# nzfeng/signed-heat-3d

Measured on AMD Instinct MI355X. Metric: grid-nodes/sec end-to-end SHM (conv+PCG), higher is better.
Workload: dtype f64 (Step 1: f64 / packed-f32 tiers)

## Files before the change

signed-heat-3d_amd/csrc/shm_kernels.hip.h:

```cpp
#pragma once
#include <hip/hip_runtime.h>
#include <stdint.h>

#include <type_traits>

#include "shm_constraints.h"
#include "shm_mc_table.h"

namespace shm {

constexpr int kBlock = 256;
constexpr int kMaxPartials = 8192;

__device__ __forceinline__ double wave_sum(double v) {
#pragma unroll
    for (int off = 32; off > 0; off >>= 1) v += __shfl_down(v, off, kWave);
    return v;
}

__device__ __forceinline__ double block_sum(double v, double* lds ) {
    v = wave_sum(v);
    const int lane = threadIdx.x & 63, w = threadIdx.x >> 6;
    if (lane == 0) lds[w] = v;
    __syncthreads();
// ... 584 lines not shown
        for (int r = 0; r < RY; r++) {
            const int j = j0 + r;
            T left = __shfl_up(cur[r + 1][VEC - 1], 1, kWave), right = __shfl_down(cur[r + 1][0], 1, kWave);
            if (active && j < n) {
                if (threadIdx.x == 0 || lane == 0) left = (i > 0) ? row_ptr(kk, j)[-1] : cur[r + 1][0];
                if (threadIdx.x == blockDim.x - 1 || lane == 63 || i + VEC >= n) right = (i + VEC < n) ? row_ptr(kk, j)[VEC] : cur[r + 1][VEC - 1];
                T out[VEC];
#pragma unroll
                for (int e = 0; e < VEC; e++) {
                    const T c = cur[r + 1][e];
                    const T xm = (e == 0) ? left : cur[r + 1][e - 1];
                    const T xp = (e == VEC - 1) ? right : cur[r + 1][e + 1];
                    const T s = (xp + cur[r + 2][e] + nxt[r][e] + xm + cur[r][e] + prv[r][e]) - (T)6 * c;
                    out[e] = -s * ih2;
                    acc += (double)c * (double)out[e];
                }
                store_vec<T, VEC>(q + (size_t)(kk + 1) * plane + (size_t)j * n + i, out);
            }
        }
        if (active && kk + 1 < kk1) {
#pragma unroll
            for (int r = 0; r < RY; r++)
#pragma unroll
                for (int e = 0; e < VEC; e++) {
                    prv[r][e] = cur[r + 1][e];
                    cur[r + 1][e] = nxt[r][e];
                }
            load_row(kk + 1, j0 - 1, cur[0]);
            load_row(kk + 1, j0 + RY, cur[RY + 1]);
        }
    }
    const int tid = threadIdx.y * blockDim.x + threadIdx.x;
    acc = wave_sum(acc);
    if ((tid & 63) == 0) red[tid >> 6] = acc;
    __syncthreads();
    if (tid == 0) partials[lb] = red[0] + red[1] + red[2] + red[3];
}

template <typename T>
__global__ __launch_bounds__(kBlock) void laplacian_kernel(GridParams G, const T* __restrict__ u, T* __restrict__ out) {
    const int n = G.n;
    const size_t plane = (size_t)n * n;
    const size_t nown = (size_t)G.nzl * plane;
    for (size_t v = (size_t)blockIdx.x * kBlock + threadIdx.x; v < nown; v += (size_t)gridDim.x * kBlock) {
        const int kk = (int)(v / plane);
        const int rem = (int)(v - (size_t)kk * plane);
        const int j = rem / n, i = rem - j * n;
        const int k = G.k0 + kk;
        const size_t c = v + plane;
        const T uc = u[c];
        const T xp = (i < n - 1) ? u[c + 1] : uc, xm = (i > 0) ? u[c - 1] : uc;
        const T yp = (j < n - 1) ? u[c + n] : uc, ym = (j > 0) ? u[c - n] : uc;
        const T zp = (k < n - 1) ? u[c + plane] : uc, zm = (k > 0) ? u[c - plane] : uc;
        out[c] = ((xp + yp + zp + xm + ym + zm) - (T)6 * uc) * (T)G.inv_h2;
    }
}

enum Scalar : int {
    SC_RHO0 = 0,
    SC_RHO_A = 1,
    SC_RHO_B = 2,
    SC_UW = 3,
    SC_SHIFT = 4,
    SC_AREA = 5,
    SC_RR = 6,
    SC_RR0 = 7,
    SC_RZ = 8,
    SC_SUMB = 9,
    SC_AXSUM = 10,
    SC_COUNT = 16
};

static __global__ __launch_bounds__(kBlock) void finalize_sum_kernel(const double* __restrict__ partials, int np, double* __restrict__ dst) {
    __shared__ double red[8];
    double s = 0.;
    for (int a = threadIdx.x; a < np; a += kBlock) s += partials[a];
    s = block_sum(s, red);
    if (threadIdx.x == 0) *dst = s;
}

template <typename T, int VEC>
__global__ __launch_bounds__(kBlock) void update_xr_kernel(size_t nvec , size_t off ,
                                                           const double* __restrict__ sc, int rho_slot, const double* __restrict__ pq,
                                                           T* __restrict__ x, const T* __restrict__ p, T* __restrict__ r,
                                                           const T* __restrict__ q, double* __restrict__ partials) {
    __shared__ double red[8];
    const double rho_cur = sc[rho_slot];
    const double alpha_d = rho_cur == 0. ? 0. : rho_cur / *pq;
    const T alpha = (T)alpha_d;
    double acc = 0.;
    for (size_t v = (size_t)blockIdx.x * kBlock + threadIdx.x; v < nvec; v += (size_t)gridDim.x * kBlock) {
        const size_t c = off + v * VEC;
        T xv[VEC], pv[VEC], rv[VEC], qv[VEC];
        load_vec<T, VEC>(x + c, xv);
        load_vec<T, VEC>(p + c, pv);
        load_vec<T, VEC>(r + c, rv);
        load_vec<T, VEC>(q + c, qv);
#pragma unroll
        for (int e = 0; e < VEC; e++) {
            xv[e] += alpha * pv[e];
            rv[e] += alpha * qv[e];
            acc += (double)rv[e] * (double)rv[e];
        }
        store_vec<T, VEC>(x + c, xv);
        store_vec<T, VEC>(r + c, rv);
    }
    acc = block_sum(acc, red);
    if (threadIdx.x == 0) partials[blockIdx.x] = acc;
}

template <typename T, int VEC>
__global__ __launch_bounds__(kBlock) void norm2_kernel(size_t nvec, size_t off, const T* __restrict__ v_, double* __restrict__ partials) {
    __shared__ double red[8];
    double acc = 0.;
    for (size_t v = (size_t)blockIdx.x * kBlock + threadIdx.x; v < nvec; v += (size_t)gridDim.x * kBlock) {
        T a[VEC];
        load_vec<T, VEC>(v_ + off + v * VEC, a);
#pragma unroll
        for (int e = 0; e < VEC; e++) acc += (double)a[e] * (double)a[e];
    }
    acc = block_sum(acc, red);
    if (threadIdx.x == 0) partials[blockIdx.x] = acc;
}

template <typename T, int VEC>
__global__ __launch_bounds__(kBlock) void update_p_kernel(size_t nvec, size_t off, double* __restrict__ sc, int rho_old_slot, int rho_new_slot,
                                                          const double* __restrict__ red0, int init, int use_uw, const T* __restrict__ z,
                                                          T* __restrict__ p) {
    const double rho_new = *red0 - (use_uw ? sc[SC_UW] : 0.);
    const double rho_old = sc[rho_old_slot];
    const double beta_d = (init || rho_old == 0.) ? 0. : rho_new / rho_old;
    const T beta = (T)beta_d;
    for (size_t v = (size_t)blockIdx.x * kBlock + threadIdx.x; v < nvec; v += (size_t)gridDim.x * kBlock) {
        const size_t c = off + v * VEC;
        T zv[VEC], pv[VEC];
        load_vec<T, VEC>(z + c, zv);
        if (!init) load_vec<T, VEC>(p + c, pv);
#pragma unroll
        for (int e = 0; e < VEC; e++) pv[e] = init ? -zv[e] : (-zv[e] + beta * pv[e]);
        store_vec<T, VEC>(p + c, pv);
    }
    if (blockIdx.x == 0 && threadIdx.x == 0) {
        sc[rho_new_slot] = rho_new;
        if (init) sc[SC_RHO0] = rho_new;
    }
}

template <typename T>
__global__ __launch_bounds__(kBlock) void gather_rows_kernel(int m, const int* __restrict__ row_ptr, const uint32_t* __restrict__ ent_node,
                                                             const double* __restrict__ ent_coef, const T* __restrict__ v,
                                                             const double* __restrict__ partials, int np, double* __restrict__ red) {
    __shared__ double lds[8];
    if (blockIdx.x == 0) {
        double s = 0.;
        for (int a = threadIdx.x; a < np; a += kBlock) s += partials[a];
        s = block_sum(s, lds);
        if (threadIdx.x == 0) red[0] = s;
        return;
    }
    const int gid = (blockIdx.x - 1) * kBlock + threadIdx.x, row = gid >> 3, k = gid & 7;
    double term = 0.;
    if (row < m) {
        const int e = row_ptr[row] + k;
        if (e < row_ptr[row + 1]) term = ent_coef[e] * (double)v[ent_node[e]];
    }
    const int base = (int)(threadIdx.x & 63) & ~7;
    double s = 0.;
#pragma unroll
    for (int a = 0; a < 8; a++) s += __shfl(term, base + a, 64);
    if (row < m && k == 0) red[1 + row] = s;
}

template <typename TM, int U>
__global__ __launch_bounds__(kBlock) void ginv_matvec_kernel(int m, int ld, const TM* __restrict__ Ginv, const double* __restrict__ w,
                                                             double* __restrict__ u) {
    __shared__ double lds[8];
    const int row = blockIdx.x;
    const TM* g = Ginv + (size_t)row * ld;
    auto load4 = [&](int c, TM (&gv)[4]) {
        if (sizeof(TM) == 4) *reinterpret_cast<float4*>(gv) = *reinterpret_cast<const float4*>(g + c);
        else {
            *reinterpret_cast<double2*>(gv) = *reinterpret_cast<const double2*>(g + c);
            *reinterpret_cast<double2*>(gv + 2) = *reinterpret_cast<const double2*>(g + c + 2);
        }
    };
    auto dot4 = [&](int c, const TM (&gv)[4]) {
        double s = (double)gv[0] * w[c];
        if (c + 1 < m) s += (double)gv[1] * w[c + 1];
        if (c + 2 < m) s += (double)gv[2] * w[c + 2];
        if (c + 3 < m) s += (double)gv[3] * w[c + 3];
        return s;
    };
    double s = 0.;
    for (int c0 = 0; c0 < m; c0 += U * kBlock * 4) {
        TM gv[U][4];
#pragma unroll
        for (int a = 0; a < U; a++) {
            const int c = c0 + (threadIdx.x + a * kBlock) * 4;
            if (c < m) load4(c, gv[a]);
        }
#pragma unroll
        for (int a = 0; a < U; a++) {
            const int c = c0 + (threadIdx.x + a * kBlock) * 4;
            if (c < m) s += dot4(c, gv[a]);
        }
    }
    s = block_sum(s, lds);
    if (threadIdx.x == 0) u[row] = s;
}
template <typename TM>
static inline void launch_ginv_matvec(hipStream_t st, int rows, int m, int ld, const TM* G, const double* w, double* u) {
    if (m <= 4 * kBlock * 4) hipLaunchKernelGGL((ginv_matvec_kernel<TM, 4>), dim3(rows), dim3(kBlock), 0, st, m, ld, G, w, u);
    else hipLaunchKernelGGL((ginv_matvec_kernel<TM, 8>), dim3(rows), dim3(kBlock), 0, st, m, ld, G, w, u);
}

template <typename T>
__global__ __launch_bounds__(kBlock) void scatter_nodes_kernel(int nnodes, const uint32_t* __restrict__ node_id, const int* __restrict__ node_ptr,
                                                               const int* __restrict__ ent_row, const double* __restrict__ ent_coef,
                                                               const double* __restrict__ u, const double* __restrict__ w, int m,
                                                               double* __restrict__ sc, int save_rr ,
                                                               T* __restrict__ v, int nred, double* scratch , unsigned* ticket ) {
    __shared__ double lds[8];
    if ((int)blockIdx.x < nred) {
        const int chunk = (m + nred - 1) / nred, a0 = (int)blockIdx.x * chunk, a1 = min(m, a0 + chunk);
        double s = 0.;
        for (int a = a0 + (int)threadIdx.x; a < a1; a += kBlock) s += u[a] * w[a];
        s = block_sum(s, lds);
        __shared__ unsigned last;
        if (threadIdx.x == 0) {
            scratch[blockIdx.x] = s;
            __threadfence();
            last = atomicAdd(ticket, 1u) == (unsigned)nred - 1u;
        }
        __syncthreads();
        if (!last) return;
        if (threadIdx.x == 0) {
            __threadfence();
            double tot = 0.;
            for (int b = 0; b < nred; b++) tot += __builtin_nontemporal_load(scratch + b);
            *ticket = 0u;
            sc[SC_UW] = tot;
            if (save_rr) sc[SC_RR] = w[-1] - tot;
            if (save_rr == 2) sc[SC_RR0] = w[-1] - tot;
        }
        return;
    }
    const int t = ((int)blockIdx.x - nred) * kBlock + threadIdx.x;
    if (t >= nnodes) return;
    double s = 0.;
    for (int e = node_ptr[t]; e < node_ptr[t + 1]; e++) s += ent_coef[e] * u[ent_row[e]];
    v[node_id[t]] = (T)((double)v[node_id[t]] - s);
}

template <typename T>
__global__ __launch_bounds__(kBlock) void shift_partial_kernel(int nitems, const ShiftItem* __restrict__ items, int n, const T* __restrict__ x,
                                                               double* __restrict__ partials) {
    __shared__ double red[8];
    double acc = 0.;
    for (int a = blockIdx.x * kBlock + threadIdx.x; a < nitems; a += gridDim.x * kBlock) {
        const ShiftItem it = items[a];
        const double v00 = -(double)x[it.node], v10 = -(double)x[it.node + 1];
        const double v01 = -(double)x[it.node + n], v11 = -(double)x[it.node + n + 1];
        const double a0 = v00 * (1. - it.tx) + v10 * it.tx;
        const double a1 = v01 * (1. - it.tx) + v11 * it.tx;
        acc += it.weight * (a0 * (1. - it.ty) + a1 * it.ty);
    }
    acc = block_sum(acc, red);
    if (threadIdx.x == 0) partials[blockIdx.x] = acc;
}

template <typename T>
__global__ __launch_bounds__(kBlock) void write_phi_kernel(size_t nown, size_t off, const T* __restrict__ x, const double* __restrict__ red0,
                                                           double area_sum, double* __restrict__ sc, T* __restrict__ phi) {
    const double shift = *red0 / area_sum;
    for (size_t v = (size_t)blockIdx.x * kBlock + threadIdx.x; v < nown; v += (size_t)gridDim.x * kBlock)
        phi[off + v] = (T)(-(double)x[off + v] - shift);
    if (blockIdx.x == 0 && threadIdx.x == 0) sc[SC_SHIFT] = shift;
}

template <typename T>
__device__ __forceinline__ double bfs_step(const T* __restrict__ Y0, const T* __restrict__ Y1, const T* __restrict__ Y2, size_t p, size_t q,
                                           double e0, double e1, double e2) {
    double a0 = (double)Y0[q] + (double)Y0[p], a1 = (double)Y1[q] + (double)Y1[p], a2 = (double)Y2[q] + (double)Y2[p];
    const double nrm = sqrt(a0 * a0 + a1 * a1 + a2 * a2);
    a0 /= nrm; a1 /= nrm; a2 /= nrm;
    return a0 * e0 + a1 * e1 + a2 * e2;
}

template <typename T>
__global__ __launch_bounds__(1024) void bfs_plane0_kernel(int n, double cell, double bx, double by, const T* __restrict__ Y0,
                                                          const T* __restrict__ Y1, const T* __restrict__ Y2, T* __restrict__ x) {
    const size_t off = (size_t)n * n;
    if (threadIdx.x == 0) {
        double phi = 0.;
        x[off] = (T)0;
        for (int i = 1; i < n; i++) {
            const double e0 = (i * cell + bx) - ((i - 1) * cell + bx);
            phi = phi + bfs_step<T>(Y0, Y1, Y2, off + i - 1, off + i, e0, 0., 0.);
            x[off + i] = (T)(-phi);
        }
    }
    __syncthreads();
    for (int i = threadIdx.x; i < n; i += blockDim.x) {
        double phi = -(double)x[off + i];
        for (int j = 1; j < n; j++) {
            const double e1 = (j * cell + by) - ((j - 1) * cell + by);
            phi = phi + bfs_step<T>(Y0, Y1, Y2, off + (size_t)(j - 1) * n + i, off + (size_t)j * n + i, 0., e1, 0.);
            x[off + (size_t)j * n + i] = (T)(-phi);
        }
    }
}

template <typename T>
__global__ __launch_bounds__(kBlock) void bfs_z_kernel(GridParams G, double cell, double bz, const T* __restrict__ Y0, const T* __restrict__ Y1,
                                                       const T* __restrict__ Y2, T* __restrict__ x) {
    const size_t plane = (size_t)G.n * G.n;
    const size_t ij = (size_t)blockIdx.x * kBlock + threadIdx.x;
    if (ij >= plane) return;
    const int kk0 = (G.k0 == 0) ? 1 : 0;
    double phi = -(double)x[(size_t)kk0 * plane + ij];
    for (int kk = kk0; kk < G.nzl; kk++) {
        const int k = G.k0 + kk;
        const double e2 = (k * cell + bz) - ((k - 1) * cell + bz);
        const size_t q = (size_t)(kk + 1) * plane + ij, pidx = q - plane;
        phi = phi + bfs_step<T>(Y0, Y1, Y2, pidx, q, 0., 0., e2);
        x[q] = (T)(-phi);
    }
}

constexpr int kDualBlock = 1024;

__device__ __forceinline__ double block_sum_1024(double v, double* lds ) {
    v = wave_sum(v);
    const int lane = threadIdx.x & 63, w = threadIdx.x >> 6;
    __syncthreads();
    if (lane == 0) lds[w] = v;
    __syncthreads();
    if (threadIdx.x == 0) {
        double s = 0.;
        for (int a = 0; a < kDualBlock / kWave; a++) s += lds[a];
        lds[16] = s;
    }
    __syncthreads();
    return lds[16];
}

template <typename T>
__global__ __launch_bounds__(kBlock) void scatter_rows_to_nodes_kernel(int nnodes, const uint32_t* __restrict__ node_id, const int* __restrict__ node_ptr,
                                                                       const int* __restrict__ ent_row, const double* __restrict__ ent_coef,
                                                                       const double* __restrict__ v, int accumulate, T* __restrict__ w, double scale = 1.0,
                                                                       T* __restrict__ saved = nullptr ) {
    const int t = blockIdx.x * kBlock + threadIdx.x;
    if (t >= nnodes) return;
    double s = 0.;
    for (int e = node_ptr[t]; e < node_ptr[t + 1]; e++) s += ent_coef[e] * v[ent_row[e]];
    const T old = w[node_id[t]];
    if (saved) saved[t] = old;
    w[node_id[t]] = (T)((accumulate ? (double)old : 0.) + scale * s);
}
template <typename T>
__global__ __launch_bounds__(kBlock) void restore_nodes_kernel(int nnodes, const uint32_t* __restrict__ node_id, const T* __restrict__ saved, T* __restrict__ w) {
    const int t = blockIdx.x * kBlock + threadIdx.x;
    if (t < nnodes) w[node_id[t]] = saved[t];
}

static __global__ __launch_bounds__(kBlock) void csr_matvec_kernel(int m, const int* __restrict__ ptr, const int* __restrict__ col, const double* __restrict__ val,
                                                            const double* __restrict__ x, double* __restrict__ y) {
    const int r = blockIdx.x * kBlock + threadIdx.x;
    if (r >= m) return;
    double s = 0.;
    for (int e = ptr[r]; e < ptr[r + 1]; e++) s += val[e] * x[col[e]];
    y[r] = s;
}

template <typename T>
__global__ __launch_bounds__(kBlock) void negate_kernel(size_t count, const T* __restrict__ in, T* __restrict__ out) {
    for (size_t v = (size_t)blockIdx.x * kBlock + threadIdx.x; v < count; v += (size_t)gridDim.x * kBlock) out[v] = -in[v];
}

template <typename T>
__global__ __launch_bounds__(kBlock) void sum_kernel(size_t nown, size_t off, const T* __restrict__ v, double* __restrict__ partials) {
    __shared__ double red[8];
    double acc = 0.;
    for (size_t a = (size_t)blockIdx.x * kBlock + threadIdx.x; a < nown; a += (size_t)gridDim.x * kBlock) acc += (double)v[off + a];
    acc = block_sum(acc, red);
    if (threadIdx.x == 0) partials[blockIdx.x] = acc;
}

static __global__ __launch_bounds__(kDualBlock) void dual_init_mu_kernel(int m, const double* __restrict__ sumb, double* __restrict__ mu, double* __restrict__ sc) {
    const double v = *sumb / (double)m;
    for (int a = threadIdx.x; a < m; a += kDualBlock) mu[a] = v;
    if (threadIdx.x == 0) sc[SC_SUMB] = *sumb;
}

static __global__ __launch_bounds__(kDualBlock) void dual_init_residual_kernel(int m, const double* __restrict__ g, const double* __restrict__ Smu,
                                                                        double* __restrict__ r, double* __restrict__ sc, int set_rr0 = 1) {
    __shared__ double lds[17];
    double s = 0.;
    for (int a = threadIdx.x; a < m; a += kDualBlock) s += g[a] - Smu[a];
    const double mean = block_sum_1024(s, lds) / (double)m;
    double rr = 0.;
    for (int a = threadIdx.x; a < m; a += kDualBlock) {
        const double v = g[a] - Smu[a] - mean;
        r[a] = v;
        rr += v * v;
    }
    rr = block_sum_1024(rr, lds);
    if (threadIdx.x == 0) {
        sc[SC_RR] = rr;
        if (set_rr0) sc[SC_RR0] = rr;
    }
}

static __global__ __launch_bounds__(kDualBlock) void dual_direction_kernel(int m, int init, const double* __restrict__ r, double* __restrict__ z,
                                                                    double* __restrict__ p, double* __restrict__ sc) {
    __shared__ double lds[17];
    double s = 0.;
    for (int a = threadIdx.x; a < m; a += kDualBlock) s += z[a];
    const double mean = block_sum_1024(s, lds) / (double)m;
    double rz = 0.;
    for (int a = threadIdx.x; a < m; a += kDualBlock) {
        const double v = z[a] - mean;
        z[a] = v;
        rz += r[a] * v;
    }
    rz = block_sum_1024(rz, lds);
    const double rz_old = sc[SC_RZ];
    const double beta = (init || rz_old == 0.) ? 0. : rz / rz_old;
    for (int a = threadIdx.x; a < m; a += kDualBlock) p[a] = init ? z[a] : z[a] + beta * p[a];
    __syncthreads();
    if (threadIdx.x == 0) sc[SC_RZ] = rz;
}

static __global__ __launch_bounds__(kDualBlock) void dual_update_kernel(int m, const double* __restrict__ Sp, const double* __restrict__ p, double* __restrict__ mu,
                                                                 double* __restrict__ r, double* __restrict__ sc) {
    __shared__ double lds[17];
    double s = 0.;
    for (int a = threadIdx.x; a < m; a += kDualBlock) s += Sp[a];
    const double mean = block_sum_1024(s, lds) / (double)m;
    double pSp = 0.;
    for (int a = threadIdx.x; a < m; a += kDualBlock) pSp += p[a] * (Sp[a] - mean);
    pSp = block_sum_1024(pSp, lds);
    const double rz_cur = sc[SC_RZ];
    const double alpha = rz_cur == 0. ? 0. : rz_cur / pSp;
    double rr = 0.;
    for (int a = threadIdx.x; a < m; a += kDualBlock) {
        mu[a] += alpha * p[a];
        const double v = r[a] - alpha * (Sp[a] - mean);
        r[a] = v;
        rr += v * v;
    }
    rr = block_sum_1024(rr, lds);
    if (threadIdx.x == 0) sc[SC_RR] = rr;
}

static __global__ __launch_bounds__(kBlock) void sum_slabs_kernel(int nslabs, double* const* __restrict__ bufs, int count) {
    const int a = blockIdx.x * kBlock + threadIdx.x;
    if (a >= count) return;
    double s = 0.;
    for (int t = 0; t < nslabs; t++) s += bufs[t][a];
    for (int t = 0; t < nslabs; t++) bufs[t][a] = s;
}

static __global__ __launch_bounds__(kBlock) void scatter_triplets_kernel(size_t cnt, const uint64_t* __restrict__ idx, const double* __restrict__ val,
                                                                  double* __restrict__ dense) {
    for (size_t a = (size_t)blockIdx.x * kBlock + threadIdx.x; a < cnt; a += (size_t)gridDim.x * kBlock) dense[idx[a]] = val[a];
}

template <typename TS, typename TD>
__global__ __launch_bounds__(kBlock) void convert_kernel(size_t count, const TS* __restrict__ src, TD* __restrict__ dst) {
    for (size_t v = (size_t)blockIdx.x * kBlock + threadIdx.x; v < count; v += (size_t)gridDim.x * kBlock) dst[v] = (TD)src[v];
}


struct GjBatch {
    const int* ptrI;
    const size_t* offD;
    const size_t* offW;
    double* D;
    double* P;
    double* R;
    double* C;
};
__device__ __forceinline__ int gj_batch_ld(const GjBatch& B, int a) { return (B.ptrI[a + 1] - B.ptrI[a] + kGJ - 1) / kGJ * kGJ; }

template <int E, int KR>
__device__ __forceinline__ void gj_scalar_step(double (&r)[E][E], double (*rowk)[kGJ], double (*colk)[kGJ], int kq, int ty, int tx, int* __restrict__ flag) {
    const int k = kq * E + KR;
    constexpr int pb = KR & 1;
    if (kq == ty) {
#pragma unroll
        for (int b = 0; b < E; b++) rowk[pb][tx * E + b] = r[KR][b];
    }
    if (kq == tx) {
#pragma unroll
        for (int a = 0; a < E; a++) colk[pb][ty * E + a] = r[a][KR];
    }
    __syncthreads();
    const double piv = rowk[pb][k];
    if (threadIdx.x == 0 && !(piv > 0.)) *flag = 1;
    double ip = __builtin_amdgcn_rcp(piv);
    ip = fma(fma(-piv, ip, 1.0), ip, ip);
    ip = fma(fma(-piv, ip, 1.0), ip, ip);
    double rv[E], cv[E];
#pragma unroll
    for (int b = 0; b < E; b++) rv[b] = rowk[pb][tx * E + b];
#pragma unroll
    for (int a = 0; a < E; a++) cv[a] = colk[pb][ty * E + a];
    const bool rowsel = ty == kq, colsel = tx == kq;
#pragma unroll
    for (int a = 0; a < E; a++)
#pragma unroll
        for (int b = 0; b < E; b++) {
            const double rowv = rv[b] * ip, colv = -cv[a] * ip;
            const double base = fma(-cv[a], rowv, r[a][b]);
            if (a == KR && b == KR) r[a][b] = rowsel ? (colsel ? ip : rowv) : (colsel ? colv : base);
            else if (a == KR) r[a][b] = rowsel ? rowv : base;
            else if (b == KR) r[a][b] = colsel ? colv : base;
            else r[a][b] = base;
        }
}
template <int E, int KR>
__device__ __forceinline__ void gj_scalar_step2(double (&r)[E][E], double* __restrict__ lds, int kq, int ty, int tx, int* __restrict__ flag) {
    static_assert(KR % 2 == 0 && KR + 1 < E, "a pair of pivots inside one block");
    const int k = kq * E + KR;
    double* buf = lds + ((KR >> 1) & 1) * 4 * kGJ;
    double *rowA = buf, *rowB = buf + kGJ, *colA = buf + 2 * kGJ, *colB = buf + 3 * kGJ;
    if (kq == ty) {
#pragma unroll
        for (int b = 0; b < E; b++) {
            rowA[tx * E + b] = r[KR][b];
            rowB[tx * E + b] = r[KR + 1][b];
        }
    }
    if (kq == tx) {
#pragma unroll
        for (int a = 0; a < E; a++) {
            colA[ty * E + a] = r[a][KR];
            colB[ty * E + a] = r[a][KR + 1];
        }
    }
    __syncthreads();
    const double piv0 = rowA[k], m01 = rowA[k + 1], m10 = colA[k + 1], m11 = rowB[k + 1];
    if (threadIdx.x == 0 && !(piv0 > 0.)) *flag = 1;
    double ip0 = __builtin_amdgcn_rcp(piv0);
    ip0 = fma(fma(-piv0, ip0, 1.0), ip0, ip0);
    ip0 = fma(fma(-piv0, ip0, 1.0), ip0, ip0);
    double rv0[E], cv0[E], rv1[E], cv1[E];
#pragma unroll
    for (int b = 0; b < E; b++) {
        rv0[b] = rowA[tx * E + b];
        rv1[b] = rowB[tx * E + b];
    }
#pragma unroll
    for (int a = 0; a < E; a++) {
        cv0[a] = colA[ty * E + a];
        cv1[a] = colB[ty * E + a];
    }
    const bool rowsel = ty == kq, colsel = tx == kq;
    const double rowv0_k1 = m01 * ip0;
#pragma unroll
    for (int b = 0; b < E; b++) {
        const double base = fma(-m10, rv0[b] * ip0, rv1[b]);
        rv1[b] = (b == KR && colsel) ? -m10 * ip0 : base;
// ... 748 lines not shown
```

signed-heat-3d_amd/csrc/shm_solver.hip.h:

```cpp
#pragma once
#include "shm_host.hip.h"
#include "shm_kernels.hip.h"
#include "shm_conv_tiered.hip.h"
#include "shm_cg_fused.hip.h"
#include "shm_twolevel.hip.h"
#include "shm_schur.hip.h"
#include "shm_dct.hip.h"
#include "shm_dct_gemm.hip.h"
#include "shm_green_fft.hip.h"
#include "shm_sample.hip.h"
#include "shm_audit.hip.h"
#include "shm_iso_indexed.hip.h"
#include "shm_iso_components.hip.h"
#include "shm_raycast.hip.h"
#include "shm_redistance.hip.h"
#include "shm_redistance_exact.hip.h"
#include "shm_plan.h"

namespace shm {

template <typename T> constexpr int vec_width() { return sizeof(T) == 8 ? 2 : 4; }

template <typename T>
struct Slab {
    int k0 = 0, k1 = 0, nzl = 0;
    size_t plane = 0, nown = 0, ntot = 0;
    DevArray<T> Y0, Y1, Y2, r , x, p, q , z ;
    DevArray<double> partials, pq_partials , red , pq , u , sc;
    DevArray<unsigned> proj_ticket;
    DevArray<int> row_ptr, ent_row, node_ptr;
    DevArray<uint32_t> ent_node, node_id;
    DevArray<double> ent_coef, nent_coef;
    DevArray<ShiftItem> shift_items;
    DevArray<double> dv;
    DevArray<int> layer_order;
    DevArray<int> sample_order;
    DevArray<unsigned char> sample_rule;
    DevArray<unsigned long long> sample_ctr;
    long long sample_key = -1;
    int sample_blocks = 0;
    long long layer_order_key = -1;
    DevArray<double> div_partials;
    int div_sum_blocks = 0;
    DevArray<T> touched_save;
    DevArray<T> W1, W2;
    DevArray<T> S1, S2, S4;
    DevArray<int> act_x, act_y;
    DevArray<unsigned> act_z;
    DevArray<int> act_planes;
    int n_act_planes = 0;
    int n_act_x = 0, n_act_y = 0;
    int n_touched = 0, n_shift = 0;
    GridParams gp{};
};

template <typename T>
struct Solver final : SolverBase {
    shm_config cfg;
    hipStream_t stream = nullptr;
    hipStream_t stream2 = nullptr;
    hipStream_t stream3 = nullptr;
    std::unique_ptr<Event> e_sch_in, e_sch_done, e_gs_done;
    hipStream_t stream_h = nullptr;
    int n = 0, alloc_n = -1;
    size_t N = 0;
    double cell = 0., lambda = 0.;
    double bbox_min[3] = {0, 0, 0};
    double conv_ctr[3] = {0, 0, 0};
    double conv_wscale = 1.;
    int64_t S = 0;
    std::vector<double> h_pos, h_wn, h_area;
    double area_sum = 0., conv_far_gap = 0., conv_skip_base = 3.0e38, last_host_setup_ms = 0., last_setup_wall_ms = 0.;
    double conv_tier_log = 0., conv_tier_skip_base = 3.0e38;
    double conv_drop_K = 64., conv_drop_eps64 = 2e-9, conv_drop_eps32 = 6.0e-8;
    double conv_w_span = 0.;
    DevArray<double> d_src_t;
    DevArray<float> d_clusters_t;
    int n_clusters_t = 0;
    bool conv_tiered = false;
    bool conv_tier_exact = false;
    bool conv_tiered32 = false;
    bool conv_reference = false;
    int step1_selected = SHM_STEP1_AUTO;
    int last_step1_arith = SHM_STEP1_AUTO;
    double last_step1_budget = 0.;
    bool fold_pq = false;
    int fold_pq_np = 0;
    double step1_budget = 0.;
    DevArray<unsigned long long> d_pair_counters;
    DevArray<unsigned> d_unit_counters;
    static constexpr int kMaxConvLaunches = 256;
    int conv_launch_index = 0;
    int conv_launches_last = 0;
    int n_clusters = 0;
    int conv_grid_cap = 1 << 30;
    bool o_fast_hint = false;
    int num_cus = 256;
    DevArray<T> d_src;
    DevArray<float> d_src32;
    DevArray<float> d_clusters;
    DevArray<double> d_exptab;
    std::vector<Slab<T>> slabs;
    int total_slabs = 1, first_slab = 0;
    std::vector<int32_t> slab_bounds;
    bool slabs_equal = true;
    void slab_range(int slab, int32_t* k0, int32_t* k1) const {
        *k0 = slab_bounds[(size_t)slab];
        *k1 = slab_bounds[(size_t)slab + 1];
    }
    bool have_problem = false, have_conv = false, have_div = false, have_phi = false, have_constraints = false;
    std::vector<Row> rows;
    std::vector<std::vector<ShiftItem>> shift_host;
    int m = 0, mp = 0;
    DevArray<double> Ginv, gjP, gjR, gjC;
    DevArray<float> Ginv32;
    struct TwoLevel {
        bool on = false;
        int box = 16, P = 0, nI = 0, nS = 0, nSp = 0, ysz = 0;
        DevArray<int> ptrI, ptrS, rowsI, colsS, sepRow, adj_ptr, adj_idx, colour_list, rowBox, chunkBox, chunkCol, tBox, tRow, sBox, sRow;
        DevArray<size_t> offW;
        DevArray<double> gjP, gjR, gjC;
        int nChunks = 0, nTChunks = 0, nbMax = 0;
        int schur_ptr[9] = {0, 0, 0, 0, 0, 0, 0, 0, 0};
        DevArray<size_t> offD, offE;
        DevArray<double> D, E, Tm, tbuf, ybuf, vS, uS;
        DevArray<float> D32, E32, T32;
        int colour_ptr[9] = {0, 0, 0, 0, 0, 0, 0, 0, 0};
        size_t szD = 0, szE = 0;
        TlBoxes view() const { return TlBoxes{ptrI.p, ptrS.p, offD.p, offE.p, rowsI.p, colsS.p}; }
    } tl;
    int ginv_rows = 0, ginv_ld = 0;
    DevArray<int> gjFlag;
    DevArray<double*> d_redptrs;
    DevArray<int> Bptr, Bcol;
    DevArray<double> Bval;
    bool have_B = false;
    using TP = T;
    DevArray<Cplx<TP>> d_tw, d_om;
    DevArray<TP> d_lam;
    DevArray<double> d_lam64;
    DevArray<double> gd_Cm, gd_Ct, gd_W1, gd_W2;
    DevArray<double> gs_lam, gs_ctab, gs_Cm, gs_Ct, gs_W0, gs_W1, gs_T, Sdense, d_rowT;
    DevArray<int> d_rowX;
    std::vector<double> h_gs_lam, h_gs_ctab, h_rowT;
    std::vector<Cplx<double>> h_gs_tw;
    DevArray<Cplx<double>> gs_tw;
    std::vector<int> h_rowX;
    bool have_S = false;
    DevArray<double> Sinv, Sinv_ones ;
    PlanIn plan_in;
    Plan plan;
    double conv_est_total_ms = 1e30;
    int log2n = 0;
    bool precond_ready = false;
    double* h_pinned = nullptr;
    Rccl::comm_t comm = nullptr;
    int vec = 1;
    std::unique_ptr<Solver<T>> full;
    bool solve_only = false;
    bool full_problem_set = false;
    bool pool_held = false;

    explicit Solver(const shm_config& c, bool solve_only_ = false) : cfg(c), solve_only(solve_only_) {
        int ndev = 0;
        hipError_t e = hipGetDeviceCount(&ndev);
        if (e != hipSuccess || ndev <= 0)
            throw Error(SHM_ERR_HIP, fmt("no HIP device available (%s); this library has no CPU fallback",
                                          e == hipSuccess ? "device count 0" : hipGetErrorString(e)));
        if (cfg.device < 0 || cfg.device >= ndev) throw Error(SHM_ERR_INVALID, fmt("device %d out of range [0,%d)", cfg.device, ndev));
        HIPCHK(hipSetDevice(cfg.device));
        HIPCHK(hipStreamCreateWithFlags(&stream, hipStreamNonBlocking));
        {
            hipDeviceProp_t prop;
            HIPCHK(hipGetDeviceProperties(&prop, cfg.device));
            conv_grid_cap = std::max(1, prop.multiProcessorCount * 4);
            num_cus = prop.multiProcessorCount;
        }
        {
            int least = 0, greatest = 0;
            HIPCHK(hipDeviceGetStreamPriorityRange(&least, &greatest));
            HIPCHK(hipStreamCreateWithPriority(&stream2, hipStreamNonBlocking, greatest));
        }
        HIPCHK(hipHostMalloc((void**)&h_pinned, 64 * sizeof(double)));
        if (cfg.world > 1 && !cfg.rccl_unique_id) throw Error(SHM_ERR_INVALID, "world>1 needs rccl_unique_id");
        if (cfg.rccl_unique_id) {
            Rccl& R = Rccl::get();
            Rccl::unique_id id;
            memcpy(&id, cfg.rccl_unique_id, sizeof id);
            R.chk(R.CommInitRank(&comm, cfg.world, id, cfg.rank), "ncclCommInitRank");
        }
        PinnedPool::get().acquire(cfg.device);
        pool_held = true;
    }
    ~Solver() override {
        (void)hipSetDevice(cfg.device);
        if (comm) (void)Rccl::get().CommDestroy(comm);
        if (h_pinned) (void)hipHostFree(h_pinned);
        for (void* b : smp_pinned)
            if (b) (void)hipHostFree(b);
        for (void* b : ray_pinned)
            if (b) (void)hipHostFree(b);
        slabs.clear();
        if (stream) (void)hipStreamDestroy(stream);
        if (stream2) (void)hipStreamDestroy(stream2);
        if (stream3) (void)hipStreamDestroy(stream3);
        if (stream_h) (void)hipStreamDestroy(stream_h);
        if (pool_held) PinnedPool::get().release(cfg.device);
    }

    void log(const char* f, ...) {
        if (!cfg.verbose) return;
        va_list ap;
        va_start(ap, f);
        vfprintf(stderr, f, ap);
        va_end(ap);
        fputc('\n', stderr);
    }

    static int grid_for(size_t work_items, int cap = 2048) {
        size_t b = (work_items + kBlock - 1) / kBlock;
        if (b < 1) b = 1;
        if (b > (size_t)cap) b = cap;
        return (int)b;
    }

    void set_problem(const shm_sources& src, const shm_grid& g) override {
        HIPCHK(hipSetDevice(cfg.device));
        if (g.n < 2) throw Error(SHM_ERR_INVALID, "grid.n must be >= 2");
        if (!(g.cell > 0.) || !std::isfinite(g.cell)) throw Error(SHM_ERR_INVALID, "grid.cell must be positive and finite");
        if (src.S <= 0 || !src.pos || !src.wnormal || !src.area) throw Error(SHM_ERR_INVALID, "sources: S>0 and non-null arrays required");
        if (!(src.lambda > 0.) || !std::isfinite(src.lambda)) throw Error(SHM_ERR_INVALID, "sources.lambda must be positive and finite");
        if (src.S > (int64_t)1 << 28) throw Error(SHM_ERR_INVALID, "too many sources");
        total_slabs = cfg.world * cfg.local_slabs;
        first_slab = cfg.rank * cfg.local_slabs;
        if (g.n < total_slabs) throw Error(SHM_ERR_INVALID, fmt("grid.n=%d smaller than the number of z-slabs %d", g.n, total_slabs));
        n = g.n;
        N = (size_t)n * n * n;
        cell = g.cell;
        lambda = src.lambda;
        for (int a = 0; a < 3; a++) bbox_min[a] = g.bbox_min[a];
        S = src.S;
        h_pos.assign(src.pos, src.pos + 3 * S);
        h_wn.assign(src.wnormal, src.wnormal + 3 * S);
        h_area.assign(src.area, src.area + S);
        for (int64_t s = 0; s < S; s++)
            for (int a = 0; a < 3; a++) {
                const double d = (h_pos[3 * s + a] - bbox_min[a]) / cell;
                if (!(d >= 0.) || !(std::floor(d) + 1. <= (double)(n - 1)))
                    throw Error(SHM_ERR_INVALID, fmt("source %lld lies outside the grid cells", (long long)s));
            }
        area_sum = 0.;
        for (int64_t s = 0; s < S; s++) area_sum += h_area[s];
        {
            double lo[3] = {1e300, 1e300, 1e300}, hi[3] = {-1e300, -1e300, -1e300};
            for (int64_t s = 0; s < S; s++)
                for (int a = 0; a < 3; a++) {
                    lo[a] = std::min(lo[a], h_pos[3 * s + a]);
                    hi[a] = std::max(hi[a], h_pos[3 * s + a]);
                }
            const double ext = std::max({hi[0] - lo[0], hi[1] - lo[1], hi[2] - lo[2], 1e-300});
            auto spread = [](uint64_t v) {
                v &= 0x1fffff;
                v = (v | v << 32) & 0x1f00000000ffffULL;
                v = (v | v << 16) & 0x1f0000ff0000ffULL;
                v = (v | v << 8) & 0x100f00f00f00f00fULL;
                v = (v | v << 4) & 0x10c30c30c30c30c3ULL;
                v = (v | v << 2) & 0x1249249249249249ULL;
                return v;
            };
            std::vector<std::pair<uint64_t, int64_t>> order((size_t)S);
            for (int64_t s = 0; s < S; s++) {
                uint64_t code = 0;
                for (int a = 0; a < 3; a++) {
                    const uint64_t q = (uint64_t)std::min(1048575.0, std::max(0.0, (h_pos[3 * s + a] - lo[a]) / ext * 1048575.0));
                    code |= spread(q) << a;
                }
                order[(size_t)s] = {code, s};
            }
            std::sort(order.begin(), order.end());
            for (int a = 0; a < 3; a++) conv_ctr[a] = bbox_min[a] + 0.5 * (double)(n - 1) * cell;
            constexpr int kConvCluster = conv_cluster<T>();
            n_clusters = (int)((S + kConvCluster - 1) / kConvCluster);
            const int64_t Spad = (int64_t)n_clusters * kConvCluster;
            std::vector<T> packed((size_t)Spad * 6, (T)0);
            std::vector<float> packed32((size_t)Spad * 6, 0.f), cl((size_t)n_clusters * kConvClusterRec, 0.f);
            double amin = 1e300, amax = 0.;
            for (int64_t s = 0; s < S; s++) {
                const double w = std::sqrt(h_wn[3 * s] * h_wn[3 * s] + h_wn[3 * s + 1] * h_wn[3 * s + 1] + h_wn[3 * s + 2] * h_wn[3 * s + 2]);
                if (w > 0.) amin = std::min(amin, w);
                amax = std::max(amax, w);
            }
            conv_wscale = amax > 0. && std::isfinite(amax) ? std::ldexp(1.0, -std::ilogb(amax) - 1) : 1.0;
            conv_w_span = amax > 0. && amin < 1e300 ? std::log(amax / amin) : 0.;
            const double wscale = sizeof(T) == 4 ? conv_wscale : 1.0;
            for (int64_t t = 0; t < Spad; t++) {
                const int64_t s = order[(size_t)std::min<int64_t>(t, S - 1)].second;
                for (int a = 0; a < 3; a++) {
                    packed[6 * t + a] = (T)(h_pos[3 * s + a] - conv_ctr[a]);
                    packed32[6 * t + a] = (float)(h_pos[3 * s + a] - conv_ctr[a]);
                    if (t < S) {
                        packed[6 * t + 3 + a] = (T)(h_wn[3 * s + a] * wscale);
                        packed32[6 * t + 3 + a] = (float)(h_wn[3 * s + a] * wscale);
                    }
                }
            }
            for (int c = 0; c < n_clusters; c++) {
                double cc[3] = {0, 0, 0};
                for (int e = 0; e < kConvCluster; e++)
                    for (int a = 0; a < 3; a++) cc[a] += (double)packed[6 * ((size_t)c * kConvCluster + e) + a];
                for (int a = 0; a < 3; a++) cc[a] /= kConvCluster;
                double rad = 0.;
                for (int e = 0; e < kConvCluster; e++) {
                    double d2 = 0.;
                    for (int a = 0; a < 3; a++) {
                        const double d = (double)packed[6 * ((size_t)c * kConvCluster + e) + a] - cc[a];
                        d2 += d * d;
                    }
                    rad = std::max(rad, std::sqrt(d2));
                }
                for (int a = 0; a < 3; a++) cl[kConvClusterRec * (size_t)c + a] = (float)cc[a];
                cl[kConvClusterRec * (size_t)c + 3] = (float)(rad * 1.00001 + 1e-30);
                double wmax2 = 0., wsum = 0.;
                for (int e = 0; e < kConvCluster; e++) {
                    double w2 = 0.;
                    for (int a = 0; a < 3; a++) {
                        const double w = (double)packed[6 * ((size_t)c * kConvCluster + e) + 3 + a];
                        w2 += w * w;
                    }
                    wmax2 = std::max(wmax2, w2);
                    wsum += std::sqrt(w2);
                }
                cl[kConvClusterRec * (size_t)c + 4] = wmax2 > 0. ? (float)(0.5 * std::log(wmax2) + 1e-5) : -1.0e30f;
                cl[kConvClusterRec * (size_t)c + 5] = wsum > 0. ? (float)(std::log(wsum) + 1e-5) : -1.0e30f;
            }
            {
                const double far_log = 25.0;
                conv_far_gap = (far_log + std::log(std::max(1.0, amax / std::max(amin, 1e-300)))) / lambda;
                const double eps = sizeof(T) == 8 ? 1.1e-16 : 6.0e-8;
                const char* sk = knob("SHM_CONV_NO_SKIP");
                conv_skip_base = sk ? 3.0e38 : std::log((double)S / eps);
                const char* tl = knob("SHM_CONV_TIER_LOG");
                conv_tier_log = tl ? atof(tl) : 8.0;
                conv_tier_skip_base = sk ? 3.0e38 : std::log((double)S / 2e-9);
                conv_drop_eps64 = sk ? 0. : 2e-9;
                conv_drop_eps32 = sk ? 0. : 6.0e-8;
                conv_drop_K = drop_rule_K(S, h_wn.data(), lambda);
                select_step1_arith(SHM_STEP1_AUTO);
            }
            d_src.upload(packed, stream);
            d_src32.upload(packed32, stream);
            {
                const int per = conv_chunk<T>();
                const int nchunks = (n_clusters + per - 1) / per;
                for (int g = 0; g < nchunks; g++) {
                    const int a = g * per, b = std::min(n_clusters, a + per);
                    double cc[3] = {0, 0, 0};
                    for (int c = a; c < b; c++)
                        for (int t = 0; t < 3; t++) cc[t] += cl[kConvClusterRec * (size_t)c + t];
                    for (int t = 0; t < 3; t++) cc[t] /= (b - a);
                    double rad = 0., lnw = -1.0e30;
                    for (int c = a; c < b; c++) {
                        double d2 = 0.;
                        for (int t = 0; t < 3; t++) {
                            const double d = (double)cl[kConvClusterRec * (size_t)c + t] - cc[t];
                            d2 += d * d;
                        }
                        rad = std::max(rad, std::sqrt(d2) + (double)cl[kConvClusterRec * (size_t)c + 3]);
                        lnw = std::max(lnw, (double)cl[kConvClusterRec * (size_t)c + 4]);
                    }
                    for (int t = 0; t < 3; t++) cl.push_back((float)cc[t]);
                    cl.push_back((float)(rad * 1.00001 + 1e-30));
                    cl.push_back((float)lnw);
                    cl.push_back(0.f);
                }
            }
            d_clusters.upload(cl, stream);
            if constexpr (sizeof(T) == 8) {
                if (!solve_only)
                    conv_drop_K = choose_drop_K(reinterpret_cast<const double*>(packed.data()), n_clusters, cl.data(), kConvClusterRec, lambda, n, cell, conv_drop_eps64, S, conv_drop_K);
            }
            if constexpr (sizeof(T) == 4) {
                n_clusters_t = (int)((S + kTierCluster - 1) / kTierCluster);
                const int64_t Sp = (int64_t)n_clusters_t * kTierCluster;
                std::vector<double> pk((size_t)Sp * 6, 0.);
                for (int64_t t = 0; t < Sp; t++) {
                    const int64_t sidx = order[(size_t)std::min<int64_t>(t, S - 1)].second;
                    for (int a = 0; a < 3; a++) {
                        pk[6 * t + a] = h_pos[3 * sidx + a] - conv_ctr[a];
                        if (t < S) pk[6 * t + 3 + a] = h_wn[3 * sidx + a];
                    }
                }
                std::vector<float> clt((size_t)n_clusters_t * kConvClusterRec, 0.f);
                for (int c = 0; c < n_clusters_t; c++) {
                    const double* q = pk.data() + 6 * (size_t)c * kTierCluster;
                    double cc[3] = {0, 0, 0}, rad = 0., wmax2 = 0., wsum = 0.;
                    for (int e = 0; e < kTierCluster; e++)
                        for (int a = 0; a < 3; a++) cc[a] += q[6 * e + a] / kTierCluster;
                    for (int e = 0; e < kTierCluster; e++) {
                        double d2 = 0., w2 = 0.;
                        for (int a = 0; a < 3; a++) {
                            d2 += (q[6 * e + a] - cc[a]) * (q[6 * e + a] - cc[a]);
                            w2 += q[6 * e + 3 + a] * q[6 * e + 3 + a];
                        }
                        rad = std::max(rad, std::sqrt(d2));
                        wmax2 = std::max(wmax2, w2);
                        wsum += std::sqrt(w2);
                    }
                    for (int a = 0; a < 3; a++) clt[kConvClusterRec * (size_t)c + a] = (float)cc[a];
                    clt[kConvClusterRec * (size_t)c + 3] = (float)(rad * 1.00001 + 1e-30);
                    clt[kConvClusterRec * (size_t)c + 4] = wmax2 > 0. ? (float)(0.5 * std::log(wmax2) + 1e-5) : -1.0e30f;
                    clt[kConvClusterRec * (size_t)c + 5] = wsum > 0. ? (float)(std::log(wsum) + 1e-5) : -1.0e30f;
                }
                if (!solve_only)
                    conv_drop_K = choose_drop_K(pk.data(), n_clusters_t, clt.data(), kConvClusterRec, lambda, n, cell, conv_drop_eps32, S, conv_drop_K);
                d_src_t.upload(pk, stream);
                d_clusters_t.upload(clt, stream);
            }
            if (!d_exptab.p) {
                std::vector<double> tab(2048);
                for (int j = 0; j < 2048; j++) tab[(size_t)j] = std::exp2((double)j / 2048.0);
                d_exptab.upload(tab, stream);
            }
            HIPCHK(hipStreamSynchronize(stream));
        }

        {
            const bool weighted = cfg.slab_plan == SHM_SLAB_PLAN_STEP1 && total_slabs > 1 && !solve_only;
            slab_bounds.assign((size_t)total_slabs + 1, 0);
            if (weighted) {
                std::vector<double> w((size_t)n);
                step1_plane_weights_host(S, h_pos.data(), h_wn.data(), lambda, n, bbox_min, cell, sizeof(T) == 8 ? SHM_F64 : SHM_F32, conv_tier_log, w.data(),
                                         sizeof(T) == 4 && knob("SHM_CONV32_CLASSIC") == nullptr);
                plan_slabs_weighted(n, total_slabs, w.data(), sizeof(T) == 8 ? 4 : 8, slab_bounds);
            } else {
                for (int sidx = 0; sidx < total_slabs; sidx++) {
                    int32_t k0, k1;
                    shm_plan_slab(n, total_slabs, sidx, &k0, &k1);
                    slab_bounds[(size_t)sidx] = k0;
                    slab_bounds[(size_t)sidx + 1] = k1;
                }
            }
            slabs_equal = true;
            for (int sidx = 0; sidx < total_slabs; sidx++) {
                int32_t k0, k1;
                shm_plan_slab(n, total_slabs, sidx, &k0, &k1);
                slabs_equal = slabs_equal && slab_bounds[(size_t)sidx] == k0 && slab_bounds[(size_t)sidx + 1] == k1;
            }
        }
        vec = (n % vec_width<T>() == 0) ? vec_width<T>() : 1;
        if (!(have_problem && n == alloc_n && (int)slabs.size() == cfg.local_slabs)) {
            slabs.clear();
            slabs.resize(cfg.local_slabs);
        }
        alloc_n = n;
        for (int ls = 0; ls < cfg.local_slabs; ls++) {
            Slab<T>& sl = slabs[ls];
            int32_t k0, k1;
            slab_range(first_slab + ls, &k0, &k1);
            sl.k0 = k0;
            sl.k1 = k1;
            sl.nzl = k1 - k0;
            sl.plane = (size_t)n * n;
            sl.nown = sl.plane * sl.nzl;
            sl.ntot = sl.plane * (sl.nzl + 2);
            if (sl.ntot >= ((size_t)1 << 32)) throw Error(SHM_ERR_INVALID, "slab too large for 32-bit local node indices; use more slabs");
            if (!solve_only)
                for (DevArray<T>* a : {&sl.Y0, &sl.Y1, &sl.Y2}) a->alloc(sl.ntot);
            for (DevArray<T>* a : {&sl.r, &sl.x, &sl.p, &sl.q}) a->alloc(sl.ntot);
            HIPCHK(hipMemsetAsync(sl.p.p, 0, sl.ntot * sizeof(T), stream));
            if (!solve_only) HIPCHK(hipMemsetAsync(sl.Y2.p, 0, sl.ntot * sizeof(T), stream));
            sl.partials.alloc(std::max<size_t>(kMaxPartials, (size_t)n * n / 8 + 8));
            sl.pq.alloc(1);
            sl.sc.alloc(SC_COUNT);
            HIPCHK(hipMemsetAsync(sl.sc.p, 0, SC_COUNT * sizeof(double), stream));
            sl.gp.n = n;
            sl.gp.nzl = sl.nzl;
            sl.gp.k0 = sl.k0;
            sl.gp.inv_h = 1. / cell;
            sl.gp.inv_h2 = 1. / (cell * cell);
        }
        HIPCHK(hipStreamSynchronize(stream));
        precond_ready = false;
        have_problem = true;
        have_conv = have_div = have_phi = have_constraints = false;
        iso_idx_valid = false;
        ray_bricks_valid = false;
        redist_valid = false;
        audit_src_ready = false;
        full_problem_set = false;
        if (!(cfg.world > 1 && !solve_only && n >= 4 && n <= 1024)) full.reset();
        log("[shm] problem set: n=%d N=%zu S=%lld slabs=%d(local %d) vec=%d", n, N, (long long)S, total_slabs, cfg.local_slabs, vec);
    }

    bool full_wanted() const { return cfg.world > 1 && !solve_only && n >= 4 && n <= 1024; }
    void ensure_full() {
        if (!full_wanted()) return;
        if (!full) {
            shm_config c = cfg;
            c.world = 1;
            c.rank = 0;
            c.local_slabs = 1;
            c.rccl_unique_id = nullptr;
            full.reset(new Solver<T>(c, true));
        }
        if (!full_problem_set) {
            shm_sources src{};
            src.S = S;
            src.pos = h_pos.data();
            src.wnormal = h_wn.data();
            src.area = h_area.data();
            src.lambda = lambda;
            shm_grid g{};
            g.n = n;
            for (int a = 0; a < 3; a++) g.bbox_min[a] = bbox_min[a];
            g.cell = cell;
            full->set_problem(src, g);
            full_problem_set = true;
        }
    }
    Step1Kernel step1_kernel() const { return conv_tiered ? kStep1TieredF64 : conv_tiered32 ? kStep1TieredF32 : kStep1Untiered; }
    PlanIn plan_inputs(const shm_opts* o) const {
        PlanIn in;
        in.f64 = sizeof(T) == 8; in.n = n; in.S = S; in.total_slabs = total_slabs;
        in.full_wanted = full_wanted(); in.fft_available = fft_available(); in.gemm_dct = gemm_dct(); in.fused_available = fused_available();
        in.step1 = step1_kernel(); in.conv_est_total_ms = conv_est_total_ms;
        if (o) {
            in.solver = o->solver; in.preconditioner = o->preconditioner; in.dual_form = o->dual_form;
            in.step1_budget = o->step1_budget; in.fast = o->fast_integration != 0;
        }
        in.knobs = plan_knobs(knob);
        return in;
    }
    void select_step1_arith(int arith) {
        if (arith != SHM_STEP1_AUTO && arith != SHM_STEP1_EXACT_F64 && arith != SHM_STEP1_REFERENCE_F64) throw Error(SHM_ERR_INVALID, "unknown step1_arith");
        conv_reference = sizeof(T) == 8 && arith == SHM_STEP1_REFERENCE_F64;
        conv_tiered = sizeof(T) == 8 && arith == SHM_STEP1_AUTO && knob("SHM_CONV_EXACT") == nullptr && tier_exponent_span_ok();
        conv_tier_exact = sizeof(T) == 8 && arith == SHM_STEP1_EXACT_F64 && knob("SHM_CONV_EXACT_CLASSIC") == nullptr && tier_exponent_span_ok(true);
        conv_tiered = conv_tiered || conv_tier_exact;
        conv_tiered32 = sizeof(T) == 4 && knob("SHM_CONV32_CLASSIC") == nullptr && tier_exponent_span_ok();
        step1_selected = sizeof(T) == 4 || (conv_tiered && !conv_tier_exact) ? SHM_STEP1_AUTO : conv_reference ? SHM_STEP1_REFERENCE_F64 : SHM_STEP1_EXACT_F64;
    }
    bool tier_exponent_span_ok(bool every_pair = false) const {
        const double rt = std::sqrt(2 * 3.5 * 3.5 + 1.5 * 1.5) * cell;
        const double reach = every_pair ? lambda * std::sqrt(3.0) * (double)(n - 1) * cell : std::min((sizeof(T) == 8 ? conv_tier_skip_base : conv_skip_base) + 2.0794415416798357, 1.0e6);
        const double bits = (4.0 * rt * lambda + reach + std::max(conv_w_span, 43.0)) * 1.4426950408889634 + 16.0;
        return bits < 990.0;
    }
    void need_problem() const {
        if (!have_problem) throw Error(SHM_ERR_STATE, "shm_grid_set_problem has not been called");
    }

    const int* layer_order_for(Slab<T>& sl, int kk_begin, int layers, int npt) {
        const bool off = knob("SHM_TIER_LAYER_ORDER") != nullptr && atoi(knob("SHM_TIER_LAYER_ORDER")) == 0;
        if (off || layers < 16) return nullptr;
        const long long key = ((long long)kk_begin << 40) ^ ((long long)layers << 20) ^ ((long long)npt << 8) ^ (long long)sl.k0 * 0x9E3779B1LL;
        if (sl.layer_order.p && sl.layer_order_key == key) return sl.layer_order.p;
        std::vector<std::pair<double, int>> byc((size_t)layers);
        for (int l = 0; l < layers; l++) byc[(size_t)l] = {std::fabs((double)(sl.k0 + kk_begin - 1 + l * npt) + 0.5 * (npt - 1) - 0.5 * (n - 1)), l};
        std::stable_sort(byc.begin(), byc.end());
        std::vector<int> order;
        order.reserve((size_t)layers);
        for (int q = 0; q < 8; q++)
            for (int r = q; r < layers; r += 8) order.push_back(byc[(size_t)r].second);
        sl.layer_order.upload(order, stream);
        sl.layer_order_key = key;
        return sl.layer_order.p;
    }
    int far_rule_now() const {
        const char* e = knob("SHM_TIER_FAR_RULE");
        if (e) return atoi(e) != 0;
        return 0;
    }
    bool far_rule_plan(Slab<T>& sl, int planes, int npt) {
        if (sizeof(T) != 8 || !conv_tiered || conv_tier_exact || slabs.size() != 1 || total_slabs != 1 || knob("SHM_TIER_FAR_RULE") != nullptr) return false;
        if (step1_budget > 0. && step1_budget != kTierBudget) return false;
        const int layers = (planes + npt - 1) / npt;
        if (layers < 64 || layers % 8 != 0 || planes % npt != 0) return false;
        const long long key = ((long long)layers << 32) ^ ((long long)npt << 16);
        if (sl.sample_key != key) {
            std::vector<char> role((size_t)layers, 2);
            std::vector<int> A, B1;
            const int nA = 8;
            for (int a = 0; a < nA; a++) {
                const int l = (int)(((long long)(2 * a + 1) * layers) / (2 * nA));
                A.push_back(l);
                role[(size_t)l] = 1;
            }
            std::vector<std::pair<double, int>> byc;
            for (int l = 0; l < layers; l++)
                if (role[(size_t)l] != 1) byc.push_back({std::fabs((double)(sl.k0 + l * npt) + 0.5 * (npt - 1) - 0.5 * (n - 1)), l});
            std::stable_sort(byc.begin(), byc.end());
            for (int a = 0; a < 8; a++) B1.push_back(byc[(size_t)a].second);
            std::vector<int> order;
            std::vector<unsigned char> rule;
            size_t next_rest = 8;
            std::vector<std::vector<int>> rest(8);
            {
                std::vector<int> want(8);
                for (int q = 0; q < 8; q++) want[(size_t)q] = layers / 8 - 1 - ((nA == 8 || q % 2 == 0) ? 1 : 0);
                bool any = true;
                while (any && next_rest < byc.size()) {
                    any = false;
                    for (int q = 0; q < 8 && next_rest < byc.size(); q++)
                        if ((int)rest[(size_t)q].size() < want[(size_t)q]) {
                            rest[(size_t)q].push_back(byc[next_rest++].second);
                            any = true;
                        }
                }
            }
            for (int q = 0, a = 0; q < 8; q++) {
                if (nA == 8 || q % 2 == 0) {
                    order.push_back(A[(size_t)a++]);
                    rule.push_back(1);
                }
                order.push_back(B1[(size_t)q]);
                rule.push_back(0);
                for (int l : rest[(size_t)q]) {
                    order.push_back(l);
                    rule.push_back(2);
                }
            }
            if ((int)order.size() != layers) throw Error(SHM_ERR_INVALID, "far_rule_plan: internal count mismatch");
            sl.sample_blocks = nA * ((n + kTierTX - 1) / kTierTX) * ((n + kTierTY - 1) / kTierTY);
            sl.sample_order.upload(order, stream);
            sl.sample_rule.upload(rule, stream);
            sl.sample_ctr.alloc(4);
            sl.sample_key = key;
        }
        return true;
    }
    void launch_conv() {
        const bool slab_log = knob("SHM_CONV_SLAB_LOG") != nullptr;
        Event slab_ev[2];
        unsigned long long slab_pairs_seen[2] = {0, 0};
        for (Slab<T>& sl : slabs) {
            if (slab_log) {
                HIPCHK(hipStreamSynchronize(stream));
                slab_ev[0].record(stream);
            }
            ConvParams P;
            P.layer_order = nullptr;
            P.unit_rule = nullptr;
            P.sample_ctr = nullptr;
            P.sample_blocks = 0;
            P.far_rule = conv_tiered && !conv_tier_exact && sizeof(T) == 8 ? far_rule_now() : 0;
            P.n = n;
            P.kk_begin = 1;
            P.kk_end = sl.nzl + 1;
            P.k0 = sl.k0;
            for (int a = 0; a < 3; a++) P.bbox_min[a] = bbox_min[a] - conv_ctr[a];
            P.cell = cell;
            P.lambda = lambda;
            P.cexp = -lambda * 2954.639443740597;
            P.cexp_inv = 1.0 / std::fabs(P.cexp);
            P.S = n_clusters * conv_cluster<T>();
            P.n_clusters = n_clusters;
            P.far_gap = conv_reference ? 3.0e38f : (float)conv_far_gap;
            const double budget = step1_budget > 0. ? step1_budget : kTierBudget;
            const double g_shift = std::log(budget / kTierBudget);
            P.tier_log = conv_tier_exact ? 3.0e38f : conv_tiered32 ? -1.0e30f : (float)std::max(2.0, conv_tier_log - g_shift);
            P.wscale = conv_wscale;
            {
                const double ratio = budget / kTierEpsFar;
                P.far_redo_ratio = ratio > 0. ? (float)ratio : 3.0e38f;
            }
            P.skip_base = conv_tier_exact || conv_reference ? 3.0e38f : (float)std::min(conv_tiered ? conv_tier_skip_base - g_shift : conv_skip_base, 3.0e38);
            {
                const double eps = conv_tier_exact ? 0. : sizeof(T) == 8 ? conv_drop_eps64 * (budget / kTierBudget) : conv_drop_eps32;
                const double eps_soft = 0.875 * eps, tau = eps_soft / conv_drop_K, tau_hard = 0.125 * eps / (double)std::max<int64_t>(1, S);
                P.drop_eps_soft = (float)eps_soft;
                P.drop_ltau = eps > 0. ? (float)std::log2(tau) : -3.0e38f;
                P.drop_ltau_hard = eps > 0. ? (float)std::log2(tau_hard) : -3.0e38f;
                P.drop_tau_hard = (float)(tau_hard * 1.0001);
                P.drop_check = P.far_redo_ratio < 1.0e30f ? (float)((double)P.far_redo_ratio / budget) : (float)(1.0 / kTierEpsFar);
                P.tier_u0 = (float)kTierU0;
                P.tier_flush = kTierFlush;
            }
            P.inv_lambda = (float)(1.0 / lambda);
            P.tiles_x = (n + kConvTile - 1) / kConvTile;
            P.tiles_y = P.tiles_x;
            const int planes = P.kk_end - P.kk_begin;
            const bool npt4 = (long long)P.tiles_x * P.tiles_y * ((planes + 15) / 16) >= conv_grid_cap;
            const bool npt4_env = knob("SHM_CONV_NPT4") != nullptr;
            const bool npt8 = sizeof(T) == 4 && !npt4_env && npt4 && (long long)P.tiles_x * P.tiles_y * ((planes + 31) / 32) >= conv_grid_cap;
            const int tile_z = npt8 ? 32 : npt4 ? 16 : 8;
            const double half_z = 0.5 * ((npt8 ? 16 : tile_z) - 1);
            const double tile_diam = 2.0 * std::sqrt(2 * 3.5 * 3.5 + half_z * half_z) * cell;
            P.exact_offset = (lambda * tile_diam > 30.0) ? 1 : 0;
            const int tiles_z = (planes + tile_z - 1) / tile_z;
            P.n_tiles = P.tiles_x * P.tiles_y * tiles_z;
            unsigned grid = (unsigned)std::min(P.n_tiles, conv_grid_cap);
            {
                int occ = 0;
                const void* kfn = npt4 ? reinterpret_cast<const void*>(conv_normalize_kernel<T, 4>) : reinterpret_cast<const void*>(conv_normalize_kernel<T, 2>);
                if constexpr (sizeof(T) == 4)
                    if (npt8) kfn = reinterpret_cast<const void*>(conv_normalize_kernel<float, 8>);
                if (conv_tiered) kfn = npt4 ? reinterpret_cast<const void*>(conv_tiered_kernel<4, double, true>) : reinterpret_cast<const void*>(conv_tiered_kernel<2, double, true>);
                if (conv_tiered32) kfn = npt4 ? reinterpret_cast<const void*>(conv_tiered_kernel<4, float, false>) : reinterpret_cast<const void*>(conv_tiered_kernel<2, float, false>);
                if (hipOccupancyMaxActiveBlocksPerMultiprocessor(&occ, kfn, kBlock, 0) != hipSuccess || occ < 1) occ = 2;
                const unsigned resident = (unsigned)(occ * num_cus);
                const double pairs = (double)sl.nown * (double)S;
                const double conv_est_ms = pairs / (sizeof(T) == 8 ? 1.2e9 : 3.5e9);
                conv_est_total_ms = (&sl == &slabs[0] ? 0. : conv_est_total_ms) + conv_est_ms;
                const double setup_est_ms = 2.2e-3 * (double)std::min<int64_t>(S, (int64_t)8 * n * n);
                if (conv_tiered || conv_tiered32) grid = std::min(grid, resident);
                if (!o_fast_hint && conv_est_ms < 4.0 * setup_est_ms && grid > resident - resident / 8) grid = resident - resident / 8;
            }
            const bool uniform_tiles = lambda * cell * n < 100.;
            const int want_chunks = (conv_tiered || conv_tiered32) ? 1 : (uniform_tiles && conv_est_total_ms >= 10. ? std::min(16, (int)std::lround(conv_est_total_ms / 2.5)) : 1);
            const int nchunks = std::max(1, std::min(tiles_z, want_chunks));
            const int chunk_planes = ((tiles_z + nchunks - 1) / nchunks) * tile_z;
            if (!d_pair_counters.p) d_pair_counters.alloc(3);
            if (!d_unit_counters.p) d_unit_counters.alloc(8 * kMaxConvLaunches);
            if (&sl == &slabs[0]) {
                HIPCHK(hipMemsetAsync(d_pair_counters.p, 0, 3 * sizeof(unsigned long long), stream));
                HIPCHK(hipMemsetAsync(d_unit_counters.p, 0, 8 * kMaxConvLaunches * sizeof(unsigned), stream));
                conv_launch_index = 0;
                conv_launches_last = 0;
            }
            unsigned long long* const cnt = d_pair_counters.p;
            auto launch_range = [&](int b0, int b1, int sel, int rule = -1, const int* order = nullptr, int order_layers = 0) {
                if (b1 <= b0) return;
                conv_launches_last++;
                const int tz_sel = 4 * sel;
                ConvParams Pc = P;
                Pc.kk_begin = 1 + b0;
                Pc.kk_end = std::min(sl.nzl + 1, 1 + b1);
                Pc.n_tiles = P.tiles_x * P.tiles_y * ((Pc.kk_end - Pc.kk_begin + tz_sel - 1) / tz_sel);
                const dim3 g((unsigned)std::min<long long>(Pc.n_tiles, grid));
                if (conv_tiered || conv_tiered32) {
                    if (conv_launch_index >= kMaxConvLaunches) throw Error(SHM_ERR_INVALID, "too many Step-1 launches");
                    unsigned* const head = d_unit_counters.p + 8 * conv_launch_index++;
                    const int npt = npt4 ? 4 : 2;
                    Pc.tiles_x = (n + kTierTX - 1) / kTierTX;
                    Pc.tiles_y = (n + kTierTY - 1) / kTierTY;
                    const int layers = order ? order_layers : (Pc.kk_end - Pc.kk_begin + npt - 1) / npt;
                    Pc.n_tiles = Pc.tiles_x * Pc.tiles_y * layers;
                    Pc.layer_order = order ? order : layer_order_for(sl, Pc.kk_begin, layers, npt);
                    if (rule >= 0) Pc.far_rule = rule;
                    const dim3 gt((unsigned)std::min<long long>((Pc.n_tiles + 3) / 4, grid));
                    if constexpr (sizeof(T) == 8) {
                        if (npt4)
                            hipLaunchKernelGGL((conv_tiered_kernel<4, double, true>), gt, dim3(kBlock), 0, stream, Pc, d_src.p, d_clusters.p, d_exptab.p, sl.Y0.p, sl.Y1.p, sl.Y2.p, cnt, head);
                        else
                            hipLaunchKernelGGL((conv_tiered_kernel<2, double, true>), gt, dim3(kBlock), 0, stream, Pc, d_src.p, d_clusters.p, d_exptab.p, sl.Y0.p, sl.Y1.p, sl.Y2.p, cnt, head);
                    } else {
                        Pc.S = n_clusters_t * kTierCluster;
                        Pc.n_clusters = n_clusters_t;
                        if (npt4)
                            hipLaunchKernelGGL((conv_tiered_kernel<4, float, false>), gt, dim3(kBlock), 0, stream, Pc, d_src_t.p, d_clusters_t.p, d_exptab.p, sl.Y0.p, sl.Y1.p, sl.Y2.p, cnt, head);
                        else
                            hipLaunchKernelGGL((conv_tiered_kernel<2, float, false>), gt, dim3(kBlock), 0, stream, Pc, d_src_t.p, d_clusters_t.p, d_exptab.p, sl.Y0.p, sl.Y1.p, sl.Y2.p, cnt, head);
                    }
                    return;
                }
                unsigned* head = nullptr;
                if (conv_launch_index < kMaxConvLaunches) head = d_unit_counters.p + 8 * conv_launch_index++;
                if constexpr (sizeof(T) == 4) {
                    if (sel == 8) {
                        hipLaunchKernelGGL((conv_normalize_kernel<float, 8>), g, dim3(kBlock), 0, stream, Pc, d_src.p, d_src32.p, d_clusters.p, d_exptab.p, sl.Y0.p, sl.Y1.p,
                                           sl.Y2.p, cnt, head);
                        return;
                    }
                }
                if (sel >= 4)
                    hipLaunchKernelGGL((conv_normalize_kernel<T, 4>), g, dim3(kBlock), 0, stream, Pc, d_src.p, d_src32.p, d_clusters.p, d_exptab.p, sl.Y0.p, sl.Y1.p, sl.Y2.p, cnt, head);
                else
                    hipLaunchKernelGGL((conv_normalize_kernel<T, 2>), g, dim3(kBlock), 0, stream, Pc, d_src.p, d_src32.p, d_clusters.p, d_exptab.p, sl.Y0.p, sl.Y1.p, sl.Y2.p, cnt, head);
            };
            const int sel0 = npt8 ? 8 : npt4 ? 4 : 2;
            if (sizeof(T) == 4 && !conv_tiered32 && nchunks == 1 && sel0 > 2 && planes % tile_z != 0) {
                int b = (planes / tile_z) * tile_z;
                launch_range(0, b, sel0);
                for (int sel = sel0 / 2; sel >= 2; sel /= 2) {
                    const int tz_sel = 4 * sel, take = sel > 2 ? ((planes - b) / tz_sel) * tz_sel : planes - b;
                    launch_range(b, b + take, sel);
                    b += take;
                }
            } else if (far_rule_plan(sl, planes, npt4 ? 4 : 2)) {
                const int npt = npt4 ? 4 : 2, layers = planes / npt;
                HIPCHK(hipMemsetAsync(sl.sample_ctr.p, 0, 4 * sizeof(unsigned long long), stream));
                P.unit_rule = sl.sample_rule.p;
                P.sample_ctr = sl.sample_ctr.p;
                P.sample_blocks = sl.sample_blocks;
                launch_range(0, planes, sel0, 0, sl.sample_order.p, layers);
                P.unit_rule = nullptr;
            } else {
                for (int b0 = 0; b0 < planes; b0 += chunk_planes) launch_range(b0, std::min(planes, b0 + chunk_planes), sel0);
            }
            if (slab_log) {
                slab_ev[1].record(stream);
                HIPCHK(hipStreamSynchronize(stream));
                unsigned long long h[2] = {0, 0};
                HIPCHK(hipMemcpy(h, d_pair_counters.p, sizeof h, hipMemcpyDeviceToHost));
                fprintf(stderr, "[shm] step1 slab planes [%d,%d) ms %.3f pairs_fp64 %.6e pairs_fp32 %.6e\n", sl.k0, sl.k1, elapsed(slab_ev[0], slab_ev[1]),
                        (double)(h[0] - slab_pairs_seen[0]), (double)(h[1] - slab_pairs_seen[1]));
                slab_pairs_seen[0] = h[0];
                slab_pairs_seen[1] = h[1];
            }
        }
        HIPCHK(hipGetLastError());
        exchange_Y_halos();
        have_conv = true;
        last_step1_arith = step1_selected;
        last_step1_budget = sizeof(T) == 8 && conv_tiered && !conv_tier_exact ? (step1_budget > 0. ? step1_budget : kTierBudget) : 0.;
    }
    void exchange_Y_halos() {
        if (total_slabs <= 1) return;
        for (int sel : {ARR_Y0, ARR_Y1, ARR_Y2}) halo_exchange(sel);
    }

    void launch_div(int scrub) {
        for (Slab<T>& sl : slabs) {
            if (vec == 1) {
                hipLaunchKernelGGL((divergence_kernel<T>), dim3((unsigned)((n + kBlock - 1) / kBlock), (unsigned)n, (unsigned)sl.nzl), dim3(kBlock), 0, stream, sl.gp,
                                   sl.Y0.p, sl.Y1.p, sl.Y2.p, sl.r.p, scrub);
                sl.div_sum_blocks = 0;
                continue;
            }
            constexpr int V = vec_width<T>();
            const DivGeometry g = div_geometry(sl);
            sl.div_partials.alloc(g.nblk);
            sl.div_sum_blocks = (int)g.nblk;
            hipLaunchKernelGGL((divergence_march_kernel<T, V>), dim3(g.nblk), dim3(kBlock), 0, stream, sl.gp, g.LX, g.xchunks, g.rowgroups, g.ZC, sl.Y0.p, sl.Y1.p, sl.Y2.p,
                               sl.r.p, scrub, sl.div_partials.p);
        }
        HIPCHK(hipGetLastError());
        have_div = true;
    }
    struct DivGeometry {
        int LX, xchunks, rowgroups, ZC;
        unsigned nblk;
    };
    DivGeometry div_geometry(const Slab<T>& sl) const {
        constexpr int V = vec_width<T>();
        const int lanes = (n + V - 1) / V;
        int LX = 1;
        while (LX < lanes && LX < kBlock) LX *= 2;
        const int xchunks = (lanes + LX - 1) / LX, RB = kBlock / LX, rowgroups = (n + RB - 1) / RB;
        const int ZC = 4;
        return {LX, xchunks, rowgroups, ZC, (unsigned)((long long)xchunks * rowgroups * ((sl.nzl + ZC - 1) / ZC))};
    }
    void sum_b_in_div_order(Slab<T>& sl, hipStream_t on) {
        if (vec == 1) {
            sl.div_sum_blocks = 0;
            return;
        }
        constexpr int V = vec_width<T>();
        const DivGeometry g = div_geometry(sl);
        sl.div_partials.alloc(g.nblk);
        sl.div_sum_blocks = (int)g.nblk;
        hipLaunchKernelGGL((sum_march_kernel<T, V>), dim3(g.nblk), dim3(kBlock), 0, on, sl.gp, g.LX, g.xchunks, g.rowgroups, g.ZC, sl.r.p, sl.div_partials.p);
        HIPCHK(hipGetLastError());
    }

    void run_conv(int step1_arith) override {
        need_problem();
        HIPCHK(hipSetDevice(cfg.device));
        step1_budget = 0.;
        select_step1_arith(step1_arith);
        launch_conv();
        HIPCHK(hipStreamSynchronize(stream));
    }
    void run_divergence(int scrub) override {
        need_problem();
        if (!have_conv) throw Error(SHM_ERR_STATE, "run_conv must precede run_divergence");
        HIPCHK(hipSetDevice(cfg.device));
        launch_div(scrub);
        HIPCHK(hipStreamSynchronize(stream));
    }

    void build_rows() {
        shm::build_rows(S, h_pos.data(), bbox_min, cell, n, rows);
        m = (int)rows.size();
        mp = ((m + kGJ - 1) / kGJ) * kGJ;
    }

    void build_shift_items(hipStream_t stream) {
        shift_host.resize(slabs.size());
        for (size_t si = 0; si < slabs.size(); si++) {
            Slab<T>& sl = slabs[si];
            shift_items_for_slab(S, h_pos.data(), h_area.data(), bbox_min, cell, n, sl.k0, sl.k1, shift_host[si]);
            sl.n_shift = (int)shift_host[si].size();
            sl.shift_items.upload(shift_host[si], stream);
        }
    }
    void upload_red_tables(hipStream_t stream) {
        std::vector<double*> ptrs;
        for (Slab<T>& sl : slabs) ptrs.push_back(sl.red.p);
        for (Slab<T>& sl : slabs) ptrs.push_back(sl.pq.p);
        d_redptrs.upload(ptrs, stream);
        HIPCHK(hipStreamSynchronize(stream));
    }
    void build_shift_items_only() {
        build_shift_items(stream);
        upload_red_tables(stream);
    }

    double estimate_step1_ms_tiered() const {
        if (S <= 0) return 0.;
        if (conv_tier_exact) {
            double nodes = 0.;
            for (const Slab<T>& sl : slabs) nodes += (double)sl.nown;
            return nodes * (double)S * 1.229e-9;
        }
        const int K = (int)std::max<int64_t>(32, std::min<int64_t>(128, 2000000 / S));
        const int64_t stride = std::max<int64_t>(1, (S * K + 1999999) / 2000000);
        uint64_t st = 0x9E3779B97F4A7C15ULL;
        auto rnd = [&]() {
            st = st * 6364136223846793005ULL + 1442695040888963407ULL;
            return (double)(st >> 11) * (1.0 / 9007199254740992.0);
        };
        const double ext = (double)(n - 1) * cell, rt2 = 2.0 * 5.17 * cell;
        const double r_near_gap = rt2 + conv_tier_log / lambda, r_keep_gap = rt2 + std::log(std::min((double)S, conv_drop_K) / (0.875 * 2e-9)) / lambda;
        std::vector<float> d2((size_t)S);
        size_t c_near = 0, c_keep = 0;
        for (int k = 0; k < K; k++) {
            const float x = (float)(bbox_min[0] + rnd() * ext), y = (float)(bbox_min[1] + rnd() * ext), z = (float)(bbox_min[2] + rnd() * ext);
            float dmin = 3.0e38f;
            for (int64_t s = 0; s < S; s += stride) {
                const float dx = x - (float)h_pos[3 * s], dy = y - (float)h_pos[3 * s + 1], dz = z - (float)h_pos[3 * s + 2];
                const float v = dx * dx + dy * dy + dz * dz;
                d2[(size_t)s] = v;
                dmin = std::min(dmin, v);
            }
            const double rn = std::sqrt((double)dmin);
            const float tn = (float)((rn + r_near_gap) * (rn + r_near_gap)), tk = (float)((rn + r_keep_gap) * (rn + r_keep_gap));
            for (int64_t s = 0; s < S; s += stride) {
                c_near += d2[(size_t)s] < tn;
                c_keep += d2[(size_t)s] < tk;
            }
        }
        const double sampled = (double)K * (double)((S + stride - 1) / stride);
        const double f_keep = (double)c_keep / sampled;
        const double f_near = conv_tiered32 ? 0. : (double)c_near / sampled;
        double nodes = 0.;
        for (const Slab<T>& sl : slabs) nodes += (double)sl.nown;
        return nodes * (double)S * (1.229e-9 * f_near + 1.84e-10 * (f_keep - f_near) + 3.3e-12);
    }
    double step1_hidden_ms(double conv_est_ms) const {
        double nodes_here = 0.;
        for (const Slab<T>& sl : slabs) nodes_here += (double)sl.nown;
        const double share = std::min(1.0, conv_est_ms / std::max(1e-30, nodes_here * (double)S / 1.2e9));
        return estimate_step1_ms_tiered() * share;
    }

    void build_constraints(const PlanIn& in, const Plan& p) {
        hipStream_t stream = stream2;
// ... 223 lines not shown
                const double* Rp = gjR.p + (size_t)((k + 1) & 1) * kGJ * mp;
                const double* Cp = gjC.p + (size_t)((k + 1) & 1) * mp * kGJ;
                hipLaunchKernelGGL(gj_step_kernel, dim3(grid), dim3(kBlock), 0, stream, M, mp, nb, k, Rp, Cp, Rn, Cn, gjFlag.p, plan.setup_prio);
            }
        } else if (outer == 1) {
            for (int kb = 0; kb < nb; kb++) {
                launch_pivot(kb);
                hipLaunchKernelGGL(gj_panels_kernel, dim3(nb), dim3(kBlock), 0, stream, M, mp, kb, gjP.p, gjR.p, 0, gjC.p, c_ld, 0, plan.setup_prio);
                hipLaunchKernelGGL((gj_update_kernel<GJ_ALL>), dim3((unsigned)((size_t)nb * (nb + 1) / 2)), dim3(kBlock), 0, stream, M, mp, nb, kb, 0, 1,
                                   gjR.p, 0, gjC.p, c_ld, 0, kGJ, plan.setup_prio);
            }
        } else {
            for (int k0 = 0; k0 < nb; k0 += outer) {
                const int nO = std::min(outer, nb - k0);
                for (int t = 0; t < nO; t++) {
                    const int kb = k0 + t;
                    launch_pivot(kb);
                    hipLaunchKernelGGL(gj_panels_kernel, dim3(nb), dim3(kBlock), 0, stream, M, mp, kb, gjP.p, gjR.p, t * kGJ, gjC.p, c_ld, t * kGJ, plan.setup_prio);
                    hipLaunchKernelGGL((gj_update_kernel<GJ_CROSS>), dim3((unsigned)(nO * nb + nO * k0)), dim3(kBlock), 0, stream, M, mp, nb, kb, k0, nO,
                                       gjR.p, t * kGJ, gjC.p, c_ld, t * kGJ, kGJ, plan.setup_prio);
                }
                const size_t nr = (size_t)(nb - nO);
                if (nr > 0)
                    hipLaunchKernelGGL((gj_update_kernel<GJ_REST>), dim3((unsigned)(nr * (nr + 1) / 2)), dim3(kBlock), 0, stream, M, mp, nb, -1, k0, nO,
                                       gjR.p, 0, gjC.p, c_ld, 0, nO * kGJ, plan.setup_prio);
            }
        }
        if (nb > 1) hipLaunchKernelGGL(gj_mirror_kernel, dim3((unsigned)((size_t)nb * (nb - 1) / 2)), dim3(kBlock), 0, stream, M, mp);
        HIPCHK(hipGetLastError());
    }
    void enqueue_invert_G() {
        const int mp = ginv_ld;
        enqueue_gj_invert(Ginv.p, mp);
        Ginv32.alloc((size_t)mp * mp);
        hipLaunchKernelGGL((convert_kernel<double, float>), dim3(grid_for((size_t)mp * mp, 4096)), dim3(kBlock), 0, stream2, (size_t)mp * mp, Ginv.p, Ginv32.p);
        HIPCHK(hipGetLastError());
    }
    void enqueue_green_table(hipStream_t st) {
        const int P = n + 8;
        const size_t n1 = (size_t)n + 1;
        {
            const double pi = 3.14159265358979323846;
            h_gs_lam.resize(n);
            h_gs_ctab.resize(2 * (size_t)n);
            for (int k = 0; k < n; k++) h_gs_lam[k] = (2. - 2. * std::cos(pi * k / n)) / (cell * cell);
            for (int r = 0; r < 2 * n; r++) h_gs_ctab[r] = std::cos(pi * r / n);
            gs_lam.upload(h_gs_lam, st);
            gs_ctab.upload(h_gs_ctab, st);
            gs_T.alloc(n1 * n1 * P);
        }
        {
            DevArray<double>&W0 = gs_W0, &W1 = gs_W1, &W2 = gs_W0;
            gs_Cm.alloc(n1 * n);
            gs_Ct.alloc((size_t)n * P);
            W0.alloc(std::max((size_t)n * n * n, (size_t)n * n1 * P));
            W1.alloc((size_t)n * n * P);
            const bool by_fft = (n & (n - 1)) == 0 && n >= 16 && n <= 512;
            if (by_fft) {
                const double pi = 3.14159265358979323846;
                h_gs_tw.resize(2 * (size_t)n);
                for (int t = 0; t < n; t++) {
                    h_gs_tw[(size_t)t] = {std::cos(2. * pi * t / n), -std::sin(2. * pi * t / n)};
                    h_gs_tw[(size_t)n + t] = {std::cos(pi * t / n), -std::sin(pi * t / n)};
                }
                gs_tw.upload(h_gs_tw, st);
                HIPCHK(hipMemsetAsync(W1.p, 0, (size_t)n * n * P * sizeof(double), st));
                hipLaunchKernelGGL(green_symbol_kernel, dim3((unsigned)std::min(n * n, 8 * num_cus)), dim3(kBlock), 0, st, n, gs_lam.p, W0.p);
                const long long Pl = P, n1l = (long long)n1;
                auto pass = [&](bool xpass, int ntiles, int tiles_a, DctAddr in, DctAddr out, const double* src, double* dst) {
                    CosiParams C;
                    C.ntiles = ntiles;
                    C.tiles_a = tiles_a;
                    C.in = in;
                    C.out = out;
                    const dim3 g((unsigned)std::min(ntiles, 16 * num_cus));
                    const Cplx<double>*tw = gs_tw.p, *om = gs_tw.p + n;
                    int l2 = 0;
                    while ((1 << l2) < n) l2++;
#define SHM_COSI_CASE(L)                                                                                                                              \
    case L:                                                                                                                                            \
        if (xpass) hipLaunchKernelGGL((cosi_lines_kernel<L, true>), g, dim3(kBlock), 0, st, C, src, dst, tw, om, plan.setup_prio);                         \
        else hipLaunchKernelGGL((cosi_lines_kernel<L, false>), g, dim3(kBlock), 0, st, C, src, dst, tw, om, plan.setup_prio);                              \
        break;
                    switch (l2) {
                        SHM_COSI_CASE(4) SHM_COSI_CASE(5) SHM_COSI_CASE(6) SHM_COSI_CASE(7) SHM_COSI_CASE(8) SHM_COSI_CASE(9)
                        default: throw Error(SHM_ERR_INVALID, "Green's table by FFT: n out of range");
                    }
#undef SHM_COSI_CASE
                };
                auto addr = [](long long a_stride, long long b_stride, long long line_stride, long long elem_stride) {
                    DctAddr A;
                    A.off = 0; A.a_stride = a_stride; A.b_stride = b_stride; A.line_stride = line_stride; A.elem_stride = elem_stride;
                    A.seg_stride = 0; A.seg_shift = 30; A.seg_mask = 0x3fffffff;
                    return A;
                };
                const int L = kCosiL;
                pass(true, n * n / L, n * n / L, addr((long long)L * n, 0, n, 1), addr((long long)L * Pl, 0, Pl, 1), W0.p, W1.p);
                pass(false, n * (P / L), P / L, addr(L, (long long)n * Pl, 1, Pl), addr(L, n1l * Pl, 1, Pl), W1.p, W2.p);
                pass(false, (int)(n1l * Pl / L), (int)(n1l * Pl / L), addr(L, 0, 1, n1l * Pl), addr(L, 0, 1, n1l * Pl), W2.p, gs_T.p);
                HIPCHK(hipGetLastError());
                return;
            }
            HIPCHK(hipMemsetAsync(gs_Ct.p, 0, (size_t)n * P * sizeof(double), st));
            hipLaunchKernelGGL(cosine_tables_kernel, dim3(grid_for(n1 * n, 1024)), dim3(kBlock), 0, st, n, P, gs_ctab.p, gs_Cm.p, gs_Ct.p);
            hipLaunchKernelGGL(green_symbol_kernel, dim3((unsigned)std::min(n * n, 8 * num_cus)), dim3(kBlock), 0, st, n, gs_lam.p, W0.p);
            const bool narrow = plan_in.tiered();
            auto tiles = [](size_t v) { return (unsigned)((v + kGemmT - 1) / kGemmT); };
            auto gemm = [&](unsigned batches, int M, int N, int K, const double* A, int lda, long long sA, const double* B, int ldb, long long sB, double* C, int ldc, long long sC) {
                if (narrow)
                    hipLaunchKernelGGL(dgemm_rm_kernel<1>, dim3((unsigned)((N + 31) / 32), tiles((size_t)M), batches), dim3(kBlock), 0, st, M, N, K, A, lda, sA, B, ldb, sB, C, ldc, sC, plan.setup_prio);
                else
                    hipLaunchKernelGGL(dgemm_rm_kernel<4>, dim3(tiles((size_t)N), tiles((size_t)M), batches), dim3(kBlock), 0, st, M, N, K, A, lda, sA, B, ldb, sB, C, ldc, sC, plan.setup_prio);
            };
            gemm(1, n * n, P, n, W0.p, n, 0LL, gs_Ct.p, P, 0LL, W1.p, P, 0LL);
            gemm((unsigned)n, (int)n1, P, n, gs_Cm.p, n, 0LL, W1.p, P, (long long)n * P, W2.p, P, (long long)(n1 * P));
            gemm(1, (int)n1, (int)(n1 * P), n, gs_Cm.p, n, 0LL, W2.p, (int)(n1 * P), 0LL, gs_T.p, (int)(n1 * P), 0LL);
            HIPCHK(hipGetLastError());
        }
    }
    void prepare_schur() {
        hipStream_t st = stream2;
        have_S = false;
        if (!plan.explicit_S) return;
        if (!plan.green_early) enqueue_green_table(st);
        schur_row_order(rows, h_rowX, h_rowT);
        d_rowX.upload(h_rowX, st);
        d_rowT.upload(h_rowT, st);
        Sdense.alloc((size_t)mp * mp);
        if (!stream3) {
            int least = 0, greatest = 0;
            HIPCHK(hipDeviceGetStreamPriorityRange(&least, &greatest));
            HIPCHK(hipStreamCreateWithPriority(&stream3, hipStreamNonBlocking, greatest));
            e_sch_in.reset(new Event());
            e_sch_done.reset(new Event());
        }
        e_sch_in->record(st);
    }
    void enqueue_schur() {
        if (!plan.explicit_S) return;
        const bool dual_direct = plan.dual_form == SHM_DUAL_DIRECT;
        hipStream_t st = dual_direct ? stream2 : stream3;
        HIPCHK(hipStreamWaitEvent(st, e_sch_in->e, 0));
        const int P = n + 8;
        if (plan.green_early) HIPCHK(hipStreamWaitEvent(st, e_gs_done->e, 0));
        HIPCHK(hipMemsetAsync(Sdense.p, 0, (size_t)mp * mp * sizeof(double), st));
        const unsigned mt = (unsigned)((m + 15) / 16);
        hipLaunchKernelGGL(schur_assemble_kernel, dim3(mt, mt), dim3(kBlock), 0, st, m, mp, n, P, d_rowX.p, d_rowT.p, gs_T.p, Sdense.p, plan.setup_prio);
        HIPCHK(hipGetLastError());
        if (dual_direct) {
            Sinv.alloc((size_t)mp * mp);
            HIPCHK(hipMemcpyAsync(Sinv.p, Sdense.p, (size_t)mp * mp * sizeof(double), hipMemcpyDeviceToDevice, st));
            if (mp > m) hipLaunchKernelGGL(set_diagonal_kernel, dim3((unsigned)((mp - m + kBlock - 1) / kBlock)), dim3(kBlock), 0, st, Sinv.p, mp, m, mp, 1.0);
            enqueue_gj_invert(Sinv.p, mp, true);
            Sinv_ones.alloc((size_t)2 * mp);
            hipLaunchKernelGGL(fill_kernel, dim3((unsigned)((m + kBlock - 1) / kBlock)), dim3(kBlock), 0, st, Sinv_ones.p + mp, m, 1.0);
            launch_ginv_matvec<double>(st, m, m, mp, Sinv.p, Sinv_ones.p + mp, Sinv_ones.p);
        } else {
            e_sch_done->record(st);
            HIPCHK(hipStreamWaitEvent(stream2, e_sch_done->e, 0));
        }
        have_S = true;
    }
    void finish_invert_G() {
        hipStream_t stream = stream2;
        int flag[2] = {0, 0};
        if (!tl.on) HIPCHK(hipMemsetAsync(gjFlag.p + 1, 0, sizeof(int), stream));
        HIPCHK(hipMemcpyAsync(flag, gjFlag.p, 2 * sizeof(int), hipMemcpyDeviceToHost, stream));
        HIPCHK(hipStreamSynchronize(stream));
        if (flag[0] || flag[1]) throw Error(SHM_ERR_SINGULAR, "A A^T is not positive definite (duplicate or degenerate constraint rows)");
    }

    void allreduce(int which , int count) {
        auto buf = [&](Slab<T>& sl) { return which == 0 ? sl.red.p : sl.pq.p; };
        if (slabs.size() > 1) {
            double** slot = d_redptrs.p + (which ? slabs.size() : 0);
            hipLaunchKernelGGL(sum_slabs_kernel, dim3((count + kBlock - 1) / kBlock), dim3(kBlock), 0, stream, (int)slabs.size(), slot, count);
        }
        if (comm) {
            Rccl& R = Rccl::get();
            R.chk(R.AllReduce(buf(slabs[0]), buf(slabs[0]), (size_t)count, Rccl::kFloat64, Rccl::kSum, comm, stream), "ncclAllReduce");
            for (size_t s = 1; s < slabs.size(); s++)
                HIPCHK(hipMemcpyAsync(buf(slabs[s]), buf(slabs[0]), (size_t)count * sizeof(double), hipMemcpyDeviceToDevice, stream));
        }
    }

    void halo_exchange_p() { halo_exchange(ARR_P); }
    void halo_exchange(int sel) { halo_exchange(sel, stream); }
    void halo_exchange(int sel, hipStream_t stream) {
        const size_t pb = slabs[0].plane * sizeof(T);
        for (size_t s = 0; s + 1 < slabs.size(); s++) {
            Slab<T>&a = slabs[s], &b = slabs[s + 1];
            HIPCHK(hipMemcpyAsync(arr(b, sel), arr(a, sel) + (size_t)a.nzl * a.plane, pb, hipMemcpyDeviceToDevice, stream));
            HIPCHK(hipMemcpyAsync(arr(a, sel) + (size_t)(a.nzl + 1) * a.plane, arr(b, sel) + b.plane, pb, hipMemcpyDeviceToDevice, stream));
        }
        if (comm) {
            Rccl& R = Rccl::get();
            const int dt = sizeof(T) == 8 ? Rccl::kFloat64 : Rccl::kFloat32;
            Slab<T>&lo = slabs.front(), &hi = slabs.back();
            const size_t cnt = lo.plane;
            R.chk(R.GroupStart(), "ncclGroupStart");
            if (cfg.rank > 0) {
                R.chk(R.Send(arr(lo, sel) + lo.plane, cnt, dt, cfg.rank - 1, comm, stream), "ncclSend(lo)");
                R.chk(R.Recv(arr(lo, sel), cnt, dt, cfg.rank - 1, comm, stream), "ncclRecv(lo)");
            }
            if (cfg.rank < cfg.world - 1) {
                R.chk(R.Send(arr(hi, sel) + (size_t)hi.nzl * hi.plane, cnt, dt, cfg.rank + 1, comm, stream), "ncclSend(hi)");
                R.chk(R.Recv(arr(hi, sel) + (size_t)(hi.nzl + 1) * hi.plane, cnt, dt, cfg.rank + 1, comm, stream), "ncclRecv(hi)");
            }
            R.chk(R.GroupEnd(), "ncclGroupEnd");
        }
    }

    struct StencilLaunch {
        dim3 grid, block;
        int xchunks, yblocks, zc;
    };
    StencilLaunch stencil_dims(const Slab<T>& sl) const {
        const int per_row = (n + vec - 1) / vec;
        int tx = 1;
        while (tx < per_row && tx < kBlock) tx <<= 1;
        const int tyb = kBlock / tx;
        const int xchunks = (per_row + tx - 1) / tx;
        const int yblocks = (n + tyb * kStRY - 1) / (tyb * kStRY);
        int zc = 16;
        while (zc > 4 && (long long)xchunks * yblocks * ((sl.nzl + zc - 1) / zc) < 1024) zc >>= 1;
        const int zchunks = (sl.nzl + zc - 1) / zc;
        return {dim3((unsigned)(xchunks * yblocks * zchunks)), dim3((unsigned)tx, (unsigned)tyb), xchunks, yblocks, zc};
    }

    void launch_stencil(Slab<T>& sl) {
        const StencilLaunch L = stencil_dims(sl);
        if (vec == 1)
            hipLaunchKernelGGL((stencil_dot_kernel<T, 1>), L.grid, L.block, 0, stream, sl.gp, L.xchunks, L.yblocks, L.zc, sl.p.p, sl.q.p, sl.partials.p);
        else
            hipLaunchKernelGGL((stencil_dot_kernel<T, vec_width<T>()>), L.grid, L.block, 0, stream, sl.gp, L.xchunks, L.yblocks, L.zc, sl.p.p, sl.q.p, sl.partials.p);
    }

    template <int VEC> void launch_update_xr(Slab<T>& sl, int rho_slot, int grid) {
        hipLaunchKernelGGL((update_xr_kernel<T, VEC>), dim3(grid), dim3(kBlock), 0, stream, sl.nown / VEC, sl.plane, sl.sc.p, rho_slot, sl.pq.p,
                           sl.x.p, sl.p.p, sl.r.p, sl.q.p, sl.partials.p);
    }
    template <int VEC> void launch_update_p(Slab<T>& sl, int rho_old, int rho_new, int init, int use_uw, const T* zsrc, int grid) {
        hipLaunchKernelGGL((update_p_kernel<T, VEC>), dim3(grid), dim3(kBlock), 0, stream, sl.nown / VEC, sl.plane, sl.sc.p, rho_old, rho_new,
                           sl.red.p, init, use_uw, zsrc, sl.p.p);
    }
    void update_p_all(int rho_old, int rho_new, int init, bool pre, const std::vector<int>& nparts) {
        for (size_t s = 0; s < slabs.size(); s++) {
            const T* zsrc = pre ? slabs[s].z.p : slabs[s].r.p;
            if (vec == 1) launch_update_p<1>(slabs[s], rho_old, rho_new, init, pre ? 0 : 1, zsrc, nparts[s]);
            else launch_update_p<vec_width<T>()>(slabs[s], rho_old, rho_new, init, pre ? 0 : 1, zsrc, nparts[s]);
        }
    }
    template <int VEC> void launch_norm2(Slab<T>& sl, const T* v, int grid) {
        hipLaunchKernelGGL((norm2_kernel<T, VEC>), dim3(grid), dim3(kBlock), 0, stream, sl.nown / VEC, sl.plane, v, sl.partials.p);
    }

    struct FusedCfg {
        int wx = 0, ry = 8, zc = 16, yblocks = 0, zchunks = 0, nw = 8, part = 0;
    };
    bool fused_available() const {
        static const bool off = knob("SHM_CG_CLASSIC") != nullptr;
        return !off && (n + vec - 1) / vec <= 8 * 64;
    }
    FusedCfg fused_cfg(const Slab<T>& sl) const {
        FusedCfg c;
        const int lanes = (n + vec - 1) / vec;
        c.wx = 1;
        while (c.wx * 64 < lanes) c.wx <<= 1;
        static const int nw_env = knob("SHM_FUSED_WAVES") ? atoi(knob("SHM_FUSED_WAVES")) : 0;
        c.ry = (vec == 1) ? 4 : 2;
        c.nw = (c.ry <= 2 && (nw_env == 16 || (nw_env == 0 && c.wx >= 4))) ? 16 : 8;
        const int wy = c.nw / c.wx;
        static const int zc_env = knob("SHM_FUSED_ZC") ? atoi(knob("SHM_FUSED_ZC")) : 0;
        c.yblocks = (n + wy * c.ry - 1) / (wy * c.ry);
        const int want = std::max(1, (2 * num_cus + c.yblocks - 1) / c.yblocks);
        c.zc = std::min(64, std::max(8, sl.nzl / want));
        if (zc_env > 0) c.zc = zc_env;
        c.zc = std::max(1, std::min(c.zc, sl.nzl));
        c.zchunks = (sl.nzl + c.zc - 1) / c.zc;
        while ((size_t)c.yblocks * c.zchunks > sl.partials.count && c.zc < sl.nzl) {
            c.zc = std::min(sl.nzl, 2 * c.zc);
            c.zchunks = (sl.nzl + c.zc - 1) / c.zc;
        }
        return c;
    }
    enum FusedPart { FUSED_ALL = 0, FUSED_INTERIOR = 1, FUSED_BOUNDARY = 2 };
    template <int MODE, int VEC, int RY, int WX>
    void launch_fused_k(Slab<T>& sl, const FusedCfg& cc, int slot_old, int slot_new, int init, int use_uw, int alpha_slot, const T* zsrc, const T* pin, T* pout) {
        FusedCfg c = cc;
        FusedParams F;
        F.n = n; F.nzl = sl.nzl; F.k0 = sl.k0; F.zc = c.zc; F.yblocks = c.yblocks; F.inv_h2 = sl.gp.inv_h2;
        F.zc_first = 0; F.zc_stride = 1;
        const bool dir_to_own = fold_pq && MODE == CGF_DIR;
        const int pq_np = (fold_pq && MODE == CGF_RES) ? fold_pq_np : 0;
        if (fold_pq && !sl.pq_partials.p) sl.pq_partials.alloc(sl.partials.count);
        if (c.part == FUSED_INTERIOR) { F.zc_first = 1; c.zchunks -= 2; }
        else if (c.part == FUSED_BOUNDARY) { F.zc_stride = c.zchunks - 1; c.zchunks = 2; }
        if constexpr (RY <= 2) {
            if (c.nw == 16) {
                hipLaunchKernelGGL((cg_fused_kernel<T, VEC, RY, WX, 16 / WX, MODE>), dim3((unsigned)(c.yblocks * c.zchunks)), dim3(1024), 0, stream, F, sl.sc.p, slot_old,
                                   slot_new, sl.red.p, sl.pq.p, init, use_uw, alpha_slot, zsrc, pin, pout, sl.r.p, dir_to_own ? sl.pq_partials.p : sl.partials.p, sl.pq_partials.p, pq_np);
                return;
            }
        }
        hipLaunchKernelGGL((cg_fused_kernel<T, VEC, RY, WX, 8 / WX, MODE>), dim3((unsigned)(c.yblocks * c.zchunks)), dim3(512), 0, stream, F, sl.sc.p, slot_old,
                           slot_new, sl.red.p, sl.pq.p, init, use_uw, alpha_slot, zsrc, pin, pout, sl.r.p, dir_to_own ? sl.pq_partials.p : sl.partials.p, sl.pq_partials.p, pq_np);
    }
    template <int MODE, int VEC, int RY>
    void launch_fused_w(Slab<T>& sl, const FusedCfg& c, int slot_old, int slot_new, int init, int use_uw, int alpha_slot, const T* zsrc, const T* pin, T* pout) {
        switch (c.wx) {
            case 1: launch_fused_k<MODE, VEC, RY, 1>(sl, c, slot_old, slot_new, init, use_uw, alpha_slot, zsrc, pin, pout); break;
            case 2: launch_fused_k<MODE, VEC, RY, 2>(sl, c, slot_old, slot_new, init, use_uw, alpha_slot, zsrc, pin, pout); break;
            case 4: launch_fused_k<MODE, VEC, RY, 4>(sl, c, slot_old, slot_new, init, use_uw, alpha_slot, zsrc, pin, pout); break;
            default: launch_fused_k<MODE, VEC, RY, 8>(sl, c, slot_old, slot_new, init, use_uw, alpha_slot, zsrc, pin, pout); break;
        }
    }
    template <int MODE>
    int launch_fused(Slab<T>& sl, int slot_old, int slot_new, int init, int use_uw, int alpha_slot, const T* zsrc, const T* pin, T* pout, int part = FUSED_ALL) {
        FusedCfg c = fused_cfg(sl);
        c.part = part;
        if (vec == 1) launch_fused_w<MODE, 1, 4>(sl, c, slot_old, slot_new, init, use_uw, alpha_slot, zsrc, pin, pout);
        else launch_fused_w<MODE, vec_width<T>(), 2>(sl, c, slot_old, slot_new, init, use_uw, alpha_slot, zsrc, pin, pout);
        return c.yblocks * c.zchunks;
    }
    void launch_x_update2(Slab<T>& sl, int use_a, int use_b, hipStream_t st = nullptr, int half = -1) {
        if (!st) st = stream;
        const size_t nall = sl.nown / vec, nlow = nall / 2;
        const size_t v0 = half == 1 ? nlow : 0, nvec = half < 0 ? nall : (half == 0 ? nlow : nall - nlow);
        if (nvec == 0) return;
        const size_t off = sl.plane + v0 * (size_t)vec;
        const unsigned g = (unsigned)((nvec + (size_t)kXuTiles * kBlock - 1) / ((size_t)kXuTiles * kBlock));
        if (vec == 1)
            hipLaunchKernelGGL((cg_x_update2_kernel<T, 1>), dim3(g), dim3(kBlock), 0, st, nvec, off, sl.sc.p, use_a, use_b, sl.p.p, sl.q.p, sl.x.p);
        else
            hipLaunchKernelGGL((cg_x_update2_kernel<T, vec_width<T>()>), dim3(g), dim3(kBlock), 0, st, nvec, off, sl.sc.p, use_a, use_b, sl.p.p, sl.q.p,
                               sl.x.p);
    }

    int stream_grid(const Slab<T>& sl) const { return grid_for(sl.nown / vec, 2048); }

    void launch_projection(const std::vector<int>& nparts, bool on_z = false, int save_rr = 0, hipStream_t st = nullptr) {
        hipStream_t stream = st ? st : this->stream;
        for (size_t s = 0; s < slabs.size(); s++) {
            Slab<T>& sl = slabs[s];
            hipLaunchKernelGGL((gather_rows_kernel<T>), dim3(1 + (8 * m + kBlock - 1) / kBlock), dim3(kBlock), 0, stream, m, sl.row_ptr.p, sl.ent_node.p,
                               sl.ent_coef.p, on_z ? sl.z.p : sl.r.p, sl.partials.p, nparts[s], sl.red.p);
        }
        if (!st) allreduce(0, 1 + m);
        for (Slab<T>& sl : slabs) {
            apply_Ginv(sl.red.p + 1, sl.u.p, false, stream);
            const int nred = std::max(1, std::min(16, m / 1024));
            if (!sl.proj_ticket.p) {
                sl.proj_ticket.alloc(1);
                HIPCHK(hipMemsetAsync(sl.proj_ticket.p, 0, sizeof(unsigned), stream));
            }
            hipLaunchKernelGGL((scatter_nodes_kernel<T>), dim3(nred + (sl.n_touched + kBlock - 1) / kBlock), dim3(kBlock), 0, stream, sl.n_touched,
                               sl.node_id.p, sl.node_ptr.p, sl.ent_row.p, sl.nent_coef.p, sl.u.p, sl.red.p + 1, m, sl.sc.p, save_rr,
                               on_z ? sl.z.p : sl.r.p, nred, sl.partials.p, sl.proj_ticket.p);
        }
    }

    bool fft_available() const {
        if (n < 16 || n > 1024 || (n & (n - 1)) != 0) return false;
        if (total_slabs == 1) return true;
        return slabs_equal && (total_slabs & (total_slabs - 1)) == 0 && n % total_slabs == 0;
    }
    bool gemm_dct() const { return !fft_available() && total_slabs == 1 && n >= 4 && n <= 1024; }
    bool precond_available() const { return fft_available() || gemm_dct(); }
    void setup_precond() {
        if (precond_ready) return;
        log2n = 0;
        while ((1 << log2n) < n) log2n++;
        std::vector<Cplx<TP>> tw(n), om(n);
        std::vector<TP> lam(n);
        const double pi = 3.14159265358979323846;
        for (int k = 0; k < n; k++) {
            tw[k] = {(TP)std::cos(-2. * pi * k / n), (TP)std::sin(-2. * pi * k / n)};
            om[k] = {(TP)std::cos(-pi * k / (2. * n)), (TP)std::sin(-pi * k / (2. * n))};
            lam[k] = (TP)((2. - 2. * std::cos(pi * k / n)) / (cell * cell));
        }
        d_tw.upload(tw, stream);
        d_om.upload(om, stream);
        d_lam.upload(lam, stream);
        std::vector<double> lam64(n);
        for (int k = 0; k < n; k++) lam64[k] = (2. - 2. * std::cos(pi * k / n)) / (cell * cell);
        d_lam64.upload(lam64, stream);
        for (Slab<T>& sl : slabs) {
            if (!gemm_dct()) sl.W1.alloc(sl.nown);
            if (total_slabs > 1) sl.W2.alloc(sl.nown);
            sl.z.alloc(sl.ntot);
            HIPCHK(hipMemsetAsync(sl.z.p, 0, sl.ntot * sizeof(T), stream));
        }
        if (gemm_dct()) {
            std::vector<double> ctab(4 * (size_t)n);
            for (int r = 0; r < 4 * n; r++) ctab[(size_t)r] = std::cos(pi * r / (2. * n));
            DevArray<double> d_ctab;
            d_ctab.upload(ctab, stream);
            gd_Cm.alloc((size_t)n * n);
            gd_Ct.alloc((size_t)n * n);
            gd_W1.alloc((size_t)n * n * n);
            gd_W2.alloc((size_t)n * n * n);
            hipLaunchKernelGGL(dct_matrix_kernel, dim3(grid_for((size_t)n * n, 1024)), dim3(kBlock), 0, stream, n, d_ctab.p, gd_Cm.p, gd_Ct.p);
            HIPCHK(hipGetLastError());
            HIPCHK(hipStreamSynchronize(stream));
        }
        HIPCHK(hipStreamSynchronize(stream));
        precond_ready = true;
    }

    void launch_dgemm(hipStream_t st, bool narrow, int prio, unsigned batches, int M, int N, int K, const double* A, int lda, long long sA, const double* B, int ldb,
                      long long sB, double* C, int ldc, long long sC) {
        auto tiles = [](size_t v) { return (unsigned)((v + kGemmT - 1) / kGemmT); };
        if (narrow)
            hipLaunchKernelGGL(dgemm_rm_kernel<1>, dim3((unsigned)((N + 31) / 32), tiles((size_t)M), batches), dim3(kBlock), 0, st, M, N, K, A, lda, sA, B, ldb, sB, C, ldc, sC, prio);
        else
            hipLaunchKernelGGL(dgemm_rm_kernel<4>, dim3(tiles((size_t)N), tiles((size_t)M), batches), dim3(kBlock), 0, st, M, N, K, A, lda, sA, B, ldb, sB, C, ldc, sC, prio);
    }

    int launch_precond_gemm(bool dot, int in_sel, int out_sel) {
        Slab<T>& sl = slabs[0];
        const size_t N3 = (size_t)n * n * n;
        const int nn = n, n2 = n * n;
        double *W1 = gd_W1.p, *W2 = gd_W2.p;
        const double* X;
        double* Z;
        if constexpr (sizeof(T) == 8) {
            X = reinterpret_cast<const double*>(arr(sl, in_sel)) + sl.plane;
            Z = reinterpret_cast<double*>(arr(sl, out_sel)) + sl.plane;
        } else {
            hipLaunchKernelGGL((convert_kernel<T, double>), dim3(grid_for(N3, 4096)), dim3(kBlock), 0, stream, N3, arr(sl, in_sel) + sl.plane, W2);
            X = W2;
            Z = W2;
        }
        auto gemm = [&](unsigned batches, int M, int Nc, int K, const double* A, int lda, long long sA, const double* B, int ldb, long long sB, double* C, int ldc, long long sC) {
            launch_dgemm(stream, false, 0, batches, M, Nc, K, A, lda, sA, B, ldb, sB, C, ldc, sC);
        };
        gemm(1, n2, nn, nn, X, nn, 0LL, gd_Ct.p, nn, 0LL, W1, nn, 0LL);
        gemm((unsigned)n, nn, nn, nn, gd_Cm.p, nn, 0LL, W1, nn, (long long)n2, W2, nn, (long long)n2);
        gemm(1, nn, n2, nn, gd_Cm.p, nn, 0LL, W2, n2, 0LL, W1, n2, 0LL);
        hipLaunchKernelGGL(spectral_scale_kernel, dim3(grid_for(N3, 4096)), dim3(kBlock), 0, stream, n, d_lam64.p, W1);
        gemm(1, nn, n2, nn, gd_Ct.p, nn, 0LL, W1, n2, 0LL, W2, n2, 0LL);
        gemm((unsigned)n, nn, nn, nn, gd_Ct.p, nn, 0LL, W2, nn, (long long)n2, W1, nn, (long long)n2);
        gemm(1, n2, nn, nn, W1, nn, 0LL, gd_Cm.p, nn, 0LL, Z, nn, 0LL);
        if constexpr (sizeof(T) != 8) hipLaunchKernelGGL((convert_kernel<double, T>), dim3(grid_for(N3, 4096)), dim3(kBlock), 0, stream, N3, W2, arr(sl, out_sel) + sl.plane);
        int np = 0;
        if (dot) {
            np = grid_for(N3, 2048);
            hipLaunchKernelGGL((dot_partial_kernel<T>), dim3(np), dim3(kBlock), 0, stream, N3, arr(sl, in_sel) + sl.plane, arr(sl, out_sel) + sl.plane, sl.partials.p);
        }
        return np;
    }

    template <int MODE, typename TIn, typename TOut, bool DOT, int LOG2N, bool XPASS>
    void launch_dct_n(const DctParams& P, int ntiles, const TIn* in, TOut* out, const TOut* dotw, double* partials, const int* tile_list, const unsigned* elem_mask) {
        constexpr bool kCanSeg = !XPASS && MODE != DCT_FUSED && !DOT;
        const bool seg = P.in.seg_shift < 30 || P.out.seg_shift < 30;
        if (seg && !kCanSeg) throw Error(SHM_ERR_INVALID, "DCT: segmented layout in a sweep that does not support it");
        if constexpr (kCanSeg) {
            if (seg) {
                launch_dct_pf<MODE, TIn, TOut, DOT, LOG2N, XPASS, true, false>(P, ntiles, in, out, dotw, partials, tile_list, elem_mask);
                return;
            }
        }
        launch_dct_pf<MODE, TIn, TOut, DOT, LOG2N, XPASS, false, false>(P, ntiles, in, out, dotw, partials, tile_list, elem_mask);
    }
    template <int MODE, typename TIn, typename TOut, bool DOT, int LOG2N, bool XPASS, bool SEG, bool PF>
    void launch_dct_pf(const DctParams& P, int ntiles, const TIn* in, TOut* out, const TOut* dotw, double* partials, const int* tile_list, const unsigned* elem_mask) {
        static uint64_t configured = 0;
        constexpr size_t lds = dct_lds_bytes<LOG2N, (int)sizeof(TP)>() + (PF ? dct_stage_bytes<LOG2N, (int)sizeof(TP)>() : 0);
        const uint64_t dev_bit = 1ull << (cfg.device & 63);
        if (!(configured & dev_bit) || cfg.device >= 64) {
            HIPCHK(hipFuncSetAttribute(reinterpret_cast<const void*>(&dct_lines_kernel<TP, TIn, TOut, MODE, DOT, LOG2N, XPASS, SEG, PF>), hipFuncAttributeMaxDynamicSharedMemorySize, (int)lds));
            configured |= dev_bit;
        }
        DctParams Q = P;
        Q.ntiles = ntiles;
        Q.debug_skip = 0;
        hipLaunchKernelGGL((dct_lines_kernel<TP, TIn, TOut, MODE, DOT, LOG2N, XPASS, SEG, PF>), dim3((unsigned)ntiles), dim3(kBlock), lds, stream, Q, in, out, d_tw.p, d_om.p, d_lam.p, dotw,
                           partials, tile_list, elem_mask);
    }
    template <int MODE, typename TIn, typename TOut, bool DOT, bool XPASS>
    void launch_dct(const DctParams& P, int ntiles, const TIn* in, TOut* out, const TOut* dotw, double* partials, const int* tile_list = nullptr,
                    const unsigned* elem_mask = nullptr) {
        switch (log2n) {
            case 4: launch_dct_n<MODE, TIn, TOut, DOT, 4, XPASS>(P, ntiles, in, out, dotw, partials, tile_list, elem_mask); break;
            case 5: launch_dct_n<MODE, TIn, TOut, DOT, 5, XPASS>(P, ntiles, in, out, dotw, partials, tile_list, elem_mask); break;
            case 6: launch_dct_n<MODE, TIn, TOut, DOT, 6, XPASS>(P, ntiles, in, out, dotw, partials, tile_list, elem_mask); break;
            case 7: launch_dct_n<MODE, TIn, TOut, DOT, 7, XPASS>(P, ntiles, in, out, dotw, partials, tile_list, elem_mask); break;
            case 8: launch_dct_n<MODE, TIn, TOut, DOT, 8, XPASS>(P, ntiles, in, out, dotw, partials, tile_list, elem_mask); break;
            case 9: launch_dct_n<MODE, TIn, TOut, DOT, 9, XPASS>(P, ntiles, in, out, dotw, partials, tile_list, elem_mask); break;
            case 10: launch_dct_n<MODE, TIn, TOut, DOT, 10, XPASS>(P, ntiles, in, out, dotw, partials, tile_list, elem_mask); break;
            default: throw Error(SHM_ERR_INVALID, "DCT preconditioner: unsupported grid size");
        }
    }

    static DctAddr plain_addr(long long off, long long a_stride, long long b_stride, long long line_stride, long long elem_stride) {
        DctAddr A{};
        A.off = off; A.a_stride = a_stride; A.b_stride = b_stride; A.line_stride = line_stride; A.elem_stride = elem_stride;
        A.seg_stride = 0; A.seg_shift = 30; A.seg_mask = (1 << 30) - 1;
        return A;
    }

    void alltoall_blocks(bool w1_to_w2, size_t blk) {
        auto srcp = [&](Slab<T>& sl) { return w1_to_w2 ? sl.W1.p : sl.W2.p; };
        auto dstp = [&](Slab<T>& sl) { return w1_to_w2 ? sl.W2.p : sl.W1.p; };
        const int ls = cfg.local_slabs;
        for (int a = 0; a < ls; a++)
            for (int b = 0; b < ls; b++)
                HIPCHK(hipMemcpyAsync(dstp(slabs[b]) + (size_t)(first_slab + a) * blk, srcp(slabs[a]) + (size_t)(first_slab + b) * blk, blk * sizeof(T),
                                      hipMemcpyDeviceToDevice, stream));
        if (comm) {
            Rccl& R = Rccl::get();
            const int dt = sizeof(T) == 8 ? Rccl::kFloat64 : Rccl::kFloat32;
            R.chk(R.GroupStart(), "ncclGroupStart");
            for (int peer = 0; peer < cfg.world; peer++) {
                if (peer == cfg.rank) continue;
                for (int a = 0; a < ls; a++)
                    for (int b = 0; b < ls; b++)
                        R.chk(R.Send(srcp(slabs[a]) + (size_t)(peer * ls + b) * blk, blk, dt, peer, comm, stream), "ncclSend(a2a)");
                for (int b = 0; b < ls; b++)
                    for (int a = 0; a < ls; a++)
                        R.chk(R.Recv(dstp(slabs[a]) + (size_t)(peer * ls + b) * blk, blk, dt, peer, comm, stream), "ncclRecv(a2a)");
            }
            R.chk(R.GroupEnd(), "ncclGroupEnd");
        }
    }

    enum ArrSel { ARR_R = 0, ARR_Z = 1, ARR_P = 2, ARR_X = 3, ARR_Q = 4, ARR_Y0 = 5, ARR_Y1 = 6, ARR_Y2 = 7 };
    static T* arr(Slab<T>& sl, int sel) {
        switch (sel) {
            case ARR_R: return sl.r.p;
            case ARR_Z: return sl.z.p;
            case ARR_P: return sl.p.p;
            case ARR_X: return sl.x.p;
            case ARR_Y0: return sl.Y0.p;
            case ARR_Y1: return sl.Y1.p;
            case ARR_Y2: return sl.Y2.p;
            default: return sl.q.p;
        }
    }
    int launch_precond(bool dot, int in_sel = ARR_R, int out_sel = ARR_Z, double scale = 1.0 ) {
        if (gemm_dct()) {
            if (scale != 1.0) throw Error(SHM_ERR_INVALID, "launch_precond: no scale on the dense-product transforms");
            return launch_precond_gemm(dot, in_sel, out_sel);
        }
        const long long nn = n, plane = (long long)n * n;
        const int P = total_slabs;
        const int nzl = n / P, nyl = n / P;
        const double inv8 = scale * 8.0 / ((double)n * n * n);
        const int kDctLines = dct_lines_for(log2n, (int)sizeof(TP));
        const int tiles_slab = (int)((long long)nzl * nn / kDctLines);
        int log2nyl = 0;
        while ((1 << log2nyl) < nyl) log2nyl++;
        const long long blk = (long long)nzl * nyl * nn;
        for (int pass = 0; pass < 7; pass++) {
            if (P == 1 && (pass == 2 || pass == 4)) continue;
            if (pass == 2) { alltoall_blocks(false, (size_t)blk); continue; }
            if (pass == 4) { alltoall_blocks(true, (size_t)blk); continue; }
            for (size_t si = 0; si < slabs.size(); si++) {
                Slab<T>& sl = slabs[si];
                const int g = first_slab + (int)si;
                DctParams Q{};
                Q.inv_n3_8 = inv8;
                Q.ky0 = 0;
                switch (pass) {
                    case 0:
                        Q.tiles_a = tiles_slab;
                        Q.in = plain_addr((long long)sl.plane, (long long)kDctLines * nn, 0, nn, 1);
                        Q.out = plain_addr(0, (long long)kDctLines * nn, 0, nn, 1);
                        launch_dct<DCT_FWD, T, TP, false, true>(Q, tiles_slab, arr(sl, in_sel), sl.W1.p, (const TP*)nullptr, nullptr);
                        break;
                    case 1:
                        Q.tiles_a = n / kDctLines;
                        Q.in = plain_addr(0, kDctLines, plane, 1, nn);
                        if (P == 1) {
                            Q.out = Q.in;
                            launch_dct<DCT_FWD, TP, TP, false, false>(Q, tiles_slab, sl.W1.p, sl.W1.p, (const TP*)nullptr, nullptr);
                        } else {
                            Q.out = plain_addr(0, kDctLines, (long long)nyl * nn, 1, nn);
                            Q.out.seg_shift = log2nyl; Q.out.seg_mask = nyl - 1; Q.out.seg_stride = blk;
                            launch_dct<DCT_FWD, TP, TP, false, false>(Q, tiles_slab, sl.W1.p, sl.W2.p, (const TP*)nullptr, nullptr);
                        }
                        break;
                    case 3: {
                        Q.tiles_a = n / kDctLines;
                        Q.in = plain_addr(0, kDctLines, nn, 1, (long long)nyl * nn);
                        Q.out = Q.in;
                        Q.ky0 = g * nyl;
                        const int tiles_z = (n / kDctLines) * nyl;
                        launch_dct<DCT_FUSED, TP, TP, false, false>(Q, tiles_z, sl.W1.p, sl.W1.p, (const TP*)nullptr, nullptr);
                        break;
                    }
                    case 5:
                        Q.tiles_a = n / kDctLines;
                        Q.out = plain_addr(0, kDctLines, plane, 1, nn);
                        if (P == 1) {
                            Q.in = Q.out;
                            launch_dct<DCT_INV, TP, TP, false, false>(Q, tiles_slab, sl.W1.p, sl.W1.p, (const TP*)nullptr, nullptr);
                        } else {
                            Q.in = plain_addr(0, kDctLines, (long long)nyl * nn, 1, nn);
                            Q.in.seg_shift = log2nyl; Q.in.seg_mask = nyl - 1; Q.in.seg_stride = blk;
                            launch_dct<DCT_INV, TP, TP, false, false>(Q, tiles_slab, sl.W2.p, sl.W1.p, (const TP*)nullptr, nullptr);
                        }
                        break;
                    case 6:
                        Q.tiles_a = tiles_slab;
                        Q.in = plain_addr(0, (long long)kDctLines * nn, 0, nn, 1);
                        Q.out = plain_addr((long long)sl.plane, (long long)kDctLines * nn, 0, nn, 1);
                        if (dot) launch_dct<DCT_INV, TP, T, true, true>(Q, tiles_slab, sl.W1.p, arr(sl, out_sel), arr(sl, in_sel), sl.partials.p);
                        else launch_dct<DCT_INV, TP, T, false, true>(Q, tiles_slab, sl.W1.p, arr(sl, out_sel), (const T*)nullptr, nullptr);
                        break;
                    default: break;
                }
            }
        }
        return dot ? tiles_slab : 0;
    }

    struct SolveClock {
        Event e_start, e_conv, e_div;
        Event e_s2a, e_s2b;
        Event e_setup;
        std::chrono::steady_clock::time_point wall0 = std::chrono::steady_clock::now();
        bool has_step1 = true;
        bool has_setup = true;
    };
    void fill_phase_stats(shm_stats* st, SolveClock& c, Event& e_pcg, Event& e_end, int iters, double rel_residual) {
        const auto wall1 = std::chrono::steady_clock::now();
        memset(st, 0, sizeof *st);
        st->n = n;
        st->S = S;
        st->iters = iters;
        st->rel_residual = rel_residual;
        st->shift = h_pinned[SC_SHIFT];
        if (c.has_step1) {
            st->ms_conv = elapsed(c.e_start, c.e_conv);
            st->ms_div = elapsed(c.e_conv, c.e_div);
        }
        if (c.has_setup) {
            st->m = m;
            HIPCHK(hipEventSynchronize(c.e_s2b.e));
            st->ms_setup = last_setup_wall_ms;
            if (c.has_step1) st->ms_wait_setup = elapsed(c.e_div, c.e_setup);
        }
        st->ms_pcg = elapsed(c.has_setup ? c.e_setup : c.e_div, e_pcg);
        st->ms_shift = elapsed(e_pcg, e_end);
        st->ms_total = std::chrono::duration<double, std::milli>(wall1 - c.wall0).count();
    }
    struct Residual {
        double rr0 = 0., rr = 0.;
        bool finite = true;
        double rel() const { return rr0 > 0. ? std::sqrt(std::fabs(rr / rr0)) : 0.; }
        bool below(double tol) const { return rr <= tol * tol * rr0; }
    };
    Residual fetch_residual(int extra_slot = -1 ) {
        HIPCHK(hipMemcpyAsync(h_pinned, slabs[0].sc.p, SC_COUNT * sizeof(double), hipMemcpyDeviceToHost, stream));
        HIPCHK(hipStreamSynchronize(stream));
        Residual r;
        r.rr0 = h_pinned[SC_RR0];
        r.rr = h_pinned[SC_RR];
        r.finite = std::isfinite(r.rr) && std::isfinite(r.rr0) && (extra_slot < 0 || std::isfinite(h_pinned[extra_slot]));
        return r;
    }
    void throw_loop_end(const char* name, bool breakdown, bool converged, int it, const Residual& r, const shm_opts& o) {
        if (breakdown) throw Error(SHM_ERR_BREAKDOWN, fmt("%s broke down at iteration %d (rr=%g, rr0=%g)", name, it, r.rr, r.rr0));
        if (!converged) throw Error(SHM_ERR_NOCONV, fmt("%s: max_iters=%d reached, rel. residual %.3e > tol %.1e", name, o.max_iters, r.rel(), o.tol));
    }
    struct SampleTimer {
        std::vector<std::unique_ptr<Event>> ev;
        const int max_samples, per;
        int n = 0;
        bool on = false;
        SampleTimer(bool enabled, int max_samples_, int events_per_sample) : max_samples(max_samples_), per(events_per_sample) {
            if (enabled) for (int a = 0; a < per * max_samples; a++) ev.emplace_back(new Event());
        }
        bool begin(bool wanted = true) { return on = !ev.empty() && n < max_samples && wanted; }
        void mark(int k, hipStream_t st) { if (on) ev[(size_t)(per * n + k)]->record(st); }
        void end() { if (on) n++; on = false; }
        double avg(int i, int j) const {
            double a = 0.;
            for (int q = 0; q < n; q++) a += elapsed(*ev[(size_t)(per * q + i)], *ev[(size_t)(per * q + j)]);
            return n ? a / n : 0.;
        }
    };
    void primal_prologue(bool pre, std::vector<int>& nparts, std::vector<int>& zparts) {
        for (size_t s = 0; s < slabs.size(); s++) {
            Slab<T>& sl = slabs[s];
            HIPCHK(hipMemsetAsync(sl.x.p, 0, sl.ntot * sizeof(T), stream));
            nparts[s] = stream_grid(sl);
            if (vec == 1) launch_norm2<1>(sl, sl.r.p, nparts[s]);
            else launch_norm2<vec_width<T>()>(sl, sl.r.p, nparts[s]);
        }
        launch_projection(nparts, false, 2);
        if (pre) {
            const int np = launch_precond(true);
            for (auto& v : zparts) v = np;
            launch_projection(zparts, true, 0);
        }
    }

    void launch_shift_and_phi() {
        for (Slab<T>& sl : slabs) {
            const int g = std::max(1, std::min(256, (sl.n_shift + kBlock - 1) / kBlock));
            hipLaunchKernelGGL((shift_partial_kernel<T>), dim3(g), dim3(kBlock), 0, stream, sl.n_shift, sl.shift_items.p, n, sl.x.p, sl.partials.p);
            hipLaunchKernelGGL(finalize_sum_kernel, dim3(1), dim3(kBlock), 0, stream, sl.partials.p, g, sl.pq.p);
        }
        allreduce(1, 1);
        for (Slab<T>& sl : slabs)
            hipLaunchKernelGGL((write_phi_kernel<T>), dim3(grid_for(sl.nown, 4096)), dim3(kBlock), 0, stream, sl.nown, sl.plane, sl.x.p, sl.pq.p, area_sum,
                               sl.sc.p, sl.q.p);
        HIPCHK(hipGetLastError());
    }

    void solve_fast(const shm_opts& o, shm_stats* st, SolveClock& clk) {
        (void)o;
        Event e_int, e_end;
        build_shift_items_only();
        Rccl* R = comm ? &Rccl::get() : nullptr;
        const int dt = sizeof(T) == 8 ? Rccl::kFloat64 : Rccl::kFloat32;
        for (size_t si = 0; si < slabs.size(); si++) {
            Slab<T>& sl = slabs[si];
            if (sl.k0 == 0) {
                hipLaunchKernelGGL((bfs_plane0_kernel<T>), dim3(1), dim3(std::min(1024, ((n + 63) / 64) * 64)), 0, stream, n, cell, bbox_min[0], bbox_min[1],
                                   sl.Y0.p, sl.Y1.p, sl.Y2.p, sl.x.p);
            } else if (si == 0) {
                R->chk(R->Recv(sl.x.p, sl.plane, dt, cfg.rank - 1, comm, stream), "ncclRecv(bfs)");
            }
            hipLaunchKernelGGL((bfs_z_kernel<T>), dim3((unsigned)((sl.plane + kBlock - 1) / kBlock)), dim3(kBlock), 0, stream, sl.gp, cell, bbox_min[2], sl.Y0.p,
                               sl.Y1.p, sl.Y2.p, sl.x.p);
            const T* top = sl.x.p + (size_t)sl.nzl * sl.plane;
            if (si + 1 < slabs.size()) HIPCHK(hipMemcpyAsync(slabs[si + 1].x.p, top, sl.plane * sizeof(T), hipMemcpyDeviceToDevice, stream));
            else if (comm && cfg.rank < cfg.world - 1) R->chk(R->Send(top, sl.plane, dt, cfg.rank + 1, comm, stream), "ncclSend(bfs)");
        }
        HIPCHK(hipGetLastError());
        e_int.record(stream);
        launch_shift_and_phi();
        e_end.record(stream);
        fetch_residual();
        have_phi = true;
        if (st) {
            fill_phase_stats(st, clk, e_int, e_end, 0, 0.);
            st->preconditioner = SHM_PRECOND_NONE;
        }
    }

    void build_active_tiles(const std::vector<int64_t>& touched_nodes) {
        Slab<T>& sl = slabs[0];
        const int L = dct_lines_for(log2n_of(n), (int)sizeof(TP));
        const ActiveTiles at = active_tiles(touched_nodes, n, L);
        sl.act_z.upload(at.zmask, stream2);
        sl.n_act_planes = (int)at.planes.size();
        sl.act_planes.upload(at.planes, stream2);
        sl.n_act_x = (int)at.ax.size();
        sl.n_act_y = (int)at.ay.size();
        sl.act_x.upload(at.ax, stream2);
        sl.act_y.upload(at.ay, stream2);
        sl.S1.alloc(sl.nown);
        sl.S2.alloc(sl.nown);
        sl.S4.alloc(sl.nown);
        sl.W1.alloc(sl.nown);
        HIPCHK(hipMemsetAsync(sl.S1.p, 0, sl.nown * sizeof(T), stream2));
        HIPCHK(hipStreamSynchronize(stream2));
    }
    static int log2n_of(int v) {
        int l = 0;
        while ((1 << l) < v) l++;
        return l;
    }
    void launch_precond_sparse(int in_sel, int out_sel) {
        Slab<T>& sl = slabs[0];
        const long long nn = n, plane = (long long)n * n;
        const int L = dct_lines_for(log2n, (int)sizeof(TP));
        const int tiles_all = (int)(plane * nn / L / nn);
        DctParams Q{};
        Q.inv_n3_8 = 8.0 / ((double)n * n * n);
        Q.ky0 = 0;
        Q.tiles_a = tiles_all;
        Q.in = plain_addr((long long)sl.plane, (long long)L * nn, 0, nn, 1);
        Q.out = plain_addr(0, (long long)L * nn, 0, nn, 1);
        launch_dct<DCT_FWD, T, TP, false, true>(Q, sl.n_act_x, arr(sl, in_sel), sl.S1.p, (const TP*)nullptr, nullptr, sl.act_x.p);
        Q.tiles_a = n / L;
        Q.in = plain_addr(0, L, plane, 1, nn);
        Q.out = Q.in;
        launch_dct<DCT_FWD, TP, TP, false, false>(Q, sl.n_act_y, sl.S1.p, sl.S2.p, (const TP*)nullptr, nullptr, sl.act_y.p);
        Q.in = plain_addr(0, L, nn, 1, plane);
        Q.out = Q.in;
        if (n < 256) launch_dct<DCT_FUSED, TP, TP, false, false>(Q, tiles_all, sl.S2.p, sl.W1.p, (const TP*)nullptr, nullptr, nullptr, sl.act_z.p);
        else {
            hipLaunchKernelGGL((zsolve_sparse_kernel<TP>), dim3((unsigned)((plane + kBlock - 1) / kBlock) + 1), dim3(kBlock), 0, stream, n, sl.n_act_planes,
                               sl.act_planes.p, d_lam64.p, sl.gp.inv_h2, sl.S2.p, sl.W1.p);
        }
        Q.in = plain_addr(0, L, plane, 1, nn);
        Q.out = Q.in;
        launch_dct<DCT_INV, TP, TP, false, false>(Q, sl.n_act_y, sl.W1.p, sl.S4.p, (const TP*)nullptr, nullptr, sl.act_y.p);
        Q.tiles_a = tiles_all;
        Q.in = plain_addr(0, (long long)L * nn, 0, nn, 1);
        Q.out = plain_addr((long long)sl.plane, (long long)L * nn, 0, nn, 1);
        launch_dct<DCT_INV, TP, T, false, true>(Q, sl.n_act_x, sl.S4.p, arr(sl, out_sel), (const T*)nullptr, nullptr, sl.act_x.p);
    }

    void solve_dual(const shm_opts& o, shm_stats* st, SolveClock& clk) {
        Event e_pcg, e_end;
        const int check_every = o.check_every > 0 ? std::min(o.check_every, 4) : 2;
        auto mv = [&](Slab<T>& sl, int k) { return sl.dv.p + (size_t)k * mp; };
        enum { V_MU = 0, V_R = 1, V_P = 2, V_Z = 3, V_T1 = 4, V_T2 = 5, V_G = 6 };
        const std::vector<int> nopart(slabs.size(), 0);
        auto gather = [&](int sel) {
            for (Slab<T>& sl : slabs)
                hipLaunchKernelGGL((gather_rows_kernel<T>), dim3(1 + (8 * m + kBlock - 1) / kBlock), dim3(kBlock), 0, stream, m, sl.row_ptr.p, sl.ent_node.p,
                                   sl.ent_coef.p, arr(sl, sel), sl.partials.p, 0, sl.red.p);
            allreduce(0, 1 + m);
        };
        auto scatter = [&](int vec, int sel, int accumulate, double scale = 1.0, bool save = false) {
            for (Slab<T>& sl : slabs)
                hipLaunchKernelGGL((scatter_rows_to_nodes_kernel<T>), dim3((sl.n_touched + kBlock - 1) / kBlock + 1), dim3(kBlock), 0, stream, sl.n_touched,
                                   sl.node_id.p, sl.node_ptr.p, sl.ent_row.p, sl.nent_coef.p, mv(sl, vec), accumulate, arr(sl, sel), scale, save ? sl.touched_save.p : (T*)nullptr);
        };
        auto precondition = [&](int init) {
            for (Slab<T>& sl : slabs) {
                apply_Ginv(mv(sl, V_R), mv(sl, V_T1), true, stream);
                hipLaunchKernelGGL(csr_matvec_kernel, dim3((m + kBlock - 1) / kBlock), dim3(kBlock), 0, stream, m, Bptr.p, Bcol.p, Bval.p, mv(sl, V_T1), mv(sl, V_T2));
                apply_Ginv(mv(sl, V_T2), mv(sl, V_Z), true, stream);
                hipLaunchKernelGGL(dual_direction_kernel, dim3(1), dim3(kDualBlock), 0, stream, m, init, mv(sl, V_R), mv(sl, V_Z), mv(sl, V_P), sl.sc.p);
            }
        };
        launch_precond(false, ARR_R, ARR_Z);
        gather(ARR_Z);
        for (Slab<T>& sl : slabs) {
            HIPCHK(hipMemcpyAsync(mv(sl, V_G), sl.red.p + 1, (size_t)m * sizeof(double), hipMemcpyDeviceToDevice, stream));
            if (sl.div_sum_blocks > 0) {
                hipLaunchKernelGGL(finalize_sum_kernel, dim3(1), dim3(kBlock), 0, stream, sl.div_partials.p, sl.div_sum_blocks, sl.pq.p);
                continue;
            }
            const int g = grid_for(sl.nown, 1024);
            hipLaunchKernelGGL((sum_kernel<T>), dim3(g), dim3(kBlock), 0, stream, sl.nown, sl.plane, sl.r.p, sl.partials.p);
            hipLaunchKernelGGL(finalize_sum_kernel, dim3(1), dim3(kBlock), 0, stream, sl.partials.p, g, sl.pq.p);
        }
        allreduce(1, 1);
        for (Slab<T>& sl : slabs) {
            hipLaunchKernelGGL(dual_init_mu_kernel, dim3(1), dim3(kDualBlock), 0, stream, m, sl.pq.p, mv(sl, V_MU), sl.sc.p);
        }
        const bool sparse_ok = total_slabs == 1 && slabs[0].n_act_x > 0;
        const bool dense_S = have_S;
        if (!dense_S)
            for (Slab<T>& sl : slabs) HIPCHK(hipMemsetAsync(sl.p.p, 0, sl.ntot * sizeof(T), stream));
        auto apply_S = [&](int vec) {
            for (Slab<T>& sl : slabs) launch_ginv_matvec<double>(stream, m, m, mp, Sdense.p, mv(sl, vec), sl.red.p + 1);
        };
        if (dense_S) apply_S(V_MU);
        else {
            scatter(V_MU, ARR_P, 0);
            if (sparse_ok) launch_precond_sparse(ARR_P, ARR_Z);
            else launch_precond(false, ARR_P, ARR_Z);
            gather(ARR_Z);
        }
        for (Slab<T>& sl : slabs)
            hipLaunchKernelGGL(dual_init_residual_kernel, dim3(1), dim3(kDualBlock), 0, stream, m, mv(sl, V_G), sl.red.p + 1, mv(sl, V_R), sl.sc.p, 1);
        const bool direct = plan.dual_form == SHM_DUAL_DIRECT && dense_S;
        if (!direct) precondition(1);
        HIPCHK(hipGetLastError());

        SampleTimer tm(st != nullptr, 32, 3);
        int it = 0;
        Residual res;
        bool converged = false, breakdown = false;
        auto finish = [&]() {
            if (gemm_dct()) {
                for (Slab<T>& sl : slabs)
                    hipLaunchKernelGGL((negate_kernel<T>), dim3(grid_for(sl.ntot, 4096)), dim3(kBlock), 0, stream, sl.ntot, sl.r.p, sl.q.p);
                scatter(V_MU, ARR_Q, 1);
                launch_precond(false, ARR_Q, ARR_X);
            } else {
                scatter(V_MU, ARR_R, 1, -1.0, true);
                launch_precond(false, ARR_R, ARR_X, -1.0);
                for (Slab<T>& sl : slabs)
                    hipLaunchKernelGGL((restore_nodes_kernel<T>), dim3((sl.n_touched + kBlock - 1) / kBlock + 1), dim3(kBlock), 0, stream, sl.n_touched, sl.node_id.p,
                                       sl.touched_save.p, sl.r.p);
            }
            gather(ARR_X);
            for (Slab<T>& sl : slabs) hipLaunchKernelGGL(finalize_sum_kernel, dim3(1), dim3(kBlock), 0, stream, sl.red.p + 1, m, sl.sc.p + SC_AXSUM);
            e_pcg.record(stream);
            launch_shift_and_phi();
            e_end.record(stream);
            return fetch_residual();
        };
        bool finished = false;
        if (direct) {
            auto apply_Sinv = [&](const double* w, double* u) { launch_ginv_matvec<double>(stream, m, m, mp, Sinv.p, w, u); };
            const int max_passes = std::min(o.max_iters, 6);
            double rr_prev = -1.;
            while (it < max_passes && !converged && !breakdown) {
                tm.begin();
                tm.mark(0, stream);
                for (Slab<T>& sl : slabs) {
                    apply_Sinv(mv(sl, V_R), mv(sl, V_T1));
                    hipLaunchKernelGGL(dual_bordered_kernel, dim3(1), dim3(kDualBlock), 0, stream, m, mv(sl, V_T1), Sinv_ones.p, (const double*)nullptr, 1, mv(sl, V_MU));
                }
                tm.mark(1, stream);
                apply_S(V_MU);
                for (Slab<T>& sl : slabs)
                    hipLaunchKernelGGL(dual_init_residual_kernel, dim3(1), dim3(kDualBlock), 0, stream, m, mv(sl, V_G), sl.red.p + 1, mv(sl, V_R), sl.sc.p, 0);
                tm.mark(2, stream);
                tm.end();
                it++;
                HIPCHK(hipGetLastError());
                res = finish();
                finished = true;
                if (!res.finite) breakdown = true;
                else if (res.below(o.tol)) converged = true;
                else if (rr_prev >= 0. && res.rr > 0.0625 * rr_prev && res.rr <= 1e-18 * res.rr0) converged = true;
                rr_prev = res.rr;
                log("[shm] dual (direct) pass=%d rel_res=%.3e", it, res.rel());
            }
        }
        while (!direct && it < o.max_iters && !converged && !breakdown) {
            const int batch_end = std::min(o.max_iters, it + check_every);
            for (; it < batch_end; it++) {
                tm.begin();
                if (!dense_S) scatter(V_P, ARR_P, 0);
                tm.mark(0, stream);
                if (dense_S) apply_S(V_P);
                else if (sparse_ok) launch_precond_sparse(ARR_P, ARR_Z);
                else launch_precond(false, ARR_P, ARR_Z);
                tm.mark(1, stream);
                if (!dense_S) gather(ARR_Z);
                for (Slab<T>& sl : slabs)
                    hipLaunchKernelGGL(dual_update_kernel, dim3(1), dim3(kDualBlock), 0, stream, m, sl.red.p + 1, mv(sl, V_P), mv(sl, V_MU), mv(sl, V_R), sl.sc.p);
                precondition(0);
                tm.mark(2, stream);
                tm.end();
            }
            HIPCHK(hipGetLastError());
            res = fetch_residual(SC_RZ);
            if (!res.finite) breakdown = true;
            else if (res.below(o.tol)) converged = true;
            log("[shm] dual it=%d rel_res=%.3e", it, res.rel());
        }
        if (!finished) finish();
        have_phi = true;
        have_div = false;
        if (st) {
            fill_phase_stats(st, clk, e_pcg, e_end, it, res.rel());
            st->shift += h_pinned[SC_AXSUM] / (double)m;
            st->ms_precond_avg = tm.avg(0, 1);
            st->ms_project_avg = tm.avg(1, 2);
            st->kernel_samples = tm.n;
            st->preconditioner = SHM_PRECOND_DCT;
            st->solver = total_slabs > 1 ? SHM_SOLVER_DUAL_SLABS : SHM_SOLVER_DUAL;
            if (direct) {
                st->bytes_per_iter = 2.0 * (double)m * m * sizeof(double);
                st->cg_form = 2;
            } else if (dense_S) {
                st->bytes_per_iter = (double)m * m * (sizeof(double) + 2.0 * sizeof(float));
                st->cg_form = 3;
            } else if (sparse_ok) {
                const double L = dct_lines_for(log2n, (int)sizeof(TP)), tile_bytes = L * n * sizeof(TP);
                const double planes_active = (double)slabs[0].n_act_y / (n / L);
                st->bytes_per_iter = 4.0 * slabs[0].n_act_x * tile_bytes + 4.0 * slabs[0].n_act_y * tile_bytes + 2.0 * planes_active * n * n * sizeof(TP);
            } else {
                st->bytes_per_iter = (double)N * (3.0 * sizeof(T) + 8.0 * sizeof(TP)) - (double)N * sizeof(T);
            }
        }
        throw_loop_end("dual CG", breakdown, converged, it, res, o);
    }

    void solve_gathered(const shm_opts& o, const PlanIn& in, shm_stats* st, SolveClock& clk) {
        Solver<T>& F = *full;
        Slab<T>& fs = F.slabs[0];
        Event e_gather;
        SolveClock fclk;
        fclk.wall0 = clk.wall0;
        fclk.has_step1 = false;
        fclk.e_s2a.record(F.stream2);
        PlanIn fin = in;
        fin.total_slabs = 1; fin.fft_available = F.fft_available(); fin.gemm_dct = F.gemm_dct();
        fin.step1 = in.tiered() ? kStep1TieredF64 : kStep1Untiered;
        Plan fplan;
        fplan.path = kPathGathered; fplan.dual_requested = true;
        F.build_constraints(fin, fplan);
        fclk.e_s2b.record(F.stream2);
        F.setup_precond();
        const size_t plane = (size_t)n * n;
        for (Slab<T>& sl : slabs)
            HIPCHK(hipMemcpyAsync(fs.r.p + (size_t)(sl.k0 + 1) * plane, sl.r.p + plane, sl.nown * sizeof(T), hipMemcpyDeviceToDevice, stream));
        if (comm) {
            Rccl& R = Rccl::get();
            const int dt = sizeof(T) == 8 ? Rccl::kFloat64 : Rccl::kFloat32;
            R.chk(R.GroupStart(), "ncclGroupStart");
            for (int peer = 0; peer < cfg.world; peer++) {
                if (peer == cfg.rank) continue;
                for (Slab<T>& sl : slabs) R.chk(R.Send(sl.r.p + plane, sl.nown, dt, peer, comm, stream), "ncclSend(gather b)");
                for (int b = 0; b < cfg.local_slabs; b++) {
                    int32_t k0, k1;
                    slab_range(peer * cfg.local_slabs + b, &k0, &k1);
                    R.chk(R.Recv(fs.r.p + (size_t)(k0 + 1) * plane, (size_t)(k1 - k0) * plane, dt, peer, comm, stream), "ncclRecv(gather b)");
                }
            }
            R.chk(R.GroupEnd(), "ncclGroupEnd");
        }
        e_gather.record(stream);
        HIPCHK(hipStreamWaitEvent(F.stream, e_gather.e, 0));
        fclk.e_start.record(F.stream);
        fclk.e_setup.record(F.stream);
        F.have_div = true;
        F.sum_b_in_div_order(fs, F.stream);
        shm_stats cst;
        memset(&cst, 0, sizeof cst);
        bool noconv = false;
        std::string noconv_msg;
        try {
            F.solve_dual(o, &cst, fclk);
        } catch (const Error& e) {
            if (e.code != SHM_ERR_NOCONV) throw;
            noconv = true;
            noconv_msg = e.what();
        }
        for (Slab<T>& sl : slabs)
            HIPCHK(hipMemcpyAsync(sl.q.p + plane, fs.q.p + (size_t)(sl.k0 + 1) * plane, sl.nown * sizeof(T), hipMemcpyDeviceToDevice, stream));
        HIPCHK(hipStreamSynchronize(stream));
        have_phi = true;
        if (st) {
            *st = cst;
            st->ms_conv = elapsed(clk.e_start, clk.e_conv);
            st->ms_div = elapsed(clk.e_conv, clk.e_div);
            st->ms_wait_setup = elapsed(clk.e_div, e_gather);
            st->ms_total = std::chrono::duration<double, std::milli>(std::chrono::steady_clock::now() - clk.wall0).count();
        }
        if (noconv) throw Error(SHM_ERR_NOCONV, noconv_msg);
    }

    void solve_primal_fused(const shm_opts& o, shm_stats* st, bool pre, SolveClock& clk) {
        std::vector<int> nparts(slabs.size()), zparts(slabs.size(), 0), kparts(slabs.size(), 0);
        fold_pq = total_slabs == 1 && !comm;
        fold_pq_np = 0;
        auto dirbuf = [&](Slab<T>& sl, int k) { return (k & 1) ? sl.q.p : sl.p.p; };
        const int zsel = pre ? ARR_Z : ARR_R;
        primal_prologue(pre, nparts, zparts);
        const bool halo_serial = comm != nullptr && knob("SHM_HALO_OVERLAP") == nullptr;
        bool overlap = total_slabs > 1 && !halo_serial;
        for (Slab<T>& sl : slabs) overlap = overlap && fused_cfg(sl).zchunks >= 3;
        if (overlap && !stream_h) HIPCHK(hipStreamCreateWithFlags(&stream_h, hipStreamNonBlocking));
        Event e_ready, e_halo;
        auto run_dir = [&](int k, int slot_old, int slot_new, int init) {
            auto sweep = [&](int part) {
                for (size_t s = 0; s < slabs.size(); s++) {
                    Slab<T>& sl = slabs[s];
                    const int out = init ? 0 : k + 1;
                    kparts[s] = launch_fused<CGF_DIR>(sl, slot_old, slot_new, init, pre ? 0 : 1, 0, arr(sl, zsel), dirbuf(sl, k), dirbuf(sl, out), part);
                }
            };
            if (!overlap) {
                if (total_slabs > 1) halo_exchange(zsel);
                sweep(FUSED_ALL);
                return;
            }
            e_ready.record(stream);
            HIPCHK(hipStreamWaitEvent(stream_h, e_ready.e, 0));
            sweep(FUSED_INTERIOR);
            halo_exchange(zsel, stream_h);
            e_halo.record(stream_h);
            HIPCHK(hipStreamWaitEvent(stream, e_halo.e, 0));
            sweep(FUSED_BOUNDARY);
        };
        auto finalize_pq = [&]() {
            if (fold_pq) {
                fold_pq_np = kparts[0];
                return;
            }
            for (size_t s = 0; s < slabs.size(); s++)
                hipLaunchKernelGGL(finalize_sum_kernel, dim3(1), dim3(kBlock), 0, stream, slabs[s].partials.p, kparts[s], slabs[s].pq.p);
            allreduce(1, 1);
        };
        run_dir(0, SC_RHO_A, SC_RHO_A, 1);
        finalize_pq();
        HIPCHK(hipGetLastError());

        SampleTimer tm(st != nullptr, 12, 8);
        const int sample_stride = pre ? 2 : 8;
        const bool xoverlap = total_slabs == 1 && !comm;
        const bool xsplit = xoverlap && !pre;
        Event e_xfork, e_xjoin;
        hipStream_t const stream_x = stream2;
        int it = 0;
        Residual res;
        bool converged = false, breakdown = false;
        while (it < o.max_iters && !converged && !breakdown) {
            const int batch_end = std::min(o.max_iters, it + o.check_every);
            for (; it < batch_end; it++) {
                const int slot_old = (it & 1) ? SC_RHO_B : SC_RHO_A, slot_new = (it & 1) ? SC_RHO_A : SC_RHO_B;
                const bool sample = tm.begin(it % sample_stride == 1);
                auto mark = [&](int k) { tm.mark(k, stream); };
                mark(0);
                for (size_t s = 0; s < slabs.size(); s++)
                    nparts[s] = launch_fused<CGF_RES>(slabs[s], slot_old, slot_new, 0, 0, (it & 1) ? SC_ALPHA_B : SC_ALPHA_A, (const T*)nullptr,
                                                      dirbuf(slabs[s], it), (T*)nullptr);
                mark(1);
                const bool fork_x = xoverlap && ((it & 1) || xsplit) && !sample && !pre;
                if (fork_x) {
                    e_xfork.record(stream);
                    HIPCHK(hipStreamWaitEvent(stream_x, e_xfork.e, 0));
                    launch_projection(nparts, false, 1, stream_x);
                    e_xjoin.record(stream_x);
                    if (xsplit) launch_x_update2(slabs[0], 1, it > 0, nullptr, it & 1);
                    else launch_x_update2(slabs[0], 1, 1);
                    HIPCHK(hipStreamWaitEvent(stream, e_xjoin.e, 0));
                } else {
                    launch_projection(nparts, false, 1);
                }
                mark(2);
                if (pre) launch_precond(true);
                mark(3);
                if (pre) launch_projection(zparts, true, 0);
                mark(4);
                if (!fork_x && xsplit) launch_x_update2(slabs[0], 1, it > 0, nullptr, it & 1);
                else if (!fork_x && (it & 1))
                    for (Slab<T>& sl : slabs) launch_x_update2(sl, 1, 1);
                mark(5);
                run_dir(it, slot_old, slot_new, 0);
                mark(6);
                finalize_pq();
                mark(7);
                tm.end();
            }
            HIPCHK(hipGetLastError());
            res = fetch_residual((it & 1) ? SC_RHO_B : SC_RHO_A);
            if (!res.finite) breakdown = true;
            else if (res.below(o.tol)) converged = true;
            log("[shm] it=%d rel_res=%.3e", it, res.rel());
        }
        if (xsplit) {
            if (it & 1) launch_x_update2(slabs[0], 1, 0, nullptr, 1);
            else if (it > 0) launch_x_update2(slabs[0], 0, 1, nullptr, 0);
        } else if (it & 1)
            for (Slab<T>& sl : slabs) launch_x_update2(sl, 1, 0);
        const PrimalLoop loop = {xsplit ? 4 : 1, 8.0, {5, 6}, {0, 1}, {{1, 2}, {3, 4}}, {4, 5}, {2, 3}};
        finish_primal(o, st, pre, clk, tm, it, res, converged, breakdown, loop);
    }
    struct PrimalLoop {
        int cg_form;
        double sweep_nt;
        int stencil[2], update_xr[2], project[2][2], update_p[2], precond[2];
    };
    void finish_primal(const shm_opts& o, shm_stats* st, bool pre, SolveClock& clk, SampleTimer& tm, int it, const Residual& res, bool converged, bool breakdown,
                       const PrimalLoop& loop) {
        Event e_pcg, e_end;
        e_pcg.record(stream);
        launch_shift_and_phi();
        e_end.record(stream);
        fetch_residual();
        have_phi = true;
        have_div = false;
        if (st) {
            fill_phase_stats(st, clk, e_pcg, e_end, it, res.rel());
            auto avg = [&](const int (&ij)[2]) { return tm.avg(ij[0], ij[1]); };
            st->ms_stencil_avg = avg(loop.stencil);
            st->ms_update_xr_avg = avg(loop.update_xr);
            st->ms_project_avg = avg(loop.project[0]) + avg(loop.project[1]);
            st->ms_update_p_avg = avg(loop.update_p);
            st->ms_precond_avg = pre ? avg(loop.precond) : 0.;
            st->kernel_samples = tm.n;
            st->preconditioner = pre ? SHM_PRECOND_DCT : SHM_PRECOND_NONE;
            st->solver = SHM_SOLVER_PRIMAL;
            st->cg_form = loop.cg_form;
            st->bytes_per_iter = loop.sweep_nt * (double)N * sizeof(T) + (pre ? (double)N * (3.0 * sizeof(T) + 8.0 * sizeof(TP)) : 0.);
        }
        throw_loop_end("projected CG", breakdown, converged, it, res, o);
    }

    void solve_primal_classic(const shm_opts& o, shm_stats* st, bool pre, SolveClock& clk) {
        std::vector<int> nparts(slabs.size()), zparts(slabs.size(), 0);
        primal_prologue(pre, nparts, zparts);
        update_p_all(SC_RHO_A, SC_RHO_A, 1, pre, nparts);
        HIPCHK(hipGetLastError());

        SampleTimer tm(st != nullptr, 32, 8);
        const int sample_stride = pre ? 2 : 8;
        int it = 0;
        Residual res;
        bool converged = false, breakdown = false;
        while (it < o.max_iters && !converged && !breakdown) {
            const int batch_end = std::min(o.max_iters, it + o.check_every);
            for (; it < batch_end; it++) {
                const int slot_old = (it & 1) ? SC_RHO_B : SC_RHO_A, slot_new = (it & 1) ? SC_RHO_A : SC_RHO_B;
                halo_exchange_p();
                tm.begin(it % sample_stride == 1);
                auto mark = [&](int k) { tm.mark(k, stream); };
                mark(0);
                for (Slab<T>& sl : slabs) launch_stencil(sl);
                mark(1);
                for (Slab<T>& sl : slabs) {
                    const StencilLaunch L = stencil_dims(sl);
                    hipLaunchKernelGGL(finalize_sum_kernel, dim3(1), dim3(kBlock), 0, stream, sl.partials.p, (int)L.grid.x, sl.pq.p);
                }
                allreduce(1, 1);
                mark(2);
                for (size_t s = 0; s < slabs.size(); s++) {
                    if (vec == 1) launch_update_xr<1>(slabs[s], slot_old, nparts[s]);
                    else launch_update_xr<vec_width<T>()>(slabs[s], slot_old, nparts[s]);
                }
                mark(3);
                launch_projection(nparts, false, 1);
                mark(4);
                if (pre) launch_precond(true);
                mark(5);
                if (pre) launch_projection(zparts, true, 0);
                mark(6);
                update_p_all(slot_old, slot_new, 0, pre, nparts);
                mark(7);
                tm.end();
            }
            HIPCHK(hipGetLastError());
            res = fetch_residual((it & 1) ? SC_RHO_B : SC_RHO_A);
            if (!res.finite) breakdown = true;
            else if (res.below(o.tol)) converged = true;
            log("[shm] it=%d rel_res=%.3e", it, res.rel());
        }
        const PrimalLoop loop = {0, 11.0, {0, 1}, {2, 3}, {{3, 4}, {5, 6}}, {6, 7}, {4, 5}};
        finish_primal(o, st, pre, clk, tm, it, res, converged, breakdown, loop);
    }

    void report_pairs(shm_stats* st) noexcept {
        if (!st || !d_pair_counters.p) return;
        unsigned long long h[3] = {0, 0, 0};
        if (hipMemcpy(h, d_pair_counters.p, sizeof h, hipMemcpyDeviceToHost) != hipSuccess) return;
        st->pairs_fp64 = (double)h[0];
        st->pairs_fp32 = (double)h[1];
        st->pairs_redone = (double)h[2];
        st->conv_launches = conv_launches_last;
    }
    void solve(const shm_opts& o_in, shm_stats* st) override {
        struct Fin {
            Solver* s;
            shm_stats* st;
            ~Fin() { s->report_pairs(st); }
        } fin{this, st};
        solve_impl(o_in, st);
    }
    void solve_impl(const shm_opts& o_in, shm_stats* st) {
        need_problem();
        HIPCHK(hipSetDevice(cfg.device));
        shm_opts o = o_in;
        PlanIn in = plan_inputs(&o);
        const Plan p = plan_solve(in);
        if (p.status != SHM_OK) throw Error(p.status, p.error);
        iso_idx_valid = false;
        ray_bricks_valid = false;
        redist_valid = false;
        const bool pre = p.precond;
        if (!(o.tol > 0.)) o.tol = sizeof(T) == 8 ? 1e-8 : 1e-5;
        if (o.max_iters <= 0) o.max_iters = 20 * n;
        if (o.check_every <= 0) o.check_every = pre ? 4 : 32;

        SolveClock clk;
        step1_budget = o.step1_budget;
        select_step1_arith(o.step1_arith);
        clk.e_start.record(stream);
        for (Slab<T>& sl : slabs)
            if (sl.proj_ticket.p) HIPCHK(hipMemsetAsync(sl.proj_ticket.p, 0, sizeof(unsigned), stream));
        o_fast_hint = o.fast_integration != 0;
        launch_conv();
        clk.e_conv.record(stream);
        launch_div(o.scrub_nonfinite);
        clk.e_div.record(stream);
        if (p.path == kPathFast) {
            log("[shm] plan: fast");
            clk.has_setup = false;
            solve_fast(o, st, clk);
            return;
        }
        in.step1 = step1_kernel();
        in.conv_est_total_ms = conv_est_total_ms;
        if (p.path == kPathGathered) {
            ensure_full();
            solve_gathered(o, in, st, clk);
            return;
        }
        static const bool setup_alone = knob("SHM_SETUP_ALONE") != nullptr;
        if (setup_alone) HIPCHK(hipStreamSynchronize(stream));
        clk.e_s2a.record(stream2);
        build_constraints(in, p);
        clk.e_s2b.record(stream2);
        const bool dual = p.path == kPathDualSlabs || p.path == kPathDualLocal;
        if (pre || dual) setup_precond();
        clk.e_setup.record(stream);
        if (dual) solve_dual(o, st, clk);
        else if (p.path == kPathPrimalFused) solve_primal_fused(o, st, pre, clk);
        else solve_primal_classic(o, st, pre, clk);
    }
    void copy_planes_to_host(int which, int ka, int kb, double* out) {
        size_t off = 0;
        for (Slab<T>& sl : slabs) {
            const int a = std::max(ka, sl.k0), b = std::min(kb, sl.k1);
            if (b <= a) continue;
            const T* srcp = nullptr;
            switch (which) {
                case SHM_FIELD_Y0: srcp = sl.Y0.p; break;
                case SHM_FIELD_Y1: srcp = sl.Y1.p; break;
                case SHM_FIELD_Y2: srcp = sl.Y2.p; break;
                case SHM_FIELD_DIV: srcp = sl.r.p; break;
                default: srcp = sl.q.p; break;
            }
            srcp += sl.plane * (size_t)(a - sl.k0 + 1);
            const size_t cnt = sl.plane * (size_t)(b - a);
            if (sizeof(T) == 8) {
                HIPCHK(hipMemcpyAsync(out + off, srcp, cnt * sizeof(double), hipMemcpyDeviceToHost, stream));
            } else {
                DevArray<double> tmp;
                tmp.alloc(cnt);
                hipLaunchKernelGGL((convert_kernel<T, double>), dim3(grid_for(cnt, 4096)), dim3(kBlock), 0, stream, cnt, srcp, tmp.p);
                HIPCHK(hipMemcpyAsync(out + off, tmp.p, cnt * sizeof(double), hipMemcpyDeviceToHost, stream));
                HIPCHK(hipStreamSynchronize(stream));
            }
            off += cnt;
        }
        HIPCHK(hipStreamSynchronize(stream));
    }
    void copy_owned_to_host(int which, double* out) {
        size_t off = 0;
        for (Slab<T>& sl : slabs) {
            const T* srcp = nullptr;
            switch (which) {
                case SHM_FIELD_Y0: srcp = sl.Y0.p; break;
                case SHM_FIELD_Y1: srcp = sl.Y1.p; break;
                case SHM_FIELD_Y2: srcp = sl.Y2.p; break;
                case SHM_FIELD_DIV: srcp = sl.r.p; break;
                default: srcp = sl.q.p; break;
            }
            srcp += sl.plane;
            if (sizeof(T) == 8) {
                HIPCHK(hipMemcpyAsync(out + off, srcp, sl.nown * sizeof(double), hipMemcpyDeviceToHost, stream));
            } else {
                DevArray<double> tmp;
                tmp.alloc(sl.nown);
                hipLaunchKernelGGL((convert_kernel<T, double>), dim3(grid_for(sl.nown, 4096)), dim3(kBlock), 0, stream, sl.nown, srcp, tmp.p);
                HIPCHK(hipMemcpyAsync(out + off, tmp.p, sl.nown * sizeof(double), hipMemcpyDeviceToHost, stream));
                HIPCHK(hipStreamSynchronize(stream));
            }
            off += sl.nown;
        }
        HIPCHK(hipStreamSynchronize(stream));
    }

    void owned_planes(int32_t* kb, int32_t* ke) override {
        need_problem();
        if (kb) *kb = slabs.front().k0;
        if (ke) *ke = slabs.back().k1;
    }
    void get_phi(double* out, int32_t* kb, int32_t* ke) override {
        need_problem();
        if (!have_phi) throw Error(SHM_ERR_STATE, "no phi: shm_grid_solve has not completed");
        HIPCHK(hipSetDevice(cfg.device));
        copy_owned_to_host(SHM_FIELD_PHI, out);
        if (kb) *kb = slabs.front().k0;
        if (ke) *ke = slabs.back().k1;
    }

    void get_field(shm_field f, double* out) override {
        need_problem();
        HIPCHK(hipSetDevice(cfg.device));
        if ((f == SHM_FIELD_Y0 || f == SHM_FIELD_Y1 || f == SHM_FIELD_Y2) && !have_conv) throw Error(SHM_ERR_STATE, "Y not computed");
        if (f == SHM_FIELD_DIV && !have_div) throw Error(SHM_ERR_STATE, "divergence not computed");
        if (f == SHM_FIELD_PHI && !have_phi) throw Error(SHM_ERR_STATE, "phi not computed");
        copy_owned_to_host((int)f, out);
    }

    void get_field_planes(shm_field f, int ka, int kb, double* out) override {
        need_problem();
        HIPCHK(hipSetDevice(cfg.device));
        if ((f == SHM_FIELD_Y0 || f == SHM_FIELD_Y1 || f == SHM_FIELD_Y2) && !have_conv) throw Error(SHM_ERR_STATE, "Y not computed");
        if (f == SHM_FIELD_DIV && !have_div) throw Error(SHM_ERR_STATE, "divergence not computed");
        if (f == SHM_FIELD_PHI && !have_phi) throw Error(SHM_ERR_STATE, "phi not computed");
        if (ka < slabs.front().k0 || kb > slabs.back().k1 || kb < ka) throw Error(SHM_ERR_INVALID, "plane range outside the planes this process owns");
        copy_planes_to_host((int)f, ka, kb, out);
    }

    void upload_owned(const double* in, int which) {
        std::vector<T> tmp;
        for (Slab<T>& sl : slabs) {
            tmp.assign(sl.ntot, (T)0);
            const int klo = std::max(0, sl.k0 - 1), khi = std::min(n, sl.k1 + 1);
            for (int k = klo; k < khi; k++)
                for (size_t a = 0; a < sl.plane; a++) tmp[(size_t)(k - sl.k0 + 1) * sl.plane + a] = (T)in[(size_t)k * sl.plane + a];
            T* dst = which == 0 ? sl.p.p : sl.r.p;
            HIPCHK(hipMemcpyAsync(dst, tmp.data(), sl.ntot * sizeof(T), hipMemcpyHostToDevice, stream));
            HIPCHK(hipStreamSynchronize(stream));
        }
    }

    void apply_laplacian(const double* u, double* out) override {
        need_problem();
        if (cfg.world != 1) throw Error(SHM_ERR_INVALID, "apply_laplacian is a single-process test entry point");
        HIPCHK(hipSetDevice(cfg.device));
        upload_owned(u, 0);
        for (Slab<T>& sl : slabs)
            hipLaunchKernelGGL((laplacian_kernel<T>), dim3(grid_for(sl.nown, 4096)), dim3(kBlock), 0, stream, sl.gp, sl.p.p, sl.q.p);
        HIPCHK(hipGetLastError());
        copy_owned_to_host(SHM_FIELD_PHI, out);
        have_phi = false;
        iso_idx_valid = false;
        ray_bricks_valid = false;
        redist_valid = false;
    }

    void get_constraints(int64_t* nodes, double* coeffs, int32_t* m_out) override {
        need_problem();
        build_rows();
        for (int r = 0; r < m; r++)
            for (int e = 0; e < 8; e++) {
                nodes[8 * (size_t)r + e] = rows[r].nodes[e];
                coeffs[8 * (size_t)r + e] = rows[r].coeffs[e];
            }
// ... 933 lines not shown
```

Before: 692.4 million.

## Pool events, consolidate control counters, and overlap dual solve tail on side stream

Replaces per-solve event creation with a persistent event pool, and merges the scattered small device counters (pair counters, unit counters, sample counters, projection tickets) into one control buffer that a single memset clears. The dual solve tail gets a fused start kernel and a two-block finalize kernel, runs the S·mu residual check on a second stream joined by an event, and queues the pair-counter copy asynchronously with the final residual fetch instead of a blocking memcpy afterward. The aim is to cut host-side launch, allocation and synchronisation overhead in the end-to-end solve. It adds stream fork/join complexity and host timing instrumentation.

```diff
diff --git a/signed-heat-3d_amd/csrc/shm_kernels.hip.h b/signed-heat-3d_amd/csrc/shm_kernels.hip.h
--- a/signed-heat-3d_amd/csrc/shm_kernels.hip.h
+++ b/signed-heat-3d_amd/csrc/shm_kernels.hip.h
@@ -760,6 +760,7 @@
                                                              const double* __restrict__ partials, int np, double* __restrict__ red) {
     __shared__ double lds[8];
     if (blockIdx.x == 0) {
+        if (np < 0) return;
         double s = 0.;
         for (int a = threadIdx.x; a < np; a += kBlock) s += partials[a];
         s = block_sum(s, lds);
@@ -1018,6 +1019,57 @@
         sc[SC_RR] = rr;
         if (set_rr0) sc[SC_RR0] = rr;
     }
+}
+
+static __global__ __launch_bounds__(kDualBlock) void dual_start_kernel(int m, const double* __restrict__ b_partials, int np, const double* __restrict__ g,
+                                                                const double* __restrict__ S_ones, double* __restrict__ mu, double* __restrict__ r,
+                                                                double* __restrict__ sc) {
+    __shared__ double lds[17];
+    __shared__ double sumb_s;
+    {
+        double s = 0.;
+        if (threadIdx.x < kBlock)
+            for (int a = threadIdx.x; a < np; a += kBlock) s += b_partials[a];
+        s = wave_sum(s);
+        if (threadIdx.x < kBlock && (threadIdx.x & 63) == 0) lds[threadIdx.x >> 6] = s;
+        __syncthreads();
+        if (threadIdx.x == 0) {
+            double t = 0.;
+            for (int a = 0; a < kBlock / kWave; a++) t += lds[a];
+            sumb_s = t;
+            sc[SC_SUMB] = t;
+        }
+        __syncthreads();
+    }
+    const double v = sumb_s / (double)m;
+    double s = 0.;
+    for (int a = threadIdx.x; a < m; a += kDualBlock) {
+        mu[a] = v;
+        s += g[a] - __dmul_rn(v, S_ones[a]);
+    }
+    const double mean = block_sum_1024(s, lds) / (double)m;
+    double rr = 0.;
+    for (int a = threadIdx.x; a < m; a += kDualBlock) {
+        const double w = g[a] - __dmul_rn(v, S_ones[a]) - mean;
+        r[a] = w;
+        rr += w * w;
+    }
+    rr = block_sum_1024(rr, lds);
+    if (threadIdx.x == 0) {
+        sc[SC_RR] = rr;
+        sc[SC_RR0] = rr;
+    }
+}
+
+static __global__ __launch_bounds__(kBlock) void finalize_sum2_kernel(const double* __restrict__ partials0, int np0, double* __restrict__ dst0,
+                                                               const double* __restrict__ partials1, int np1, double* __restrict__ dst1) {
+    __shared__ double red[8];
+    const double* __restrict__ partials = blockIdx.x ? partials1 : partials0;
+    const int np = blockIdx.x ? np1 : np0;
+    double s = 0.;
+    for (int a = threadIdx.x; a < np; a += kBlock) s += partials[a];
+    s = block_sum(s, red);
+    if (threadIdx.x == 0) *(blockIdx.x ? dst1 : dst0) = s;
 }
 
 static __global__ __launch_bounds__(kDualBlock) void dual_direction_kernel(int m, int init, const double* __restrict__ r, double* __restrict__ z,
diff --git a/signed-heat-3d_amd/csrc/shm_solver.hip.h b/signed-heat-3d_amd/csrc/shm_solver.hip.h
--- a/signed-heat-3d_amd/csrc/shm_solver.hip.h
+++ b/signed-heat-3d_amd/csrc/shm_solver.hip.h
@@ -21,13 +21,17 @@
 
 template <typename T> constexpr int vec_width() { return sizeof(T) == 8 ? 2 : 4; }
 
+template <typename U> struct CtrlView {
+    U* p = nullptr;
+};
+
 template <typename T>
 struct Slab {
     int k0 = 0, k1 = 0, nzl = 0;
     size_t plane = 0, nown = 0, ntot = 0;
     DevArray<T> Y0, Y1, Y2, r , x, p, q , z ;
     DevArray<double> partials, pq_partials , red , pq , u , sc;
-    DevArray<unsigned> proj_ticket;
+    CtrlView<unsigned> proj_ticket;
     DevArray<int> row_ptr, ent_row, node_ptr;
     DevArray<uint32_t> ent_node, node_id;
     DevArray<double> ent_coef, nent_coef;
@@ -36,7 +40,7 @@
     DevArray<int> layer_order;
     DevArray<int> sample_order;
     DevArray<unsigned char> sample_rule;
-    DevArray<unsigned long long> sample_ctr;
+    CtrlView<unsigned long long> sample_ctr;
     long long sample_key = -1;
     int sample_blocks = 0;
     long long layer_order_key = -1;
@@ -61,6 +65,13 @@
     hipStream_t stream2 = nullptr;
     hipStream_t stream3 = nullptr;
     std::unique_ptr<Event> e_sch_in, e_sch_done, e_gs_done;
+    enum { EV_START, EV_CONV, EV_DIV, EV_S2A, EV_S2B, EV_SETUP, EV_PCG, EV_END, EV_FORK, EV_JOIN, EV_AUX0, EV_AUX1, EV_AUX2, EV_AUX3, EV_SLAB0, EV_SLAB1, EV_TIMER0 };
+    std::vector<std::unique_ptr<Event>> ev_pool;
+    Event& ev(int slot) {
+        if ((size_t)slot >= ev_pool.size()) ev_pool.resize((size_t)slot + 1);
+        if (!ev_pool[(size_t)slot]) ev_pool[(size_t)slot].reset(new Event());
+        return *ev_pool[(size_t)slot];
+    }
     hipStream_t stream_h = nullptr;
     int n = 0, alloc_n = -1;
     size_t N = 0;
@@ -87,8 +98,15 @@
     bool fold_pq = false;
     int fold_pq_np = 0;
     double step1_budget = 0.;
-    DevArray<unsigned long long> d_pair_counters;
-    DevArray<unsigned> d_unit_counters;
+    DevArray<unsigned long long> ctrl;
+    unsigned long long* h_pairs = nullptr;
+    double host_us[4] = {0., 0., 0., 0.};
+    using HostClock = std::chrono::steady_clock;
+    static double us_since(HostClock::time_point t0) { return std::chrono::duration<double, std::micro>(HostClock::now() - t0).count(); }
+    bool pairs_fetched = false;
+    bool pairs_queued = false;
+    CtrlView<unsigned long long> d_pair_counters;
+    CtrlView<unsigned> d_unit_counters;
     static constexpr int kMaxConvLaunches = 256;
     int conv_launch_index = 0;
     int conv_launches_last = 0;
@@ -182,6 +200,7 @@
             HIPCHK(hipStreamCreateWithPriority(&stream2, hipStreamNonBlocking, greatest));
         }
         HIPCHK(hipHostMalloc((void**)&h_pinned, 64 * sizeof(double)));
+        HIPCHK(hipHostMalloc((void**)&h_pairs, 4 * sizeof(unsigned long long)));
         if (cfg.world > 1 && !cfg.rccl_unique_id) throw Error(SHM_ERR_INVALID, "world>1 needs rccl_unique_id");
         if (cfg.rccl_unique_id) {
             Rccl& R = Rccl::get();
@@ -201,6 +220,8 @@
         for (void* b : ray_pinned)
             if (b) (void)hipHostFree(b);
         slabs.clear();
+        ev_pool.clear();
+        if (h_pairs) (void)hipHostFree(h_pairs);
         if (stream) (void)hipStreamDestroy(stream);
         if (stream2) (void)hipStreamDestroy(stream2);
         if (stream3) (void)hipStreamDestroy(stream3);
@@ -479,6 +500,7 @@
             sl.gp.inv_h = 1. / cell;
             sl.gp.inv_h2 = 1. / (cell * cell);
         }
+        bind_control();
         HIPCHK(hipStreamSynchronize(stream));
         precond_ready = false;
         have_problem = true;
@@ -624,19 +646,39 @@
             sl.sample_blocks = nA * ((n + kTierTX - 1) / kTierTX) * ((n + kTierTY - 1) / kTierTY);
             sl.sample_order.upload(order, stream);
             sl.sample_rule.upload(rule, stream);
-            sl.sample_ctr.alloc(4);
             sl.sample_key = key;
         }
         return true;
+    }
+    size_t control_words() const {
+        return (4 + 5 * slabs.size() + (size_t)8 * kMaxConvLaunches / 2 + 15) / 16 * 16;
+    }
+    void bind_control() {
+        const size_t L = slabs.size(), words = control_words();
+        if (ctrl.count < words || !ctrl.p) {
+            ctrl.alloc(words);
+            HIPCHK(hipMemsetAsync(ctrl.p, 0, ctrl.count * sizeof(unsigned long long), stream));
+        }
+        d_pair_counters.p = ctrl.p;
+        for (size_t s = 0; s < L; s++) {
+            slabs[s].sample_ctr.p = ctrl.p + 4 + 4 * s;
+            slabs[s].proj_ticket.p = reinterpret_cast<unsigned*>(ctrl.p + 4 + 4 * L + s);
+        }
+        d_unit_counters.p = reinterpret_cast<unsigned*>(ctrl.p + 4 + 5 * L);
+    }
+    void clear_control() {
+        HIPCHK(hipMemsetAsync(ctrl.p, 0, control_words() * sizeof(unsigned long long), stream));
+        pairs_fetched = pairs_queued = false;
     }
     void launch_conv() {
         const bool slab_log = knob("SHM_CONV_SLAB_LOG") != nullptr;
-        Event slab_ev[2];
+        const HostClock::time_point t_entry = HostClock::now();
+        Event* slab_ev[2] = {slab_log ? &ev(EV_SLAB0) : nullptr, slab_log ? &ev(EV_SLAB1) : nullptr};
         unsigned long long slab_pairs_seen[2] = {0, 0};
         for (Slab<T>& sl : slabs) {
             if (slab_log) {
                 HIPCHK(hipStreamSynchronize(stream));
-                slab_ev[0].record(stream);
+                slab_ev[0]->record(stream);
             }
             ConvParams P;
             P.layer_order = nullptr;
@@ -710,18 +752,15 @@
             const int want_chunks = (conv_tiered || conv_tiered32) ? 1 : (uniform_tiles && conv_est_total_ms >= 10. ? std::min(16, (int)std::lround(conv_est_total_ms / 2.5)) : 1);
             const int nchunks = std::max(1, std::min(tiles_z, want_chunks));
             const int chunk_planes = ((tiles_z + nchunks - 1) / nchunks) * tile_z;
-            if (!d_pair_counters.p) d_pair_counters.alloc(3);
-            if (!d_unit_counters.p) d_unit_counters.alloc(8 * kMaxConvLaunches);
             if (&sl == &slabs[0]) {
-                HIPCHK(hipMemsetAsync(d_pair_counters.p, 0, 3 * sizeof(unsigned long long), stream));
-                HIPCHK(hipMemsetAsync(d_unit_counters.p, 0, 8 * kMaxConvLaunches * sizeof(unsigned), stream));
+                clear_control();
                 conv_launch_index = 0;
                 conv_launches_last = 0;
             }
             unsigned long long* const cnt = d_pair_counters.p;
             auto launch_range = [&](int b0, int b1, int sel, int rule = -1, const int* order = nullptr, int order_layers = 0) {
                 if (b1 <= b0) return;
-                conv_launches_last++;
+                if (conv_launches_last++ == 0) host_us[1] = us_since(t_entry);
                 const int tz_sel = 4 * sel;
                 ConvParams Pc = P;
                 Pc.kk_begin = 1 + b0;
@@ -779,7 +818,6 @@
                 }
             } else if (far_rule_plan(sl, planes, npt4 ? 4 : 2)) {
                 const int npt = npt4 ? 4 : 2, layers = planes / npt;
-                HIPCHK(hipMemsetAsync(sl.sample_ctr.p, 0, 4 * sizeof(unsigned long long), stream));
                 P.unit_rule = sl.sample_rule.p;
                 P.sample_ctr = sl.sample_ctr.p;
                 P.sample_blocks = sl.sample_blocks;
@@ -789,11 +827,11 @@
                 for (int b0 = 0; b0 < planes; b0 += chunk_planes) launch_range(b0, std::min(planes, b0 + chunk_planes), sel0);
             }
             if (slab_log) {
-                slab_ev[1].record(stream);
+                slab_ev[1]->record(stream);
                 HIPCHK(hipStreamSynchronize(stream));
                 unsigned long long h[2] = {0, 0};
                 HIPCHK(hipMemcpy(h, d_pair_counters.p, sizeof h, hipMemcpyDeviceToHost));
-                fprintf(stderr, "[shm] step1 slab planes [%d,%d) ms %.3f pairs_fp64 %.6e pairs_fp32 %.6e\n", sl.k0, sl.k1, elapsed(slab_ev[0], slab_ev[1]),
+                fprintf(stderr, "[shm] step1 slab planes [%d,%d) ms %.3f pairs_fp64 %.6e pairs_fp32 %.6e\n", sl.k0, sl.k1, elapsed(*slab_ev[0], *slab_ev[1]),
                         (double)(h[0] - slab_pairs_seen[0]), (double)(h[1] - slab_pairs_seen[1]));
                 slab_pairs_seen[0] = h[0];
                 slab_pairs_seen[1] = h[1];
@@ -1323,9 +1361,10 @@
             HIPCHK(hipMemcpyAsync(Sinv.p, Sdense.p, (size_t)mp * mp * sizeof(double), hipMemcpyDeviceToDevice, st));
             if (mp > m) hipLaunchKernelGGL(set_diagonal_kernel, dim3((unsigned)((mp - m + kBlock - 1) / kBlock)), dim3(kBlock), 0, st, Sinv.p, mp, m, mp, 1.0);
             enqueue_gj_invert(Sinv.p, mp, true);
-            Sinv_ones.alloc((size_t)2 * mp);
+            Sinv_ones.alloc((size_t)3 * mp);
             hipLaunchKernelGGL(fill_kernel, dim3((unsigned)((m + kBlock - 1) / kBlock)), dim3(kBlock), 0, st, Sinv_ones.p + mp, m, 1.0);
             launch_ginv_matvec<double>(st, m, m, mp, Sinv.p, Sinv_ones.p + mp, Sinv_ones.p);
+            launch_ginv_matvec<double>(st, m, m, mp, Sdense.p, Sinv_ones.p + mp, Sinv_ones.p + 2 * (size_t)mp);
         } else {
             e_sch_done->record(st);
             HIPCHK(hipStreamWaitEvent(stream2, e_sch_done->e, 0));
@@ -1521,10 +1560,6 @@
         for (Slab<T>& sl : slabs) {
             apply_Ginv(sl.red.p + 1, sl.u.p, false, stream);
             const int nred = std::max(1, std::min(16, m / 1024));
-            if (!sl.proj_ticket.p) {
-                sl.proj_ticket.alloc(1);
-                HIPCHK(hipMemsetAsync(sl.proj_ticket.p, 0, sizeof(unsigned), stream));
-            }
             hipLaunchKernelGGL((scatter_nodes_kernel<T>), dim3(nred + (sl.n_touched + kBlock - 1) / kBlock), dim3(kBlock), 0, stream, sl.n_touched,
                                sl.node_id.p, sl.node_ptr.p, sl.ent_row.p, sl.nent_coef.p, sl.u.p, sl.red.p + 1, m, sl.sc.p, save_rr,
                                on_z ? sl.z.p : sl.r.p, nred, sl.partials.p, sl.proj_ticket.p);
@@ -1789,15 +1824,22 @@
     }
 
     struct SolveClock {
-        Event e_start, e_conv, e_div;
-        Event e_s2a, e_s2b;
-        Event e_setup;
+        Event &e_start, &e_conv, &e_div;
+        Event &e_s2a, &e_s2b;
+        Event& e_setup;
+        explicit SolveClock(Solver& s)
+            : e_start(s.ev(EV_START)), e_conv(s.ev(EV_CONV)), e_div(s.ev(EV_DIV)), e_s2a(s.ev(EV_S2A)), e_s2b(s.ev(EV_S2B)), e_setup(s.ev(EV_SETUP)) {}
         std::chrono::steady_clock::time_point wall0 = std::chrono::steady_clock::now();
         bool has_step1 = true;
         bool has_setup = true;
     };
     void fill_phase_stats(shm_stats* st, SolveClock& c, Event& e_pcg, Event& e_end, int iters, double rel_residual) {
         const auto wall1 = std::chrono::steady_clock::now();
+        struct Lap {
+            double& us;
+            HostClock::time_point t0 = HostClock::now();
+            ~Lap() { us = us_since(t0); }
+        } lap{host_us[2]};
         memset(st, 0, sizeof *st);
         st->n = n;
         st->S = S;
@@ -1824,9 +1866,19 @@
         double rel() const { return rr0 > 0. ? std::sqrt(std::fabs(rr / rr0)) : 0.; }
         bool below(double tol) const { return rr <= tol * tol * rr0; }
     };
-    Residual fetch_residual(int extra_slot = -1 ) {
+    void queue_pairs_copy(hipStream_t on) {
+        if (!d_pair_counters.p || pairs_fetched || pairs_queued || solve_only || knob("SHM_SOLVE_TAIL_CLASSIC") != nullptr) return;
+        HIPCHK(hipMemcpyAsync(h_pairs, d_pair_counters.p, 3 * sizeof(unsigned long long), hipMemcpyDeviceToHost, on));
+        pairs_queued = true;
+    }
+    Residual fetch_residual(int extra_slot = -1 , bool last = false,
+                            Event* join = nullptr) {
+        if (join) HIPCHK(hipStreamWaitEvent(stream, join->e, 0));
         HIPCHK(hipMemcpyAsync(h_pinned, slabs[0].sc.p, SC_COUNT * sizeof(double), hipMemcpyDeviceToHost, stream));
+        if (last) queue_pairs_copy(stream);
         HIPCHK(hipStreamSynchronize(stream));
+        if (pairs_queued) pairs_fetched = true;
+        pairs_queued = false;
         Residual r;
         r.rr0 = h_pinned[SC_RR0];
         r.rr = h_pinned[SC_RR];
@@ -1838,12 +1890,12 @@
         if (!converged) throw Error(SHM_ERR_NOCONV, fmt("%s: max_iters=%d reached, rel. residual %.3e > tol %.1e", name, o.max_iters, r.rel(), o.tol));
     }
     struct SampleTimer {
-        std::vector<std::unique_ptr<Event>> ev;
+        std::vector<Event*> ev;
         const int max_samples, per;
         int n = 0;
         bool on = false;
-        SampleTimer(bool enabled, int max_samples_, int events_per_sample) : max_samples(max_samples_), per(events_per_sample) {
-            if (enabled) for (int a = 0; a < per * max_samples; a++) ev.emplace_back(new Event());
+        SampleTimer(Solver& s, bool enabled, int max_samples_, int events_per_sample) : max_samples(max_samples_), per(events_per_sample) {
+            if (enabled) for (int a = 0; a < per * max_samples; a++) ev.push_back(&s.ev(EV_TIMER0 + a));
         }
         bool begin(bool wanted = true) { return on = !ev.empty() && n < max_samples && wanted; }
         void mark(int k, hipStream_t st) { if (on) ev[(size_t)(per * n + k)]->record(st); }
@@ -1870,11 +1922,12 @@
         }
     }
 
-    void launch_shift_and_phi() {
+    void launch_shift_and_phi(const double* also = nullptr, int also_n = 0, double* also_dst = nullptr) {
         for (Slab<T>& sl : slabs) {
             const int g = std::max(1, std::min(256, (sl.n_shift + kBlock - 1) / kBlock));
             hipLaunchKernelGGL((shift_partial_kernel<T>), dim3(g), dim3(kBlock), 0, stream, sl.n_shift, sl.shift_items.p, n, sl.x.p, sl.partials.p);
-            hipLaunchKernelGGL(finalize_sum_kernel, dim3(1), dim3(kBlock), 0, stream, sl.partials.p, g, sl.pq.p);
+            if (also) hipLaunchKernelGGL(finalize_sum2_kernel, dim3(2), dim3(kBlock), 0, stream, sl.partials.p, g, sl.pq.p, also, also_n, also_dst);
+            else hipLaunchKernelGGL(finalize_sum_kernel, dim3(1), dim3(kBlock), 0, stream, sl.partials.p, g, sl.pq.p);
         }
         allreduce(1, 1);
         for (Slab<T>& sl : slabs)
@@ -1885,7 +1938,7 @@
 
     void solve_fast(const shm_opts& o, shm_stats* st, SolveClock& clk) {
         (void)o;
-        Event e_int, e_end;
+        Event &e_int = ev(EV_PCG), &e_end = ev(EV_END);
         build_shift_items_only();
         Rccl* R = comm ? &Rccl::get() : nullptr;
         const int dt = sizeof(T) == 8 ? Rccl::kFloat64 : Rccl::kFloat32;
@@ -1907,7 +1960,7 @@
         e_int.record(stream);
         launch_shift_and_phi();
         e_end.record(stream);
-        fetch_residual();
+        fetch_residual(-1, true);
         have_phi = true;
         if (st) {
             fill_phase_stats(st, clk, e_int, e_end, 0, 0.);
@@ -1971,7 +2024,7 @@
     }
 
     void solve_dual(const shm_opts& o, shm_stats* st, SolveClock& clk) {
-        Event e_pcg, e_end;
+        Event &e_pcg = ev(EV_PCG), &e_end = ev(EV_END);
         const int check_every = o.check_every > 0 ? std::min(o.check_every, 4) : 2;
         auto mv = [&](Slab<T>& sl, int k) { return sl.dv.p + (size_t)k * mp; };
         enum { V_MU = 0, V_R = 1, V_P = 2, V_Z = 3, V_T1 = 4, V_T2 = 5, V_G = 6 };
@@ -1995,65 +2048,102 @@
                 hipLaunchKernelGGL(dual_direction_kernel, dim3(1), dim3(kDualBlock), 0, stream, m, init, mv(sl, V_R), mv(sl, V_Z), mv(sl, V_P), sl.sc.p);
             }
         };
+        const bool dense_S = have_S;
+        const bool direct = plan.dual_form == SHM_DUAL_DIRECT && dense_S;
+        const bool tail = direct && slabs.size() == 1 && comm == nullptr && knob("SHM_SOLVE_TAIL_CLASSIC") == nullptr;
+        Event &e_fork = ev(EV_FORK), &e_join = ev(EV_JOIN);
         launch_precond(false, ARR_R, ARR_Z);
-        gather(ARR_Z);
-        for (Slab<T>& sl : slabs) {
-            HIPCHK(hipMemcpyAsync(mv(sl, V_G), sl.red.p + 1, (size_t)m * sizeof(double), hipMemcpyDeviceToDevice, stream));
-            if (sl.div_sum_blocks > 0) {
-                hipLaunchKernelGGL(finalize_sum_kernel, dim3(1), dim3(kBlock), 0, stream, sl.div_partials.p, sl.div_sum_blocks, sl.pq.p);
-                continue;
-            }
-            const int g = grid_for(sl.nown, 1024);
-            hipLaunchKernelGGL((sum_kernel<T>), dim3(g), dim3(kBlock), 0, stream, sl.nown, sl.plane, sl.r.p, sl.partials.p);
-            hipLaunchKernelGGL(finalize_sum_kernel, dim3(1), dim3(kBlock), 0, stream, sl.partials.p, g, sl.pq.p);
-        }
-        allreduce(1, 1);
-        for (Slab<T>& sl : slabs) {
-            hipLaunchKernelGGL(dual_init_mu_kernel, dim3(1), dim3(kDualBlock), 0, stream, m, sl.pq.p, mv(sl, V_MU), sl.sc.p);
+        if (tail) {
+            Slab<T>& sl = slabs[0];
+            const double* b_partials = sl.div_partials.p;
+            int np = sl.div_sum_blocks;
+            if (np <= 0) {
+                np = grid_for(sl.nown, 1024);
+                b_partials = sl.partials.p;
+                hipLaunchKernelGGL((sum_kernel<T>), dim3(np), dim3(kBlock), 0, stream, sl.nown, sl.plane, sl.r.p, sl.partials.p);
+            }
+            hipLaunchKernelGGL((gather_rows_kernel<T>), dim3(1 + (8 * m + kBlock - 1) / kBlock), dim3(kBlock), 0, stream, m, sl.row_ptr.p, sl.ent_node.p, sl.ent_coef.p,
+                               arr(sl, ARR_Z), sl.partials.p, -1, mv(sl, V_G) - 1);
+            hipLaunchKernelGGL(dual_start_kernel, dim3(1), dim3(kDualBlock), 0, stream, m, b_partials, np, mv(sl, V_G), Sinv_ones.p + 2 * (size_t)mp, mv(sl, V_MU),
+                               mv(sl, V_R), sl.sc.p);
         }
         const bool sparse_ok = total_slabs == 1 && slabs[0].n_act_x > 0;
-        const bool dense_S = have_S;
-        if (!dense_S)
-            for (Slab<T>& sl : slabs) HIPCHK(hipMemsetAsync(sl.p.p, 0, sl.ntot * sizeof(T), stream));
         auto apply_S = [&](int vec) {
             for (Slab<T>& sl : slabs) launch_ginv_matvec<double>(stream, m, m, mp, Sdense.p, mv(sl, vec), sl.red.p + 1);
         };
-        if (dense_S) apply_S(V_MU);
-        else {
-            scatter(V_MU, ARR_P, 0);
-            if (sparse_ok) launch_precond_sparse(ARR_P, ARR_Z);
-            else launch_precond(false, ARR_P, ARR_Z);
+        if (!tail) {
             gather(ARR_Z);
-        }
-        for (Slab<T>& sl : slabs)
-            hipLaunchKernelGGL(dual_init_residual_kernel, dim3(1), dim3(kDualBlock), 0, stream, m, mv(sl, V_G), sl.red.p + 1, mv(sl, V_R), sl.sc.p, 1);
-        const bool direct = plan.dual_form == SHM_DUAL_DIRECT && dense_S;
+            for (Slab<T>& sl : slabs) {
+                HIPCHK(hipMemcpyAsync(mv(sl, V_G), sl.red.p + 1, (size_t)m * sizeof(double), hipMemcpyDeviceToDevice, stream));
+                if (sl.div_sum_blocks > 0) {
+                    hipLaunchKernelGGL(finalize_sum_kernel, dim3(1), dim3(kBlock), 0, stream, sl.div_partials.p, sl.div_sum_blocks, sl.pq.p);
+                    continue;
+                }
+                const int g = grid_for(sl.nown, 1024);
+                hipLaunchKernelGGL((sum_kernel<T>), dim3(g), dim3(kBlock), 0, stream, sl.nown, sl.plane, sl.r.p, sl.partials.p);
+                hipLaunchKernelGGL(finalize_sum_kernel, dim3(1), dim3(kBlock), 0, stream, sl.partials.p, g, sl.pq.p);
+            }
+            allreduce(1, 1);
+            for (Slab<T>& sl : slabs) {
+                hipLaunchKernelGGL(dual_init_mu_kernel, dim3(1), dim3(kDualBlock), 0, stream, m, sl.pq.p, mv(sl, V_MU), sl.sc.p);
+            }
+            if (!dense_S)
+                for (Slab<T>& sl : slabs) HIPCHK(hipMemsetAsync(sl.p.p, 0, sl.ntot * sizeof(T), stream));
+            if (dense_S) apply_S(V_MU);
+            else {
+                scatter(V_MU, ARR_P, 0);
+                if (sparse_ok) launch_precond_sparse(ARR_P, ARR_Z);
+                else launch_precond(false, ARR_P, ARR_Z);
+                gather(ARR_Z);
+            }
+            for (Slab<T>& sl : slabs)
+                hipLaunchKernelGGL(dual_init_residual_kernel, dim3(1), dim3(kDualBlock), 0, stream, m, mv(sl, V_G), sl.red.p + 1, mv(sl, V_R), sl.sc.p, 1);
+        }
         if (!direct) precondition(1);
         HIPCHK(hipGetLastError());
 
-        SampleTimer tm(st != nullptr, 32, 3);
+        SampleTimer tm(*this, st != nullptr, 32, 4);
         int it = 0;
         Residual res;
         bool converged = false, breakdown = false;
-        auto finish = [&]() {
+        auto finish = [&](bool fork_check = false) {
+            auto check_beside = [&]() {
+                if (!fork_check) return;
+                Slab<T>& sl = slabs[0];
+                e_fork.record(stream);
+                HIPCHK(hipStreamWaitEvent(stream2, e_fork.e, 0));
+                tm.mark(3, stream2);
+                launch_ginv_matvec<double>(stream2, m, m, mp, Sdense.p, mv(sl, V_MU), mv(sl, V_T2));
+                hipLaunchKernelGGL(dual_init_residual_kernel, dim3(1), dim3(kDualBlock), 0, stream2, m, mv(sl, V_G), mv(sl, V_T2), mv(sl, V_R), sl.sc.p, 0);
+                tm.mark(2, stream2);
+                queue_pairs_copy(stream2);
+                e_join.record(stream2);
+            };
             if (gemm_dct()) {
                 for (Slab<T>& sl : slabs)
                     hipLaunchKernelGGL((negate_kernel<T>), dim3(grid_for(sl.ntot, 4096)), dim3(kBlock), 0, stream, sl.ntot, sl.r.p, sl.q.p);
                 scatter(V_MU, ARR_Q, 1);
                 launch_precond(false, ARR_Q, ARR_X);
+                check_beside();
             } else {
                 scatter(V_MU, ARR_R, 1, -1.0, true);
                 launch_precond(false, ARR_R, ARR_X, -1.0);
+                check_beside();
                 for (Slab<T>& sl : slabs)
                     hipLaunchKernelGGL((restore_nodes_kernel<T>), dim3((sl.n_touched + kBlock - 1) / kBlock + 1), dim3(kBlock), 0, stream, sl.n_touched, sl.node_id.p,
                                        sl.touched_save.p, sl.r.p);
             }
             gather(ARR_X);
-            for (Slab<T>& sl : slabs) hipLaunchKernelGGL(finalize_sum_kernel, dim3(1), dim3(kBlock), 0, stream, sl.red.p + 1, m, sl.sc.p + SC_AXSUM);
-            e_pcg.record(stream);
-            launch_shift_and_phi();
+            if (tail) {
+                e_pcg.record(stream);
+                launch_shift_and_phi(slabs[0].red.p + 1, m, slabs[0].sc.p + SC_AXSUM);
+            } else {
+                for (Slab<T>& sl : slabs) hipLaunchKernelGGL(finalize_sum_kernel, dim3(1), dim3(kBlock), 0, stream, sl.red.p + 1, m, sl.sc.p + SC_AXSUM);
+                e_pcg.record(stream);
+                launch_shift_and_phi();
+            }
             e_end.record(stream);
-            return fetch_residual();
+            return fetch_residual(-1, true, fork_check ? &e_join : nullptr);
         };
         bool finished = false;
         if (direct) {
@@ -2068,14 +2158,16 @@
                     hipLaunchKernelGGL(dual_bordered_kernel, dim3(1), dim3(kDualBlock), 0, stream, m, mv(sl, V_T1), Sinv_ones.p, (const double*)nullptr, 1, mv(sl, V_MU));
                 }
                 tm.mark(1, stream);
-                apply_S(V_MU);
-                for (Slab<T>& sl : slabs)
-                    hipLaunchKernelGGL(dual_init_residual_kernel, dim3(1), dim3(kDualBlock), 0, stream, m, mv(sl, V_G), sl.red.p + 1, mv(sl, V_R), sl.sc.p, 0);
-                tm.mark(2, stream);
-                tm.end();
+                if (!tail) {
+                    apply_S(V_MU);
+                    for (Slab<T>& sl : slabs)
+                        hipLaunchKernelGGL(dual_init_residual_kernel, dim3(1), dim3(kDualBlock), 0, stream, m, mv(sl, V_G), sl.red.p + 1, mv(sl, V_R), sl.sc.p, 0);
+                    tm.mark(2, stream);
+                }
                 it++;
                 HIPCHK(hipGetLastError());
-                res = finish();
+                res = finish(tail);
+                tm.end();
                 finished = true;
                 if (!res.finite) breakdown = true;
                 else if (res.below(o.tol)) converged = true;
@@ -2114,7 +2206,7 @@
             fill_phase_stats(st, clk, e_pcg, e_end, it, res.rel());
             st->shift += h_pinned[SC_AXSUM] / (double)m;
             st->ms_precond_avg = tm.avg(0, 1);
-            st->ms_project_avg = tm.avg(1, 2);
+            st->ms_project_avg = tail ? tm.avg(3, 2) : tm.avg(1, 2);
             st->kernel_samples = tm.n;
             st->preconditioner = SHM_PRECOND_DCT;
             st->solver = total_slabs > 1 ? SHM_SOLVER_DUAL_SLABS : SHM_SOLVER_DUAL;
@@ -2138,8 +2230,8 @@
     void solve_gathered(const shm_opts& o, const PlanIn& in, shm_stats* st, SolveClock& clk) {
         Solver<T>& F = *full;
         Slab<T>& fs = F.slabs[0];
-        Event e_gather;
-        SolveClock fclk;
+        Event& e_gather = ev(EV_AUX0);
+        SolveClock fclk(F);
         fclk.wall0 = clk.wall0;
         fclk.has_step1 = false;
         fclk.e_s2a.record(F.stream2);
@@ -2211,7 +2303,7 @@
         bool overlap = total_slabs > 1 && !halo_serial;
         for (Slab<T>& sl : slabs) overlap = overlap && fused_cfg(sl).zchunks >= 3;
         if (overlap && !stream_h) HIPCHK(hipStreamCreateWithFlags(&stream_h, hipStreamNonBlocking));
-        Event e_ready, e_halo;
+        Event &e_ready = ev(EV_AUX0), &e_halo = ev(EV_AUX1);
         auto run_dir = [&](int k, int slot_old, int slot_new, int init) {
             auto sweep = [&](int part) {
                 for (size_t s = 0; s < slabs.size(); s++) {
@@ -2246,11 +2338,11 @@
         finalize_pq();
         HIPCHK(hipGetLastError());
 
-        SampleTimer tm(st != nullptr, 12, 8);
+        SampleTimer tm(*this, st != nullptr, 12, 8);
         const int sample_stride = pre ? 2 : 8;
         const bool xoverlap = total_slabs == 1 && !comm;
         const bool xsplit = xoverlap && !pre;
-        Event e_xfork, e_xjoin;
+        Event &e_xfork = ev(EV_AUX2), &e_xjoin = ev(EV_AUX3);
         hipStream_t const stream_x = stream2;
         int it = 0;
         Residual res;
@@ -2314,11 +2406,11 @@
     };
     void finish_primal(const shm_opts& o, shm_stats* st, bool pre, SolveClock& clk, SampleTimer& tm, int it, const Residual& res, bool converged, bool breakdown,
                        const PrimalLoop& loop) {
-        Event e_pcg, e_end;
+        Event &e_pcg = ev(EV_PCG), &e_end = ev(EV_END);
         e_pcg.record(stream);
         launch_shift_and_phi();
         e_end.record(stream);
-        fetch_residual();
+        fetch_residual(-1, true);
         have_phi = true;
         have_div = false;
         if (st) {
@@ -2344,7 +2436,7 @@
         update_p_all(SC_RHO_A, SC_RHO_A, 1, pre, nparts);
         HIPCHK(hipGetLastError());
 
-        SampleTimer tm(st != nullptr, 32, 8);
+        SampleTimer tm(*this, st != nullptr, 32, 8);
         const int sample_stride = pre ? 2 : 8;
         int it = 0;
         Residual res;
@@ -2393,7 +2485,8 @@
     void report_pairs(shm_stats* st) noexcept {
         if (!st || !d_pair_counters.p) return;
         unsigned long long h[3] = {0, 0, 0};
-        if (hipMemcpy(h, d_pair_counters.p, sizeof h, hipMemcpyDeviceToHost) != hipSuccess) return;
+        if (pairs_fetched) memcpy(h, h_pairs, sizeof h);
+        else if (hipMemcpy(h, d_pair_counters.p, sizeof h, hipMemcpyDeviceToHost) != hipSuccess) return;
         st->pairs_fp64 = (double)h[0];
         st->pairs_fp32 = (double)h[1];
         st->pairs_redone = (double)h[2];
@@ -2403,7 +2496,17 @@
         struct Fin {
             Solver* s;
             shm_stats* st;
-            ~Fin() { s->report_pairs(st); }
+            ~Fin() {
+                const HostClock::time_point t0 = HostClock::now();
+                s->report_pairs(st);
+                s->host_us[3] = us_since(t0);
+                if (knob("SHM_HOST_TIMES") != nullptr) {
+                    const auto verbose = s->cfg.verbose;
+                    s->cfg.verbose = 1;
+                    s->log("[shm] host us: plan %.1f step1-queue %.1f phase-stats %.1f pairs %.1f", s->host_us[0], s->host_us[1], s->host_us[2], s->host_us[3]);
+                    s->cfg.verbose = verbose;
+                }
+            }
         } fin{this, st};
         solve_impl(o_in, st);
     }
@@ -2411,8 +2514,10 @@
         need_problem();
         HIPCHK(hipSetDevice(cfg.device));
         shm_opts o = o_in;
+        const HostClock::time_point t_plan = HostClock::now();
         PlanIn in = plan_inputs(&o);
         const Plan p = plan_solve(in);
+        host_us[0] = us_since(t_plan);
         if (p.status != SHM_OK) throw Error(p.status, p.error);
         iso_idx_valid = false;
         ray_bricks_valid = false;
@@ -2422,12 +2527,10 @@
         if (o.max_iters <= 0) o.max_iters = 20 * n;
         if (o.check_every <= 0) o.check_every = pre ? 4 : 32;
 
-        SolveClock clk;
+        SolveClock clk(*this);
         step1_budget = o.step1_budget;
         select_step1_arith(o.step1_arith);
         clk.e_start.record(stream);
-        for (Slab<T>& sl : slabs)
-            if (sl.proj_ticket.p) HIPCHK(hipMemsetAsync(sl.proj_ticket.p, 0, sizeof(unsigned), stream));
         o_fast_hint = o.fast_integration != 0;
         launch_conv();
         clk.e_conv.record(stream);
```

New measurement: 696.6 million, median of 6. About the same (+0.6%).
